# choutilin/makani

Measured on AMD Instinct MI355X. Metric: SFNO fwd+bwd samples/sec, 73ch 721x1440, higher is better.
Workload: dtype bf16; 1 GPU; sfno_linear_73chq_sc3_layers8_edim384 fwd+bwd+Adam, 73ch 721x1440, per-GPU batch 1; global_batch=1, parallelism=h1, spectral_dtype=f32 (GEMMs as 6 bf16 MFMA products of exact 3-way operand splits), step_launch=eager, micro_batches=1, python_gc=disabled in the timed region, adam=after backward

## Files before the change

include/makani_amd.h:

```cpp
#ifndef MAKANI_AMD_H
#define MAKANI_AMD_H

#include <stdint.h>

#ifdef __cplusplus
extern "C" {
#endif

int mk_version(void);
const char* mk_last_error(void);


int mk_quadrature(int grid, int nlat, double* theta, double* weights);

int mk_legendre_kpad(int nlat);

int mk_legendre_table(int grid, int nlat, int lmax, int mmax, int with_quad_weights, float* out);

int mk_fft_twiddle_len(int nlon);
int mk_fft_twiddles(int nlon, float* out);

int mk_rfft(const void* x, int x_dtype, float* xf, const float* twiddles,
            int bc, int nlat, int nlon, int mmax, float scale0, float scale_m, float scale_h,
            void* stream);

int mk_irfft(const float* xf, void* x, int x_dtype, const float* twiddles,
             int bc, int nlat, int nlon, int mmax, float scale0, float scale_m, float scale_h,
             void* stream);

int mk_legendre_fwd(const float* xf, const float* tab, float* c,
                    int bc, int nlat, int lmax, int mmax_loc, int m_off, int mmax_glob, void* stream);

int mk_legendre_inv(const float* c, const float* tab, float* xf,
                    int bc, int nlat, int lmax, int mmax_loc, int m_off, int mmax_glob, void* stream);

long long mk_legendre_x3_bytes(int nlat, int lmax, int mmax, int inverse);
int mk_legendre_x3_split(const float* tab, void* out, int nlat, int lmax, int mmax, int inverse, void* stream);
int mk_legendre_fwd_x3(const float* xf, const void* tab_x3, float* c,
                       int bc, int nlat, int lmax, int mmax_loc, int m_off, int mmax_glob, void* stream);
int mk_legendre_inv_x3(const float* c, const void* tab_x3, float* xf,
                       int bc, int nlat, int lmax, int mmax_loc, int m_off, int mmax_glob, void* stream);

int mk_rfft_ex(const void* x, int x_dtype, float* xf, const float* twiddles, int bc, int nlat, int nlon,
               int mmax, float scale0, float scale_m, float scale_h, int xf_layout, void* stream);
int mk_irfft_ex(const float* xf, void* x, int x_dtype, const float* twiddles, int bc, int nlat, int nlon,
                int mmax, float scale0, float scale_m, float scale_h, int xf_layout, void* stream);
int mk_legendre_fwd_x3_ex(const float* xf, const void* tab_x3, float* c, int bc, int nlat, int lmax,
                          int mmax_loc, int m_off, int mmax_glob, int xf_layout, void* stream);
int mk_legendre_inv_x3_ex(const float* c, const void* tab_x3, float* xf, int bc, int nlat, int lmax,
                          int mmax_loc, int m_off, int mmax_glob, int xf_layout, void* stream);

int mk_rfft_pm(const void* x, int x_dtype, float* xf, const float* twiddles, int bc, int nlat, int nlon, int mmax,
               float scale0, float scale_m, float scale_h, int chans, int chans_per_peer, void* stream);
int mk_irfft_pm(const float* xf, void* x, int x_dtype, const float* twiddles, int bc, int nlat, int nlon, int mmax,
                float scale0, float scale_m, float scale_h, int chans, int chans_per_peer, void* stream);

int mk_irfft_sums(const float* xf, void* x, int x_dtype, const float* twiddles, int bc, int nlat, int nlon, int mmax,
                  float scale0, float scale_m, float scale_h, int xf_layout, int chans, int chans_per_peer, double* rowsums,
                  void* stream);

int mk_dhconv_fwd(const float* x, const float* w, float* y, int lloc, int mloc, int batch,
                  int cin, int cout, int l_off, int m_off, void* stream);
int mk_dhconv_dgrad(const float* gy, const float* w, float* gx, int lloc, int mloc, int batch,
                    int cin, int cout, int l_off, int m_off, void* stream);
int mk_dhconv_wgrad(const float* x, const float* gy, float* gw, int lloc, int mloc, int batch,
                    int cin, int cout, int l_off, int m_off, void* stream);

int mk_dhconv_fwd_x3(const float* x, const float* w, float* y, int lloc, int mloc, int batch,
                     int cin, int cout, int l_off, int m_off, void* stream);
int mk_dhconv_dgrad_x3(const float* gy, const float* w, float* gx, int lloc, int mloc, int batch,
                       int cin, int cout, int l_off, int m_off, void* stream);
int mk_dhconv_wgrad_x3(const float* x, const float* gy, float* gw, int lloc, int mloc, int batch,
                       int cin, int cout, int l_off, int m_off, void* stream);

int mk_diag_fwd(const float* x, const float* w, float* y, int batch, int cin, int cout, long long P, void* stream);
int mk_diag_dgrad(const float* gy, const float* w, float* gx, int batch, int cin, int cout, long long P, void* stream);
int mk_diag_wgrad(const float* x, const float* gy, float* gw, int batch, int cin, int cout, long long P, void* stream);

int mk_spec_pack(const float* c_std, float* c_prv, int bc, int lloc, int mloc, void* stream);
int mk_spec_unpack(const float* c_prv, float* c_std, int bc, int lloc, int mloc,
                   int l_off, int m_off, void* stream);

int mk_bias_gelu_fwd(const void* x, const float* bias, void* y, int dtype, int rows, int C, long long P,
                     void* stream);
int mk_bias_gelu_bwd(const void* x, const float* bias, const void* gy, void* gx, float* gbias, int dtype,
                     int rows, int C, long long P, void* stream);
int mk_instnorm_fwd(const void* x, const float* weight, const float* bias, void* y, float* stats,
                    double* workspace, int dtype, int rows, int C, long long P, float eps, int fuse_gelu,
                    void* stream);
int mk_instnorm_bwd(const void* x, const void* gy, const float* stats, const float* weight, const float* bias,
                    void* gx, double* workspace, int dtype, int rows, int C, long long P, int fuse_gelu,
                    void* stream);

int mk_instnorm_fwd_ex(const void* x, const float* weight, const float* bias, void* y, float* stats,
                       double* workspace, int dtype, int rows, int C, long long P, long long count, float eps,
                       int fuse_gelu, int phase, void* stream);
int mk_instnorm_bwd_ex(const void* x, const void* gy, const float* stats, const float* weight, const float* bias,
                       void* gx, double* workspace, int dtype, int rows, int C, long long P, long long count,
                       int fuse_gelu, int phase, void* stream);
int mk_instnorm_bwd_wb(const void* x, const void* gy, const float* stats, const float* weight, const float* bias, void* gx,
                       double* workspace, float* gwb, int dtype, int C, long long P, int fuse_gelu, void* stream);

int mk_wmse_fwd(const void* pred, int dtype, const float* tar, const float* wrow, double* loss, long long rows,
                int H, int W, float scale, void* stream);
int mk_wmse_bwd(const void* pred, int dtype, const float* tar, const float* wrow, const float* gloss, void* gpred,
                long long rows, int H, int W, float scale, void* stream);

int mk_conv1x1_x3(const float* a, long long lda, const float* b, long long ldb, float* c, long long ldc, int M, int K, long long N,
                  int batch, long long sa, long long sb, long long sc, int mode, void* stream);
int mk_conv1x1_x3_bias_act(const float* a, long long lda, const float* b, long long ldb, float* c, long long ldc, int M, int K,
                           long long N, int batch, long long sb, long long sc, const float* bias, int act, void* stream);

int mk_conv1x1_wgrad(const void* gy, const void* x, float* gw, int batch, int cout, int cin, long long P,
                     void* stream);
int mk_conv1x1_wgrad_act(const void* gy, const void* x, float* gw, int batch, int cout, int cin, long long P, int x_act,
                         void* stream);
long long mk_pce_image_bytes(int M, int K);
int mk_pce_pack(const void* w, int w_dtype , int transpose, int M, int K, int ldw, void* img,
                void* stream);
int mk_pce_pack_layout(int M, int K, long long* out3);
int mk_pce_pack_batch(const void* desc_dev, int n, void* arena, long long total_elements, void* stream);
int mk_pce_gemm(const void* x, const void* wimg, void* y, const float* bias, const void* addend, const void* aux_in,
                void* aux_out, int gelu, int batch, int M, int K, long long P, void* stream);
int mk_pce_gemm_ex(const void* x, const void* wimg, void* y, const float* bias, const void* addend, const float* addend_affine,
                   const void* aux_in, void* aux_out, int gelu, double* rowstats, int batch, int M, int K, long long P,
                   void* stream);
long long mk_pce_mlp_image_bytes(int M, int Hd, int K1);
int mk_pce_mlp_pack(const void* a1, int a1_transposed, int lda1, const void* a2, int a2_transposed, int lda2,
                    int w_dtype , int M, int Hd, int K1, void* img, void* stream);
int mk_pce_mlp(const void* x, const void* wimg, void* y, void* mid_out, const void* mid_in, const float* b1, const float* b2,
               double* rowstats_y, double* rowsum_mid, int mode, int batch, int M, int Hd, int K1, long long P, void* stream);
int mk_pce_mlp_debug_stamps(unsigned long long* out512);
int mk_instnorm_coeffs(const double* sums, const float* weight, const float* bias, float* stats, float* affine, int rows,
                       int C, long long count, float eps, void* stream);
int mk_pce_debug_stamps(unsigned long long* out512);

int mk_adam_step(float* p, const float* g, float* m, float* v, long long n, float lr, float beta1, float beta2, float eps,
                 float weight_decay, int step, void* stream);

long long mk_mt_chunks(long long n);
int mk_mt_sumsq(int T, const uint64_t* x, const long long* n, double* partials, double* tsum, int clip_mode, float max_norm,
                float* norm_out, float* coef_out, float* steps, const int* inc_slots, int ninc, void* stream);
int mk_mt_norm_finish(int T, const double* tsum, int clip_mode, float max_norm, float* norm_out, float* coef_out,
                      float* steps, const int* inc_slots, int ninc, void* stream);
int mk_mt_step_inc(float* steps, const int* slots, int nslots, void* stream);
int mk_mt_scale(int T, const uint64_t* x, const long long* n, const float* coef, void* stream);
int mk_mt_adam(int T, const uint64_t* pgmv, const long long* n, const int* step_or_slot, const float* steps, float lr,
               const float* lr_dev, float beta1, float beta2, float eps, float weight_decay, int adamw, const float* coef,
               void* stream);
int mk_mt_lamb(int stage, int T, const uint64_t* pgmv, const long long* n, const int* step_or_slot, const float* steps,
               float lr, const float* lr_dev, float beta1, float beta2, float beta3, float eps, float weight_decay, int adamw,
               int bias_correction, int trust, const float* coef, double* part_p, double* part_u, double* tsum_p,
               double* tsum_u, void* stream);

long long mk_geo_metric_workspace(int B, int C, int H);
int mk_geo_metric_sums(const void* pred, int dtype, const float* tar, const float* clim, const float* wrow, double* workspace,
                       double* sums, int B, int C, int H, int W, void* stream);

long long mk_geo_lp_workspace(int B, int C, int H);
int mk_geo_lp_sums(const void* pred, int dtype, const float* tar, const float* wrow, double* workspace, double* sums, int p,
                   int B, int C, int H, int W, void* stream);
int mk_geo_lp_bwd(const void* pred, int dtype, const float* tar, const float* wrow, const float* g, void* gpred, int p,
                  int B, int C, int H, int W, void* stream);

int mk_input_assemble(const void* x, int x_dtype, const float* u, const float* stat, const float* mean, const float* std,
                      const int* mask_chans, int n_mask, int mask_src, void* out, int out_dtype, int B, int T, int C, int Cu,
                      int Cs, int H, int W, void* stream);
int mk_input_assemble_bwd(const void* gout, int g_dtype, const float* stat, const float* std, const int* mask_chans, int n_mask,
                          int mask_src, void* gx, int x_dtype, int B, int T, int C, int Cu, int Cs, int H, int W, void* stream);
// ... 10 lines not shown
```

makani_amd/_lib.py:

```python
import ctypes
import os

import torch

from . import build as _build

_LIB = None

_c_int = ctypes.c_int
_c_float = ctypes.c_float
_vp = ctypes.c_void_p

SIGNATURES = {
    "mk_version": (_c_int, []),
    "mk_last_error": (ctypes.c_char_p, []),
    "mk_quadrature": (_c_int, [_c_int, _c_int, _vp, _vp]),
    "mk_legendre_kpad": (_c_int, [_c_int]),
    "mk_legendre_table": (_c_int, [_c_int, _c_int, _c_int, _c_int, _c_int, _vp]),
    "mk_fft_twiddle_len": (_c_int, [_c_int]),
    "mk_fft_twiddles": (_c_int, [_c_int, _vp]),
    "mk_rfft": (_c_int, [_vp, _c_int, _vp, _vp, _c_int, _c_int, _c_int, _c_int, _c_float, _c_float, _c_float, _vp]),
    "mk_irfft": (_c_int, [_vp, _vp, _c_int, _vp, _c_int, _c_int, _c_int, _c_int, _c_float, _c_float, _c_float, _vp]),
    "mk_legendre_fwd": (_c_int, [_vp, _vp, _vp, _c_int, _c_int, _c_int, _c_int, _c_int, _c_int, _vp]),
    "mk_legendre_inv": (_c_int, [_vp, _vp, _vp, _c_int, _c_int, _c_int, _c_int, _c_int, _c_int, _vp]),
    "mk_legendre_x3_bytes": (ctypes.c_longlong, [_c_int, _c_int, _c_int, _c_int]),
    "mk_legendre_x3_split": (_c_int, [_vp, _vp, _c_int, _c_int, _c_int, _c_int, _vp]),
    "mk_legendre_fwd_x3": (_c_int, [_vp, _vp, _vp, _c_int, _c_int, _c_int, _c_int, _c_int, _c_int, _vp]),
    "mk_legendre_inv_x3": (_c_int, [_vp, _vp, _vp, _c_int, _c_int, _c_int, _c_int, _c_int, _c_int, _vp]),
    "mk_rfft_ex": (_c_int, [_vp, _c_int, _vp, _vp, _c_int, _c_int, _c_int, _c_int, _c_float, _c_float, _c_float, _c_int, _vp]),
    "mk_irfft_ex": (_c_int, [_vp, _vp, _c_int, _vp, _c_int, _c_int, _c_int, _c_int, _c_float, _c_float, _c_float, _c_int, _vp]),
    "mk_rfft_pm": (_c_int, [_vp, _c_int, _vp, _vp, _c_int, _c_int, _c_int, _c_int, _c_float, _c_float, _c_float, _c_int, _c_int, _vp]),
    "mk_irfft_pm": (_c_int, [_vp, _vp, _c_int, _vp, _c_int, _c_int, _c_int, _c_int, _c_float, _c_float, _c_float, _c_int, _c_int, _vp]),
    "mk_irfft_sums": (_c_int, [_vp, _vp, _c_int, _vp, _c_int, _c_int, _c_int, _c_int, _c_float, _c_float, _c_float, _c_int, _c_int,
                               _c_int, _vp, _vp]),
    "mk_legendre_fwd_x3_ex": (_c_int, [_vp, _vp, _vp, _c_int, _c_int, _c_int, _c_int, _c_int, _c_int, _c_int, _vp]),
    "mk_legendre_inv_x3_ex": (_c_int, [_vp, _vp, _vp, _c_int, _c_int, _c_int, _c_int, _c_int, _c_int, _c_int, _vp]),
    "mk_dhconv_fwd": (_c_int, [_vp, _vp, _vp] + [_c_int] * 7 + [_vp]),
    "mk_dhconv_dgrad": (_c_int, [_vp, _vp, _vp] + [_c_int] * 7 + [_vp]),
    "mk_dhconv_wgrad": (_c_int, [_vp, _vp, _vp] + [_c_int] * 7 + [_vp]),
    "mk_dhconv_fwd_x3": (_c_int, [_vp, _vp, _vp] + [_c_int] * 7 + [_vp]),
    "mk_dhconv_dgrad_x3": (_c_int, [_vp, _vp, _vp] + [_c_int] * 7 + [_vp]),
    "mk_dhconv_wgrad_x3": (_c_int, [_vp, _vp, _vp] + [_c_int] * 7 + [_vp]),
    "mk_diag_fwd": (_c_int, [_vp, _vp, _vp, _c_int, _c_int, _c_int, ctypes.c_longlong, _vp]),
    "mk_diag_dgrad": (_c_int, [_vp, _vp, _vp, _c_int, _c_int, _c_int, ctypes.c_longlong, _vp]),
    "mk_diag_wgrad": (_c_int, [_vp, _vp, _vp, _c_int, _c_int, _c_int, ctypes.c_longlong, _vp]),
    "mk_spec_pack": (_c_int, [_vp, _vp, _c_int, _c_int, _c_int, _vp]),
    "mk_spec_unpack": (_c_int, [_vp, _vp, _c_int, _c_int, _c_int, _c_int, _c_int, _vp]),
    "mk_bias_gelu_fwd": (_c_int, [_vp, _vp, _vp, _c_int, _c_int, _c_int, ctypes.c_longlong, _vp]),
    "mk_bias_gelu_bwd": (_c_int, [_vp, _vp, _vp, _vp, _vp, _c_int, _c_int, _c_int, ctypes.c_longlong, _vp]),
    "mk_instnorm_fwd": (_c_int, [_vp, _vp, _vp, _vp, _vp, _vp, _c_int, _c_int, _c_int, ctypes.c_longlong, _c_float,
                                 _c_int, _vp]),
    "mk_instnorm_fwd_ex": (_c_int, [_vp, _vp, _vp, _vp, _vp, _vp, _c_int, _c_int, _c_int, ctypes.c_longlong,
                                    ctypes.c_longlong, _c_float, _c_int, _c_int, _vp]),
    "mk_instnorm_bwd_ex": (_c_int, [_vp, _vp, _vp, _vp, _vp, _vp, _vp, _c_int, _c_int, _c_int, ctypes.c_longlong,
                                    ctypes.c_longlong, _c_int, _c_int, _vp]),
    "mk_instnorm_bwd_wb": (_c_int, [_vp, _vp, _vp, _vp, _vp, _vp, _vp, _vp, _c_int, _c_int, ctypes.c_longlong, _c_int, _vp]),
    "mk_wmse_fwd": (_c_int, [_vp, _c_int, _vp, _vp, _vp, ctypes.c_longlong, _c_int, _c_int, _c_float, _vp]),
    "mk_wmse_bwd": (_c_int, [_vp, _c_int, _vp, _vp, _vp, _vp, ctypes.c_longlong, _c_int, _c_int, _c_float, _vp]),
    "mk_conv1x1_wgrad": (_c_int, [_vp, _vp, _vp, _c_int, _c_int, _c_int, ctypes.c_longlong, _vp]),
    "mk_conv1x1_x3": (_c_int, [_vp, ctypes.c_longlong, _vp, ctypes.c_longlong, _vp, ctypes.c_longlong, _c_int, _c_int, ctypes.c_longlong,
                               _c_int, ctypes.c_longlong, ctypes.c_longlong, ctypes.c_longlong, _c_int, _vp]),
    "mk_conv1x1_x3_bias_act": (_c_int, [_vp, ctypes.c_longlong, _vp, ctypes.c_longlong, _vp, ctypes.c_longlong, _c_int, _c_int,
                                        ctypes.c_longlong, _c_int, ctypes.c_longlong, ctypes.c_longlong, _vp, _c_int, _vp]),
    "mk_conv1x1_wgrad_act": (_c_int, [_vp, _vp, _vp, _c_int, _c_int, _c_int, ctypes.c_longlong, _c_int, _vp]),
    "mk_pce_mlp_image_bytes": (ctypes.c_longlong, [_c_int, _c_int, _c_int]),
    "mk_pce_mlp_pack": (_c_int, [_vp, _c_int, _c_int, _vp, _c_int, _c_int, _c_int, _c_int, _c_int, _c_int, _vp, _vp]),
    "mk_pce_mlp": (_c_int, [_vp, _vp, _vp, _vp, _vp, _vp, _vp, _vp, _vp, _c_int, _c_int, _c_int, _c_int, _c_int,
                            ctypes.c_longlong, _vp]),
    "mk_pce_mlp_debug_stamps": (_c_int, [_vp]),
    "mk_pce_image_bytes": (ctypes.c_longlong, [_c_int, _c_int]),
    "mk_pce_pack": (_c_int, [_vp, _c_int, _c_int, _c_int, _c_int, _c_int, _vp, _vp]),
    "mk_pce_pack_layout": (_c_int, [_c_int, _c_int, _vp]),
    "mk_pce_pack_batch": (_c_int, [_vp, _c_int, _vp, ctypes.c_longlong, _vp]),
    "mk_pce_gemm": (_c_int, [_vp, _vp, _vp, _vp, _vp, _vp, _vp, _c_int, _c_int, _c_int, _c_int, ctypes.c_longlong, _vp]),
    "mk_pce_gemm_ex": (_c_int, [_vp, _vp, _vp, _vp, _vp, _vp, _vp, _vp, _c_int, _vp, _c_int, _c_int, _c_int, ctypes.c_longlong, _vp]),
    "mk_instnorm_coeffs": (_c_int, [_vp, _vp, _vp, _vp, _vp, _c_int, _c_int, ctypes.c_longlong, ctypes.c_float, _vp]),
    "mk_pce_debug_stamps": (_c_int, [_vp]),
    "mk_adam_step": (_c_int, [_vp, _vp, _vp, _vp, ctypes.c_longlong] + [_c_float] * 5 + [_c_int, _vp]),
    "mk_instnorm_bwd": (_c_int, [_vp, _vp, _vp, _vp, _vp, _vp, _vp, _c_int, _c_int, _c_int, ctypes.c_longlong,
                                 _c_int, _vp]),
    "mk_mt_chunks": (ctypes.c_longlong, [ctypes.c_longlong]),
    "mk_mt_sumsq": (_c_int, [_c_int, _vp, _vp, _vp, _vp, _c_int, _c_float, _vp, _vp, _vp, _vp, _c_int, _vp]),
    "mk_mt_norm_finish": (_c_int, [_c_int, _vp, _c_int, _c_float, _vp, _vp, _vp, _vp, _c_int, _vp]),
    "mk_mt_step_inc": (_c_int, [_vp, _vp, _c_int, _vp]),
    "mk_mt_scale": (_c_int, [_c_int, _vp, _vp, _vp, _vp]),
    "mk_mt_adam": (_c_int, [_c_int, _vp, _vp, _vp, _vp, _c_float, _vp] + [_c_float] * 4 + [_c_int, _vp, _vp]),
    "mk_mt_lamb": (_c_int, [_c_int, _c_int, _vp, _vp, _vp, _vp, _c_float, _vp] + [_c_float] * 5 + [_c_int] * 3
                   + [_vp] * 6),
    "mk_geo_metric_workspace": (ctypes.c_longlong, [_c_int, _c_int, _c_int]),
    "mk_geo_metric_sums": (_c_int, [_vp, _c_int, _vp, _vp, _vp, _vp, _vp, _c_int, _c_int, _c_int, _c_int, _vp]),
    "mk_geo_lp_workspace": (ctypes.c_longlong, [_c_int, _c_int, _c_int]),
    "mk_geo_lp_sums": (_c_int, [_vp, _c_int, _vp, _vp, _vp, _vp] + [_c_int] * 5 + [_vp]),
    "mk_geo_lp_bwd": (_c_int, [_vp, _c_int, _vp, _vp, _vp, _vp] + [_c_int] * 5 + [_vp]),
    "mk_input_assemble": (_c_int, [_vp, _c_int, _vp, _vp, _vp, _vp, _vp, _c_int, _c_int, _vp, _c_int] + [_c_int] * 7 + [_vp]),
    "mk_input_assemble_bwd": (_c_int, [_vp, _c_int, _vp, _vp, _vp, _c_int, _c_int, _vp, _c_int] + [_c_int] * 7 + [_vp]),
    "mk_history_workspace": (ctypes.c_longlong, [_c_int, _c_int, _c_int]),
    "mk_history_sums": (_c_int, [_vp, _c_int, _vp, _vp, _vp, _vp] + [_c_int] * 6 + [_vp]),
}


def lib_path():
    return _build.LIB


def load():
    global _LIB
    if _LIB is not None:
        return _LIB
    path = _build.LIB
    override = os.environ.get("MK_LIB_OVERRIDE")
    if override:
        path = override
    elif _build.stale():
        if _build.have_hipcc():
            path = _build.build(verbose=False)
        elif not os.path.exists(path):
            raise RuntimeError(f"makani_amd: {path} is missing and hipcc is not available to build it")
        else:
            raise RuntimeError(f"makani_amd: {path} is older than its sources and hipcc is not available to rebuild it")
    try:
        lib = ctypes.CDLL(path)
    except OSError as e:
        raise RuntimeError(f"makani_amd: cannot load the HIP extension {path}: {e}") from e
    for name, (res, args) in SIGNATURES.items():
        fn = getattr(lib, name)
# ... 11 lines not shown
```

makani_amd/csrc/fft.hip:

```cpp
#include "common.h"
#include "../../include/makani_amd.h"

#include <hip/hip_bf16.h>
#include <cstdlib>
#include <type_traits>
#include <utility>

namespace {

struct XfLayout {
    int sm, sk;
    int C, Cp, Bn;
    long long pstride;
};
static thread_local XfLayout g_xl = {0, 0, 0, 0, 0, 0};
static thread_local double* g_rowsums = nullptr;

struct XfChan {
    size_t pbase;
    int bcx0, BCx;
};
__device__ __forceinline__ XfChan xf_chan(const XfLayout& xl, int bc0, int BC) {
    XfChan c{0, bc0, BC};
    if (xl.Cp) {
        const int b = bc0 / xl.C, ch = bc0 - b * xl.C, pp = ch / xl.Cp;
        c.pbase = (size_t)pp * (size_t)xl.pstride;
        c.bcx0 = b * xl.Cp + (ch - pp * xl.Cp);
        c.BCx = xl.Bn * xl.Cp;
    }
    return c;
}


template <int I>
using IC = std::integral_constant<int, I>;

template <class F, int... Is>
__device__ __forceinline__ void static_for_impl(F&& f, std::integer_sequence<int, Is...>) {
    (f(IC<Is>{}), ...);
}
template <int N, class F>
__device__ __forceinline__ void static_for(F&& f) {
    static_for_impl(static_cast<F&&>(f), std::make_integer_sequence<int, N>{});
}

constexpr double kPi = 3.14159265358979323846264338327950288;

constexpr double cx_reduce(double x) {
    while (x > kPi) x -= 2.0 * kPi;
    while (x < -kPi) x += 2.0 * kPi;
    return x;
}
constexpr double cx_sin(double x) {
    x = cx_reduce(x);
    double term = x, sum = x;
    for (int n = 1; n < 20; ++n) {
        term *= -x * x / ((2.0 * n) * (2.0 * n + 1.0));
        sum += term;
    }
    return sum;
}
constexpr double cx_cos(double x) {
    x = cx_reduce(x);
    double term = 1.0, sum = 1.0;
    for (int n = 1; n < 20; ++n) {
        term *= -x * x / ((2.0 * n - 1.0) * (2.0 * n));
        sum += term;
    }
    return sum;
}

__device__ __forceinline__ float2 cmul(float2 a, float2 b) {
    return make_float2(a.x * b.x - a.y * b.y, a.x * b.y + a.y * b.x);
}
__device__ __forceinline__ float2 cadd(float2 a, float2 b) { return make_float2(a.x + b.x, a.y + b.y); }
__device__ __forceinline__ float2 csub(float2 a, float2 b) { return make_float2(a.x - b.x, a.y - b.y); }
__device__ __forceinline__ float2 mul_mi(float2 a) { return make_float2(a.y, -a.x); }

template <int R>
struct Dft;

template <>
struct Dft<2> {
    static __device__ __forceinline__ void run(float2 (&v)[2]) {
        const float2 a = v[0], b = v[1];
        v[0] = cadd(a, b);
        v[1] = csub(a, b);
    }
};

template <>
struct Dft<3> {
    static __device__ __forceinline__ void run(float2 (&v)[3]) {
        constexpr float s = 0.86602540378443864676f;
        const float2 t = cadd(v[1], v[2]);
        const float2 d = csub(v[1], v[2]);
        const float2 m = make_float2(v[0].x - 0.5f * t.x, v[0].y - 0.5f * t.y);
        const float2 q = mul_mi(make_float2(s * d.x, s * d.y));
// ... 403 lines not shown
    float* x = (float*)xout;
    MK_REQUIRE(x_dtype == 0 || x_dtype == 1, "x_dtype must be 0 (fp32) or 1 (bf16)");
    MK_REQUIRE(x_dtype == 0 || (!fft_legacy() && mmax <= 241 && (nlon == 480 || nlon == 1440)),
               "bf16 output rows are built for the production lengths only (nlon 480 / 1440, mmax <= 241)");
    MK_REQUIRE(x && xf && twiddles, "null pointer");
    MK_REQUIRE(bc > 0 && nlat > 0 && nlon >= 2 && nlon % 2 == 0, "bad sizes (nlon must be even)");
    MK_REQUIRE(mmax >= 1 && mmax <= nlon / 2 + 1, "mmax out of range");
    MK_REQUIRE((long long)nlat * mk::ceil_div(bc, 8) < 2147483647LL, "grid too large");
    hipStream_t st = (hipStream_t)stream;
    const bool split = !fft_legacy() && mmax <= 241 && (nlon == 480 || nlon == 1440);
    if (split && nlon == 480) {
        launch_irfft_split<1>(xf, xout, x_dtype, twiddles, bc, nlat, mmax, scale0, scale_m, scale_h, st);
    } else if (split) {
        launch_irfft_split<3>(xf, xout, x_dtype, twiddles, bc, nlat, mmax, scale0, scale_m, scale_h, st);
    } else
    switch (nlon / 2) {
#define X(H, G) \
    case H:     \
        launch_irfft<H, G>(xf, x, twiddles, bc, nlat, mmax, scale0, scale_m, scale_h, st); \
        break;
        MK_FFT_SIZES(X)
#undef X
        default: {
            MK_REQUIRE((long long)nlat * bc < 2147483647LL, "grid too large");
            const dim3 grid((unsigned)(nlat * bc));
            const size_t lds = sizeof(float2) * mmax;
            hipLaunchKernelGGL(irdft_generic_kernel, grid, dim3(kThreads), lds, st, (const float2*)xf, x,
                               (const float2*)twiddles, bc, nlat, nlon, mmax, scale0, scale_m, scale_h, g_xl);
        }
    }
    MK_LAUNCH_CHECK();
    return 0;
}

static int fft_pm_setup(int bc, int nlat, int nlon, int mmax, int chans, int chans_per_peer) {
    MK_REQUIRE(chans > 0 && chans_per_peer > 0 && bc % chans == 0 && chans % chans_per_peer == 0, "bad channel blocking");
    MK_REQUIRE(chans_per_peer % 24 == 0, "channel blocks must be multiples of 24 (tiles of 8 / 24 rows must not straddle them)");
    MK_REQUIRE(!fft_legacy() && mmax <= 241 && (nlon == 480 || nlon == 1440), "peer-major rows exist for the split kernels only");
    const int Bn = bc / chans;
    g_xl = XfLayout{1, mmax, chans, chans_per_peer, Bn, (long long)nlat * mmax * Bn * chans_per_peer};
    return 0;
}

extern "C" int mk_rfft_pm(const void* x, int x_dtype, float* xf, const float* twiddles, int bc, int nlat, int nlon, int mmax,
                          float scale0, float scale_m, float scale_h, int chans, int chans_per_peer, void* stream) {
    MK_REQUIRE(x && xf && twiddles, "null pointer");
    MK_REQUIRE(bc > 0 && nlat > 0 && mmax >= 1, "bad sizes");
    MK_REQUIRE(x_dtype == 0 || x_dtype == 1, "x_dtype must be 0 (fp32) or 1 (bf16)");
    if (int e = fft_pm_setup(bc, nlat, nlon, mmax, chans, chans_per_peer)) return e;
    if (nlon == 480)
        launch_rfft_split<1>(x, x_dtype, xf, twiddles, bc, nlat, mmax, scale0, scale_m, scale_h, (hipStream_t)stream);
    else
        launch_rfft_split<3>(x, x_dtype, xf, twiddles, bc, nlat, mmax, scale0, scale_m, scale_h, (hipStream_t)stream);
    MK_LAUNCH_CHECK();
    return 0;
}

extern "C" int mk_irfft_pm(const float* xf, void* x, int x_dtype, const float* twiddles, int bc, int nlat, int nlon, int mmax,
                           float scale0, float scale_m, float scale_h, int chans, int chans_per_peer, void* stream) {
    MK_REQUIRE(x && xf && twiddles, "null pointer");
    MK_REQUIRE(bc > 0 && nlat > 0 && mmax >= 1, "bad sizes");
    MK_REQUIRE(x_dtype == 0 || x_dtype == 1, "x_dtype must be 0 (fp32) or 1 (bf16)");
    if (int e = fft_pm_setup(bc, nlat, nlon, mmax, chans, chans_per_peer)) return e;
    if (nlon == 480)
        launch_irfft_split<1>(xf, x, x_dtype, twiddles, bc, nlat, mmax, scale0, scale_m, scale_h, (hipStream_t)stream);
    else
        launch_irfft_split<3>(xf, x, x_dtype, twiddles, bc, nlat, mmax, scale0, scale_m, scale_h, (hipStream_t)stream);
    MK_LAUNCH_CHECK();
    return 0;
}

extern "C" int mk_irfft_sums(const float* xf, void* x, int x_dtype, const float* twiddles, int bc, int nlat, int nlon, int mmax,
                             float scale0, float scale_m, float scale_h, int xf_layout, int chans, int chans_per_peer,
                             double* rowsums, void* stream) {
    MK_REQUIRE(rowsums != nullptr, "null pointer");
    MK_REQUIRE(!fft_legacy() && mmax <= 241 && (nlon == 480 || nlon == 1440), "row statistics come from the split kernels only");
    g_rowsums = rowsums;
    const int rc = chans_per_peer > 0
        ? mk_irfft_pm(xf, x, x_dtype, twiddles, bc, nlat, nlon, mmax, scale0, scale_m, scale_h, chans, chans_per_peer, stream)
        : mk_irfft_ex(xf, x, x_dtype, twiddles, bc, nlat, nlon, mmax, scale0, scale_m, scale_h, xf_layout, stream);
    g_rowsums = nullptr;
    return rc;
}
```

makani_amd/csrc/fft_split.h:

```cpp

constexpr int SH = 240;
constexpr int SP = 272;
constexpr int SNSUB = 24;
constexpr int STHREADS = 384;
constexpr int SLDS_F2 = SNSUB * SP + 96;

__device__ __forceinline__ int pair_tile(int i) {
    const int xcd = i & 7, seq = i >> 3;
    return ((((seq >> 1) << 3) + xcd) << 1) + (seq & 1);
}

__device__ __forceinline__ int sub_base(int sr, int S) { return sr * SP + 4 * (sr / S); }
__device__ __forceinline__ int phi(int i) { return i + (i >> 4); }
__device__ __forceinline__ int opaque(int v) {
    asm volatile("" : "+v"(v));
    return v;
}

template <typename T> __device__ __forceinline__ float as_stored(float v);
template <> __device__ __forceinline__ float as_stored<float>(float v) { return v; }
template <> __device__ __forceinline__ float as_stored<__hip_bfloat16>(float v) { return __bfloat162float(__float2bfloat16(v)); }

template <bool SUMS = false, typename TOut = float>
__device__ __forceinline__ void split_passes(float2* lds, int tid, int S, const float2 (&tw15)[15], float* red = nullptr) {
// ... 111 lines not shown
#pragma unroll
            for (int c = 0; c < S; ++c) InVec<TIn>::unpack(raw[it][c], vals[c]);
#pragma unroll
            for (int sq = 0; sq < S; ++sq) {
                float4* dst = reinterpret_cast<float4*>(lds + sub_base(g * S + sq, S) + (E / 2) * p);
#pragma unroll
                for (int h = 0; h < E / 4; ++h) {
                    float o[4];
#pragma unroll
                    for (int a = 0; a < 4; ++a) {
                        const int f = (4 * h + a) * S + sq;
                        o[a] = vals[f / E][f % E];
                    }
                    dst[h] = make_float4(o[0], o[1], o[2], o[3]);
                }
            }
        }
    }
    __syncthreads();
    if (!(exp & 2)) split_passes(lds, tid, S, tw15);
    float2 wfirst[S];
    wfirst[0] = tw[HH + S * (tid / G)];
#pragma unroll
    for (int s = 1; s < S; ++s) wfirst[s] = tw[HH + s * (tid / G)];
    __syncthreads();
    if (exp & 8) return;

    const float2* tw2 = tw + HH;
    constexpr int NPAIR = SH / 2 + 1;
    constexpr int STEP = STHREADS / G, PIT = (NPAIR + STEP - 1) / STEP;
    static_assert(STHREADS % G == 0, "items of a thread must keep their channel");
    const int mp0 = tid / G, g = tid - mp0 * G;
    if (bc0 + g < BC) {
        float2* dst0 = xf + xc.pbase + ((size_t)mp0 * xl.sm + (size_t)k * xl.sk) * xc.BCx + (xc.bcx0 + g);
        float2* dst1 = xf + xc.pbase + ((size_t)(SH - mp0) * xl.sm + (size_t)k * xl.sk) * xc.BCx + (xc.bcx0 + g);
        const ptrdiff_t dstep = (ptrdiff_t)STEP * xl.sm * xc.BCx;
#pragma unroll
        for (int it = 0; it < PIT; ++it) {
            const int mp = mp0 + STEP * it;
            if (mp < NPAIR) {
                const int m1 = SH - mp;
                const int p0 = phi(mp), p1 = phi(mp == 0 ? 0 : m1);
                const float2 wsub = it ? cmul(wfirst[0], tw2[S * STEP * it]) : wfirst[0];
                float2 acc0 = make_float2(0.f, 0.f), acc1 = make_float2(0.f, 0.f);
#pragma unroll
                for (int s = 0; s < S; ++s) {
                    const float2* zs = lds + sub_base(g * S + s, S);
                    const float2 a = zs[p0];
                    const float2 b = zs[p1];
                    const float2 e = make_float2(0.5f * (a.x + b.x), 0.5f * (a.y - b.y));
                    const float2 d = make_float2(0.5f * (a.x - b.x), 0.5f * (a.y + b.y));
                    const float2 pp = cmul(wsub, d);
                    float2 f0 = make_float2(e.x + pp.y, e.y - pp.x);
                    float2 f1 = make_float2(e.x - pp.y, -e.y - pp.x);
                    if (s > 0) {
                        const float2 w = it ? cmul(wfirst[s], tw2[s * STEP * it]) : wfirst[s];
                        constexpr float kc[3] = {1.f, 0.5f, -0.5f}, ks[3] = {0.f, -0.86602540378443864676f, -0.86602540378443864676f};
                        static_assert(S == 1 || S == 3, "combine constants are for S = 3");
                        f0 = cmul(f0, w);
                        f1 = cmul(f1, cmul(make_float2(w.x, -w.y), make_float2(kc[s], ks[s])));
                    }
                    acc0 = cadd(acc0, f0);
                    acc1 = cadd(acc1, f1);
                }
                if (exp & 4) {
                    if (acc0.x + acc1.x != 12345.678f) continue;
                }
                if (mp < M) {
                    const float sc = (mp == 0) ? scale0 : scale_m;
                    dst0[(ptrdiff_t)it * dstep] = make_float2(sc * acc0.x, sc * acc0.y);
                }
                if (m1 != mp && m1 < M) {
                    const float sc = (m1 == HH) ? scale_h : scale_m;
                    dst1[-(ptrdiff_t)it * dstep] = make_float2(sc * acc1.x, sc * acc1.y);
                }
            }
        }
    }
}

template <typename T> struct OutVec;
template <> struct OutVec<float> {
    static constexpr int E = 4;
    static __device__ __forceinline__ void store(float* p, const float (&o)[4]) {
        *reinterpret_cast<float4*>(p) = make_float4(o[0], o[1], o[2], o[3]);
    }
};
template <> struct OutVec<__hip_bfloat16> {
    static constexpr int E = 8;
    static __device__ __forceinline__ void store(__hip_bfloat16* p, const float (&o)[8]) {
        __hip_bfloat16 h[8];
#pragma unroll
        for (int i = 0; i < 8; ++i) h[i] = __float2bfloat16(o[i]);
        *reinterpret_cast<uint4*>(p) = *reinterpret_cast<const uint4*>(h);
    }
};

template <int S, typename TOut, bool WIDE, int PERSIST, bool SUMS = false>
__global__ __launch_bounds__(STHREADS, PERSIST ? 3 : 5) void irfft_split_kernel(const float2* __restrict__ xf, TOut* __restrict__ x,
                                                               const float2* __restrict__ tw, int BC, int K, int M,
                                                               float scale0, float scale_m, float scale_h, XfLayout xl,
                                                               double* __restrict__ rowsums) {
    constexpr int N = 480 * S, G = SNSUB / S, HH = N / 2;
    extern __shared__ __attribute__((aligned(16))) float2 lds[];
    float* red = reinterpret_cast<float*>(lds + SLDS_F2);
    const int tid = threadIdx.x;
    const int ntile = (BC + G - 1) / G;
    const int total = ntile * K;
    const float2* tw2 = tw + HH;
    const int total16 = (total + 15) & ~15;
    auto next_valid = [&](int i) {
        while (i < total16 && pair_tile(i) >= total) i += (int)gridDim.x;
        return i;
    };
    int sched = PERSIST ? next_valid(blockIdx.x) : (int)blockIdx.x;
    if (sched >= total16) return;
    int tile = pair_tile(sched);
    if (!PERSIST && tile >= total) return;

    float2 tw15[15];
    auto load_tw15 = [&]() {
#pragma unroll
        for (int r = 0; r < 15; ++r) tw15[r] = tw[((tid & 15) * r) * S];
    };
    if constexpr (PERSIST != 0) load_tw15();

    float2 wfirst[S];
    wfirst[0] = tw2[S * (tid / G)];
#pragma unroll
    for (int s = 1; s < S; ++s) wfirst[s] = tw2[s * (tid / G)];

    constexpr int NPAIR = SH / 2 + 1;
    constexpr int PIT = (G * NPAIR + STHREADS - 1) / STHREADS;
    float2 xa[PIT], xb[PIT];
    constexpr int STEP = STHREADS / G;
    static_assert(STHREADS % G == 0 && PIT == (NPAIR + STEP - 1) / STEP, "items of a thread keep their channel");
    auto gather = [&](int t, int tl) {
        const int k = t / ntile, bc0 = (t - k * ntile) * G;
        const XfChan xc = xf_chan(xl, bc0, BC);
        const int jp0 = tl / G, g = tl - jp0 * G;
        const bool chan_ok = bc0 + g < BC;
        if constexpr (!WIDE) {
            typedef unsigned int gf_u2 __attribute__((ext_vector_type(2)));
            const float2* tbase = xf + xc.pbase + (size_t)k * xl.sk * xc.BCx + xc.bcx0;
            const __amdgpu_buffer_rsrc_t rs = __builtin_amdgcn_make_buffer_rsrc(const_cast<float2*>(tbase), 0, 0x7FFFFFFF, 0x00020000);
            const unsigned mstride = (unsigned)xl.sm * (unsigned)xc.BCx * 8u;
            unsigned offa = (unsigned)g * 8u + (unsigned)jp0 * mstride;
            unsigned offb = (unsigned)g * 8u + (unsigned)(SH - jp0) * mstride;
            const unsigned dstepb = (unsigned)STEP * mstride;
#pragma unroll
            for (int it = 0; it < PIT; ++it) {
                const int jp = jp0 + STEP * it, j1 = SH - jp;
                const bool oa = chan_ok && jp < NPAIR && jp < M, ob = chan_ok && jp < NPAIR && j1 < M;
                xa[it] = __builtin_bit_cast(float2, (gf_u2)__builtin_amdgcn_raw_buffer_load_b64(rs, oa ? offa : 0x80000000u, 0, 0));
                xb[it] = __builtin_bit_cast(float2, (gf_u2)__builtin_amdgcn_raw_buffer_load_b64(rs, ob ? offb : 0x80000000u, 0, 0));
                offa += dstepb;
                offb -= dstepb;
            }
        } else {
            const float2* base = xf + xc.pbase + (size_t)k * xl.sk * xc.BCx + (xc.bcx0 + g);
#pragma unroll
            for (int it = 0; it < PIT; ++it) {
                const int jp = jp0 + STEP * it, j1 = SH - jp;
                const bool oa = chan_ok && jp < NPAIR && jp < M, ob = chan_ok && jp < NPAIR && j1 < M;
                xa[it] = *(oa ? base + (size_t)jp * xl.sm * xc.BCx : xf);
                xb[it] = *(ob ? base + (size_t)j1 * xl.sm * xc.BCx : xf);
            }
        }
    };
    gather(tile, tid);
  for (;;) {
    const int tl = opaque(tid);
    const int k = tile / ntile, bc0 = (tile - k * ntile) * G;
    const int jp0 = tl / G, g = tl - jp0 * G;
    const bool chan_ok = bc0 + g < BC;
#pragma unroll
    for (int it = 0; it < PIT; ++it) {
        const int jp = jp0 + STEP * it;
        if (jp >= NPAIR) continue;
        const int j1 = SH - jp;
        const float sa = (chan_ok && jp < M) ? ((jp == 0) ? scale0 : scale_m) : 0.f;
        const float sb = (chan_ok && j1 < M) ? ((j1 == HH) ? scale_h : scale_m) : 0.f;
        const float2 a0 = make_float2(sa * xa[it].x, sa * xa[it].y);
        const float2 b0 = make_float2(sb * xb[it].x, sb * xb[it].y);
        float2 wsub = it ? cmul(wfirst[0], tw2[S * STEP * it]) : wfirst[0];
        wsub.y = -wsub.y;
#pragma unroll
        for (int s = 0; s < S; ++s) {
            float2 ya = a0, yb = b0;
            if (s > 0) {
                constexpr float kc[3] = {1.f, 0.5f, -0.5f}, ks[3] = {0.f, 0.86602540378443864676f, 0.86602540378443864676f};
                const float2 w = it ? cmul(wfirst[s], tw2[s * STEP * it]) : wfirst[s];
                ya = cmul(ya, make_float2(w.x, -w.y));
                yb = cmul(yb, cmul(w, make_float2(kc[s], ks[s])));
            }
            if (jp == 0) {
                ya.y = 0.f;
                yb.y = 0.f;
                if (S > 1) yb.x *= 2.f;
            }
            const float2 e = make_float2(ya.x + yb.x, ya.y - yb.y);
            const float2 d = make_float2(ya.x - yb.x, ya.y + yb.y);
            const float2 t = cmul(wsub, d);
            float2* zs = lds + sub_base(g * S + s, S);
            zs[jp] = make_float2(e.x - t.y, -(e.y + t.x));
            if (jp != 0 && j1 != jp) zs[j1] = make_float2(e.x + t.y, e.y - t.x);
        }
    }
    if constexpr (PERSIST == 0) load_tw15();
    __syncthreads();
    const int next = PERSIST ? next_valid(sched + (int)gridDim.x) : total16;
    if (next < total16) gather(pair_tile(next), opaque(tid));
    if constexpr (SUMS) split_passes<true, TOut>(lds, tl, S, tw15, red);
    else split_passes(lds, tl, S, tw15);
    __syncthreads();
    if (SUMS && tl < 2 * G) {
        const int gch = tl >> 1, t = tl & 1;
        if (bc0 + gch < BC) {
            float v = 0.f;
#pragma unroll
            for (int sq = 0; sq < S; ++sq) v += red[2 * (gch * S + sq) + t];
            atomicAdd(&rowsums[2 * (size_t)(bc0 + gch) + t], (double)v);
        }
    }

    constexpr int EO = OutVec<TOut>::E;
    constexpr int GPR = N / (EO * S), NGRP = G * GPR, OIT = (NGRP + STHREADS - 1) / STHREADS;
#pragma unroll
    for (int it = 0; it < OIT; ++it) {
        const int v = tl + it * STHREADS;
        const int g = v / GPR, p = v - g * GPR;
        if (v < NGRP && bc0 + g < BC) {
            float r[S][EO];
#pragma unroll
            for (int sq = 0; sq < S; ++sq) {
                const float2* zs = lds + sub_base(g * S + sq, S) + phi((EO / 2) * p);
#pragma unroll
                for (int h = 0; h < EO / 2; ++h) {
                    const float2 z = zs[h];
                    r[sq][2 * h] = z.x;
                    r[sq][2 * h + 1] = -z.y;
                }
            }
            TOut* dst = x + ((size_t)(bc0 + g) * K + k) * N + (size_t)p * EO * S;
#pragma unroll
            for (int c = 0; c < S; ++c) {
                float o[EO];
#pragma unroll
                for (int e = 0; e < EO; ++e) {
                    const int f = c * EO + e;
                    o[e] = r[f % S][f / S];
                }
                OutVec<TOut>::store(dst + c * EO, o);
            }
        }
    }
    if (next >= total16) break;
    sched = next;
    tile = pair_tile(next);
    __syncthreads();
  }
}

static inline unsigned split_grid(long long tiles) { return (unsigned)((tiles + 15) / 16 * 16); }

static inline int fft_exp() {
    static const int v = [] { const char* e = getenv("MK_FFT_EXP"); return e ? atoi(e) : 0; }();
    return v;
}

template <int S>
int launch_rfft_split(const void* x, int x_dtype, float* xf, const float* tw, int bc, int nlat, int mmax, float s0,
                      float sm, float sh, hipStream_t st) {
    constexpr int G = SNSUB / S;
    const dim3 grid((unsigned)((mk::ceil_div(bc, G) * nlat + 15) / 16 * 16));
    const size_t lds = sizeof(float2) * SLDS_F2;
    if (x_dtype == 0)
        hipLaunchKernelGGL((rfft_split_kernel<S, float>), grid, dim3(STHREADS), lds, st, (const float*)x, (float2*)xf,
                           (const float2*)tw, bc, nlat, mmax, s0, sm, sh, fft_exp(), g_xl);
    else
        hipLaunchKernelGGL((rfft_split_kernel<S, __hip_bfloat16>), grid, dim3(STHREADS), lds, st,
                           (const __hip_bfloat16*)x, (float2*)xf, (const float2*)tw, bc, nlat, mmax, s0, sm, sh, fft_exp(), g_xl);
    return 0;
}

template <int S>
int launch_irfft_split(const float* xf, void* x, int x_dtype, const float* tw, int bc, int nlat, int mmax, float s0,
                       float sm, float sh, hipStream_t st) {
    constexpr int G = SNSUB / S;
    const dim3 grid(split_grid(mk::ceil_div(bc, G) * (long long)nlat));
    const size_t lds = sizeof(float2) * SLDS_F2 + 2 * SNSUB * sizeof(float);
    const long long bcx = g_xl.Cp ? (long long)g_xl.Bn * g_xl.Cp : (long long)bc;
    const bool wide = ((long long)SH * g_xl.sm + 1) * bcx * 8 >= (1LL << 31);
#define MK_IRFFT_LAUNCH(T, W, PS, SM)                                                                                  \
    hipLaunchKernelGGL((irfft_split_kernel<S, T, W, PS, SM>), grid, dim3(STHREADS), lds, st, (const float2*)xf, (T*)x,    \
                       (const float2*)tw, bc, nlat, mmax, s0, sm, sh, g_xl, g_rowsums)
#define MK_IRFFT_PICK(T)                                                                                               \
    if (g_rowsums) {                                                                                                   \
        if (wide) MK_IRFFT_LAUNCH(T, true, 1, true); else MK_IRFFT_LAUNCH(T, false, 0, true);                          \
    } else {                                                                                                           \
        if (wide) MK_IRFFT_LAUNCH(T, true, 1, false); else MK_IRFFT_LAUNCH(T, false, 0, false);                        \
    }
    if (x_dtype == 0) {
        MK_IRFFT_PICK(float)
    } else {
        MK_IRFFT_PICK(__hip_bfloat16)
    }
#undef MK_IRFFT_PICK
#undef MK_IRFFT_LAUNCH
    return 0;
}

static inline bool fft_legacy() {
    static const bool v = [] {
        const char* e = getenv("MK_FFT_LEGACY");
        return e && e[0] == '1';
    }();
    return v;
}
```

makani_amd/csrc/gemm_x3.hip:

```cpp
#include "common.h"
#include "../../include/makani_amd.h"

#include <cstdint>
#include <cstdlib>

namespace {

typedef float f32x16 __attribute__((ext_vector_type(16)));
typedef __bf16 bf16x8 __attribute__((ext_vector_type(8)));
typedef uint32_t u32x4 __attribute__((ext_vector_type(4)));

#ifndef MK_X3_DB
#define MK_X3_DB 1
#endif
constexpr int X3_DB = MK_X3_DB;
constexpr int XT = 256;
constexpr int XM = 128, XN = 128, XK = 32;
constexpr int XPITCH = 208;
constexpr int XROWB = 192;
constexpr int XIMG = XM * XPITCH + 128;
constexpr int X3_LDS = 2 * XIMG;

__device__ __forceinline__ int plain_off(int r) { return r * XPITCH; }
__device__ __forceinline__ int pair_off(int r) { return ((r >> 1) + ((r & 1) << 6)) * XPITCH + ((r & 1) << 7); }
// ... 247 lines not shown
#pragma unroll
                for (int t = 0; t < 6; ++t)
#pragma unroll
                    for (int b = 0; b < 2; ++b) {
#if defined(MK_X3_SKIP25)
                        if (s == 1 && b == 1) continue;
#endif
#if defined(MK_X3_NOMFMA)
                        acc[a][b][t] += __builtin_bit_cast(float4, af[PA[t]]).x * __builtin_bit_cast(float4, bf[b][PB[t]]).y;
#elif defined(MK_X3_AGPR)
                        asm volatile("v_mfma_f32_32x32x16_bf16 %0, %1, %2, %0" : "+a"(acc[a][b]) : "v"(af[PA[t]]), "v"(bf[b][PB[t]]));
#else
                        acc[a][b] = __builtin_amdgcn_mfma_f32_32x32x16_bf16(af[PA[t]], bf[b][PB[t]], acc[a][b], 0, 0, 0);
#endif
                    }
            }
    }
}

template <int DB, class AS, class BS, int EPI = 0>
__device__ __forceinline__ void x3_tile(const AS& as, const BS& bs, int kt0, int kt1, int rvalid, int cvalid, float* cbase,
                                        long long ldc, char* lds, int exp = 0, const float* rowbias = nullptr, int act = 0) {
    const int tid = threadIdx.x, lane = tid & 63;
    const int wave = __builtin_amdgcn_readfirstlane(tid >> 6);
    const int wr = wave >> 1, wc = wave & 1;
    const int fi = lane & 31, kg = lane >> 5;
    char* As = lds;
    char* Bs = lds + XIMG;

    f32x16 acc[2][2];
#pragma unroll
    for (int a = 0; a < 2; ++a)
#pragma unroll
        for (int b = 0; b < 2; ++b)
#pragma unroll
            for (int r = 0; r < 16; ++r) acc[a][b][r] = 0.f;
#if !defined(MK_X3_VGPR_ACC)
    asm volatile("" : "+a"(acc[0][0]), "+a"(acc[0][1]), "+a"(acc[1][0]), "+a"(acc[1][1]));
#endif

    bool live[2];
    int a_off[2], b_off[2];
#pragma unroll
    for (int a = 0; a < 2; ++a) {
        a_off[a] = AS::row_off(wr * 64 + a * 32 + fi) + kg * 16;
        b_off[a] = BS::row_off(wc * 64 + 2 * fi + a) + kg * 16;
        live[a] = (wr * 64 + a * 32 < rvalid) && (wc * 64 < cvalid);
    }

    typename AS::Regs ra;
    typename BS::Regs rb[DB];
    if (kt0 < kt1) {
        as.gload(kt0, ra, tid);
        bs.gload(kt0, rb[0], tid);
        as.sstore(ra, As, tid);
        bs.sstore(rb[0], Bs, tid);
        __syncthreads();
        if (kt0 + 1 < kt1) as.gload(kt0 + 1, ra, tid);
#pragma unroll
        for (int j = 0; j < DB; ++j)
            if (kt0 + 1 + j < kt1) bs.gload(kt0 + 1 + j, rb[j], tid);
    }
    for (int ktb = kt0; ktb < kt1; ktb += DB) {
#pragma unroll
        for (int j = 0; j < DB; ++j) {
            const int kt = ktb + j;
            if (kt >= kt1) break;
            if (!(exp & 4)) x3_mfma_step(As, Bs, a_off, b_off, live, acc);
            if (kt + 1 < kt1) {
                __syncthreads();
                if (!(exp & 2)) {
                    as.sstore(ra, As, tid);
                    bs.sstore(rb[j], Bs, tid);
                }
                __syncthreads();
                if (!(exp & 1)) {
                    if (kt + 2 < kt1 && !(exp & 8)) as.gload(kt + 2, ra, tid);
                    if (kt + 1 + DB < kt1 && !(exp & 16)) bs.gload(kt + 1 + DB, rb[j], tid);
                }
            }
        }
    }
    const int col = wc * 64 + 2 * fi;
    if (col < cvalid) {
#pragma unroll
        for (int a = 0; a < 2; ++a)
#pragma unroll
            for (int r = 0; r < 16; ++r) {
                const int row = wr * 64 + a * 32 + (r & 3) + 8 * (r >> 2) + 4 * kg;
                if (row < rvalid) {
                    if constexpr (EPI == 1) {
                        float2* d = reinterpret_cast<float2*>(cbase + (long long)row * ldc + col);
                        const float2 o = *d;
                        *d = make_float2(o.x + acc[a][0][r], o.y + acc[a][1][r]);
                        continue;
                    } else if constexpr (EPI == 2) {
                        atomicAdd(cbase + (long long)row * ldc + col, acc[a][0][r]);
                        if (col + 1 < cvalid) atomicAdd(cbase + (long long)row * ldc + col + 1, acc[a][1][r]);
                        continue;
                    } else if constexpr (EPI == 3) {
                        const float bv = rowbias ? rowbias[row] : 0.f;
                        float v0 = acc[a][0][r] + bv, v1 = acc[a][1][r] + bv;
                        if (act) {
                            v0 = 0.5f * v0 * (1.f + erff(v0 * 0.70710678118654752440f));
                            v1 = 0.5f * v1 * (1.f + erff(v1 * 0.70710678118654752440f));
                        }
                        *reinterpret_cast<float2*>(cbase + (long long)row * ldc + col) = make_float2(v0, v1);
                        continue;
                    }
#ifndef MK_X3_PLAIN_STORE
                    typedef float x3_f2 __attribute__((ext_vector_type(2)));
                    x3_f2 v2;
                    v2[0] = acc[a][0][r];
                    v2[1] = acc[a][1][r];
                    __builtin_nontemporal_store(v2, reinterpret_cast<x3_f2*>(cbase + (long long)row * ldc + col));
#else
                    *reinterpret_cast<float2*>(cbase + (long long)row * ldc + col) = make_float2(acc[a][0][r], acc[a][1][r]);
#endif
                }
            }
    }
}

struct TileId {
    int batch, tm, tn;
    bool valid;
};
__device__ __forceinline__ TileId decode_block(int nbatch, int tiles_m, int tiles_n) {
    const int bid = blockIdx.x;
    const int xcd = bid & 7, q = bid >> 3;
    const int T = tiles_m * tiles_n;
    TileId t;
    t.batch = (q / T) * 8 + xcd;
    const int r = q % T;
    t.tm = r / tiles_n;
    t.tn = r - t.tm * tiles_n;
    t.valid = t.batch < nbatch;
    return t;
}
static inline long long grid_blocks(int nbatch, int tiles_m, int tiles_n) {
    return (long long)mk::ceil_div(nbatch, 8) * 8 * tiles_m * tiles_n;
}

static int x3_exp() {
    static const int v = [] { const char* e = getenv("MK_X3_EXP"); return e ? atoi(e) : 0; }();
    return v;
}

struct LegX3Params {
    const float* src;
    const char* tab;
    float* dst;
    int K, L, Mloc, m_off, N2;
    int RT;
    int KC;
    int tiles_n;
    int kmajor;
    int exp;
};

template <class AS>
__global__ __launch_bounds__(XT, 3) void legendre_fwd_x3_kernel(LegX3Params p) {
    extern __shared__ __attribute__((aligned(16))) char lds_x3[];
    const TileId t = decode_block(p.Mloc, p.RT, p.tiles_n);
    if (!t.valid) return;
    const int m = t.batch, mg = p.m_off + m;
// ... 195 lines not shown
    if (nblk >= 2147483647LL) return -1;
    if (33LL * p.Mloc * p.N2 * 4 >= (1LL << 31)) return -2;
    const dim3 grid((unsigned)nblk), blk(XT);
    if (fwd) hipLaunchKernelGGL(legendre_fwd_x3_kernel<F32TileStager>, grid, blk, X3_LDS, st, p);
    else hipLaunchKernelGGL(legendre_inv_x3_kernel<F32TileStager>, grid, blk, X3_LDS, st, p);
    return 0;
}

extern "C" int mk_legendre_fwd_x3_ex(const float* xf, const void* tab_x3, float* c, int bc, int nlat, int lmax,
                                     int mmax_loc, int m_off, int mmax_glob, int xf_layout, void* stream) {
    MK_REQUIRE(xf && tab_x3 && c, "null pointer");
    MK_REQUIRE(bc > 0 && nlat > 0 && lmax > 0 && mmax_loc > 0, "bad sizes");
    MK_REQUIRE(m_off >= 0 && m_off + mmax_loc <= mmax_glob, "mode shard out of range");
    MK_REQUIRE(xf_layout == 0 || xf_layout == 1, "xf_layout must be 0 ([M][K][BC]) or 1 ([K][M][BC])");
    MK_REQUIRE(legendre_x3_launch(true, xf, tab_x3, c, bc, nlat, lmax, mmax_loc, m_off, xf_layout, (hipStream_t)stream) == 0,
               "operand too large: grid over 2^31 blocks, or 33 * mmax_loc * 2 * bc * 4 bytes (one k-step of the data operand) over 2^31");
    MK_LAUNCH_CHECK();
    return 0;
}

extern "C" int mk_legendre_fwd_x3(const float* xf, const void* tab_x3, float* c, int bc, int nlat, int lmax, int mmax_loc,
                                  int m_off, int mmax_glob, void* stream) {
    return mk_legendre_fwd_x3_ex(xf, tab_x3, c, bc, nlat, lmax, mmax_loc, m_off, mmax_glob, 0, stream);
}

extern "C" int mk_legendre_inv_x3_ex(const float* c, const void* tab_x3, float* xf, int bc, int nlat, int lmax,
                                     int mmax_loc, int m_off, int mmax_glob, int xf_layout, void* stream) {
    MK_REQUIRE(xf && tab_x3 && c, "null pointer");
    MK_REQUIRE(bc > 0 && nlat > 0 && lmax > 0 && mmax_loc > 0, "bad sizes");
    MK_REQUIRE(m_off >= 0 && m_off + mmax_loc <= mmax_glob, "mode shard out of range");
    MK_REQUIRE(xf_layout == 0 || xf_layout == 1, "xf_layout must be 0 ([M][K][BC]) or 1 ([K][M][BC])");
    MK_REQUIRE(legendre_x3_launch(false, c, tab_x3, xf, bc, nlat, lmax, mmax_loc, m_off, xf_layout, (hipStream_t)stream) == 0,
               "operand too large: grid over 2^31 blocks, or 33 * mmax_loc * 2 * bc * 4 bytes (one k-step of the data operand) over 2^31");
    MK_LAUNCH_CHECK();
    return 0;
}

extern "C" int mk_legendre_inv_x3(const float* c, const void* tab_x3, float* xf, int bc, int nlat, int lmax, int mmax_loc,
                                  int m_off, int mmax_glob, void* stream) {
    return mk_legendre_inv_x3_ex(c, tab_x3, xf, bc, nlat, lmax, mmax_loc, m_off, mmax_glob, 0, stream);
}

static int dh_x3_check(const void* a, const void* b, const void* c, int lloc, int mloc, int batch, int cin, int cout,
                       int l_off, int m_off) {
    MK_REQUIRE(a && b && c, "null pointer");
    MK_REQUIRE(lloc > 0 && mloc > 0 && batch > 0 && cin > 0 && cout > 0, "bad sizes");
    MK_REQUIRE(l_off >= 0 && m_off >= 0, "negative shard offset");
    MK_REQUIRE(cin % 2 == 0 && cout % 2 == 0, "the bf16x3 dhconv kernels need even channel counts (use the fp32 kernels)");
    return 0;
}

extern "C" int mk_dhconv_fwd_x3(const float* x, const float* w, float* y, int lloc, int mloc, int batch, int cin,
                                int cout, int l_off, int m_off, void* stream) {
    if (int e = dh_x3_check(x, w, y, lloc, mloc, batch, cin, cout, l_off, m_off)) return e;
    DhX3Params p{x, w, y, lloc, mloc, batch, cin, cout, l_off, m_off, mk::ceil_div(mloc * batch, XM),
                 mk::ceil_div(2 * cout, XN), x3_exp()};
    const long long nblk = grid_blocks(lloc, p.tiles_m, p.tiles_n);
    MK_REQUIRE(nblk < 2147483647LL, "grid too large");
    hipLaunchKernelGGL(dhconv_fwd_x3_kernel, dim3((unsigned)nblk), dim3(XT), X3_LDS, (hipStream_t)stream, p);
    MK_LAUNCH_CHECK();
    return 0;
}

extern "C" int mk_dhconv_dgrad_x3(const float* gy, const float* w, float* gx, int lloc, int mloc, int batch, int cin,
                                  int cout, int l_off, int m_off, void* stream) {
    if (int e = dh_x3_check(gy, w, gx, lloc, mloc, batch, cin, cout, l_off, m_off)) return e;
    DhX3Params p{gy, w, gx, lloc, mloc, batch, cin, cout, l_off, m_off, mk::ceil_div(mloc * batch, XM),
                 mk::ceil_div(2 * cin, XN), x3_exp()};
    const long long nblk = grid_blocks(lloc, p.tiles_m, p.tiles_n);
    MK_REQUIRE(nblk < 2147483647LL, "grid too large");
    hipLaunchKernelGGL(dhconv_dgrad_x3_kernel, dim3((unsigned)nblk), dim3(XT), X3_LDS, (hipStream_t)stream, p);
    MK_LAUNCH_CHECK();
    return 0;
}

extern "C" int mk_dhconv_wgrad_x3(const float* x, const float* gy, float* gw, int lloc, int mloc, int batch, int cin,
                                  int cout, int l_off, int m_off, void* stream) {
    if (int e = dh_x3_check(x, gy, gw, lloc, mloc, batch, cin, cout, l_off, m_off)) return e;
    DhX3Params p{x, gy, gw, lloc, mloc, batch, cin, cout, l_off, m_off, mk::ceil_div(cin, XM),
                 mk::ceil_div(2 * cout, XN), x3_exp()};
    const long long nblk = grid_blocks(lloc, p.tiles_m, p.tiles_n);
    MK_REQUIRE(nblk < 2147483647LL, "grid too large");
    hipLaunchKernelGGL(dhconv_wgrad_x3_kernel, dim3((unsigned)nblk), dim3(XT), X3_LDS, (hipStream_t)stream, p);
    MK_LAUNCH_CHECK();
    return 0;
}


namespace {
struct ConvX3Params {
    const float* a;
    const float* b;
    float* c;
    long long lda, ldb, ldc, sa, sb, sc;
    int M, K, N, nwork, tiles_m, tiles_n, nslab, kslab;
    const float* bias;
    int act;
};
template <int MODE>
__global__ __launch_bounds__(XT, 3) void conv_x3_kernel(ConvX3Params p) {
    extern __shared__ __attribute__((aligned(16))) char lds_x3[];
    TileId t = decode_block(p.nwork, p.tiles_m, MODE == 2 ? p.tiles_n : 1);
    if (!t.valid) return;
    if constexpr (MODE != 2) {
        const int w = t.batch;
        t.batch = w / p.tiles_n;
        t.tn = w - t.batch * p.tiles_n;
    }
    const int m0 = t.tm * XM, n0 = t.tn * XN;
    if constexpr (MODE == 2) {
        const int b = t.batch / p.nslab, slab = t.batch - b * p.nslab;
        const int kt0 = slab * p.kslab, ktn = (p.K + XK - 1) / XK;
        const int kt1 = kt0 + p.kslab < ktn ? kt0 + p.kslab : ktn;
        RowStager as, bs;
        as.base = p.a + b * p.sa + (long long)m0 * p.lda;
        as.ld = p.lda;
        as.rows = p.M - m0;
        as.kvalid = p.K;
        bs.base = p.b + b * p.sb + (long long)n0 * p.ldb;
        bs.ld = p.ldb;
        bs.rows = p.N - n0;
        bs.kvalid = p.K;
        x3_tile<X3_DB, RowStager, RowStager, 2>(as, bs, kt0, kt1, p.M - m0, p.N - n0, p.c + (long long)m0 * p.ldc + n0, p.ldc, lds_x3);
    } else {
        RowStager as;
        as.base = p.a + (long long)m0 * p.lda;
        as.ld = p.lda;
        as.rows = p.M - m0;
        as.kvalid = (p.K + 3) / 4 * 4;
        TransStager bs;
        bs.base = p.b + t.batch * p.sb + n0;
        bs.ldk = p.ldb;
        bs.k_lo = 0;
        bs.k_hi = p.K;
        bs.cvalid = p.N - n0;
        x3_tile<X3_DB, RowStager, TransStager, MODE>(as, bs, 0, (p.K + XK - 1) / XK, p.M - m0, p.N - n0,
                                                     p.c + t.batch * p.sc + (long long)m0 * p.ldc + n0, p.ldc, lds_x3, 0,
                                                     (MODE == 3 && p.bias) ? p.bias + m0 : nullptr, p.act);
    }
}
}

static int conv_x3_launch(const float* a, long long lda, const float* b, long long ldb, float* c, long long ldc, int M, int K,
                          long long N, int batch, long long sa, long long sb, long long sc, int mode, const float* bias, int act,
                          void* stream) {
    MK_REQUIRE(a && b && c, "null pointer");
    MK_REQUIRE(M > 0 && K > 0 && N > 0 && batch > 0, "bad sizes");
    MK_REQUIRE(mode >= 0 && mode <= 3, "mode must be 0 (store), 1 (accumulate), 2 (weight gradient) or 3 (store with bias / GELU)");
    MK_REQUIRE((((uintptr_t)a | (uintptr_t)b | (uintptr_t)c) & 15) == 0, "operands must be 16-byte aligned");
    ConvX3Params p;
    p.a = a; p.b = b; p.c = c;
    p.lda = lda; p.ldb = ldb; p.ldc = ldc;
    p.sa = sa; p.sb = sb; p.sc = sc;
    p.M = M; p.K = K;
    p.bias = bias; p.act = act;
    MK_REQUIRE(N < 2147483647LL, "N too large");
    p.N = (int)N;
    p.tiles_m = mk::ceil_div(M, XM);
    p.tiles_n = mk::ceil_div((int)N, XN);
    p.nslab = 1;
    p.kslab = 0;
    if (mode == 2) {
        MK_REQUIRE(lda % 4 == 0 && ldb % 4 == 0 && K % 4 == 0 && sa % 4 == 0 && sb % 4 == 0, "weight gradient: row strides and the contraction length must be multiples of 4");
        const int ktn = mk::ceil_div(K, XK);
        long long want = 1536 / ((long long)p.tiles_m * p.tiles_n * batch);
        if (want < 1) want = 1;
// ... 36 lines not shown
```

makani_amd/csrc/pointwise.hip:

```cpp
#include "common.h"
#include "../../include/makani_amd.h"

#include <hip/hip_bf16.h>

namespace {

constexpr int kT = 256;
constexpr int kE = 8;
constexpr int kSteps = 4;
constexpr int kChunk = kT * kE * kSteps;

template <typename T> struct IO;
template <> struct IO<float> {
    static __device__ __forceinline__ void load(const float* p, float (&v)[kE]) {
        const float4 a = reinterpret_cast<const float4*>(p)[0], b = reinterpret_cast<const float4*>(p)[1];
        v[0] = a.x; v[1] = a.y; v[2] = a.z; v[3] = a.w; v[4] = b.x; v[5] = b.y; v[6] = b.z; v[7] = b.w;
    }
    static __device__ __forceinline__ void store(float* p, const float (&v)[kE]) {
        reinterpret_cast<float4*>(p)[0] = make_float4(v[0], v[1], v[2], v[3]);
        reinterpret_cast<float4*>(p)[1] = make_float4(v[4], v[5], v[6], v[7]);
    }
    static __device__ __forceinline__ float ld1(const float* p) { return *p; }
    static __device__ __forceinline__ void st1(float* p, float v) { *p = v; }
};
// ... 47 lines not shown
        const PhiPair c = normal_cdf_pdf_fast(z);
        return fmaf(z, c.phi, c.Phi);
    }
};

template <typename T, class F>
__device__ __forceinline__ void for_chunk(long long P, F&& f) {
    const long long c0 = (long long)blockIdx.x * kChunk;
#pragma unroll
    for (int s = 0; s < kSteps; ++s) {
        const long long off = c0 + ((long long)s * kT + threadIdx.x) * kE;
        if (off + kE <= P)
            f(off, kE);
        else if (off < P)
            f(off, (int)(P - off));
    }
}

__device__ __forceinline__ float block_sum(float v, float* red) {
#pragma unroll
    for (int o = 32; o > 0; o >>= 1) v += __shfl_down(v, o, 64);
    const int lane = threadIdx.x & 63, wave = threadIdx.x >> 6;
    __syncthreads();
    if (lane == 0) red[wave] = v;
    __syncthreads();
    return red[0] + red[1] + red[2] + red[3];
}

template <typename T>
__global__ __launch_bounds__(kT) void bias_gelu_fwd_kernel(const T* __restrict__ x, const float* __restrict__ bias,
                                                           T* __restrict__ y, int C, long long P) {
    const int row = blockIdx.y;
    const float b = bias ? bias[row % C] : 0.f;
    const T* xr = x + (long long)row * P;
    T* yr = y + (long long)row * P;
    for_chunk<T>(P, [&](long long off, int n) {
        float v[kE];
        if (n == kE) {
            IO<T>::load(xr + off, v);
#pragma unroll
            for (int i = 0; i < kE; ++i) v[i] = Act<T>::gelu(v[i] + b);
            IO<T>::store(yr + off, v);
        } else {
            for (int i = 0; i < n; ++i) IO<T>::st1(yr + off + i, Act<T>::gelu(IO<T>::ld1(xr + off + i) + b));
        }
    });
}

template <typename T>
__global__ __launch_bounds__(kT) void bias_gelu_bwd_kernel(const T* __restrict__ x, const float* __restrict__ bias,
                                                           const T* __restrict__ gy, T* __restrict__ gx,
                                                           float* __restrict__ gbias, int C, long long P) {
    __shared__ float red[4];
    const int row = blockIdx.y;
    const float b = bias ? bias[row % C] : 0.f;
    const long long ro = (long long)row * P;
    float acc = 0.f;
    for_chunk<T>(P, [&](long long off, int n) {
        float v[kE], g[kE];
        if (n == kE) {
            IO<T>::load(x + ro + off, v);
            IO<T>::load(gy + ro + off, g);
#pragma unroll
            for (int i = 0; i < kE; ++i) {
                g[i] *= Act<T>::gelu_grad(v[i] + b);
                acc += g[i];
            }
            IO<T>::store(gx + ro + off, g);
        } else {
            for (int i = 0; i < n; ++i) {
                const float r = IO<T>::ld1(gy + ro + off + i) * Act<T>::gelu_grad(IO<T>::ld1(x + ro + off + i) + b);
                acc += r;
                IO<T>::st1(gx + ro + off + i, r);
            }
        }
    });
    if (gbias) {
        const float s = block_sum(acc, red);
        if (threadIdx.x == 0) atomicAdd(&gbias[row % C], s);
    }
}

template <typename T>
__global__ __launch_bounds__(kT) void rowsum2_kernel(const T* __restrict__ x, double* __restrict__ sums, long long P) {
    __shared__ float red[4];
    const int row = blockIdx.y;
    const T* xr = x + (long long)row * P;
    float s1 = 0.f, s2 = 0.f;
    for_chunk<T>(P, [&](long long off, int n) {
        float v[kE];
        if (n == kE) {
            IO<T>::load(xr + off, v);
#pragma unroll
            for (int i = 0; i < kE; ++i) {
                s1 += v[i];
                s2 = fmaf(v[i], v[i], s2);
            }
        } else {
            for (int i = 0; i < n; ++i) {
                const float t = IO<T>::ld1(xr + off + i);
                s1 += t;
                s2 = fmaf(t, t, s2);
            }
        }
    });
    const float t1 = block_sum(s1, red);
    const float t2 = block_sum(s2, red);
    if (threadIdx.x == 0) {
        atomicAdd(&sums[2 * row], (double)t1);
        atomicAdd(&sums[2 * row + 1], (double)t2);
    }
}

template <typename T, bool GELU>
__global__ __launch_bounds__(kT) void instnorm_apply_kernel(const T* __restrict__ x, const double* __restrict__ sums,
                                                            const float* __restrict__ w, const float* __restrict__ b,
                                                            T* __restrict__ y, float* __restrict__ stats, int C,
                                                            long long P, double count, float eps) {
    const int row = blockIdx.y, c = row % C;
    const double mean_d = sums[2 * row] / count;
    double var_d = sums[2 * row + 1] / count - mean_d * mean_d;
    if (var_d < 0.0) var_d = 0.0;
    const float mean = (float)mean_d, rstd = (float)(1.0 / sqrt(var_d + (double)eps));
    if (blockIdx.x == 0 && threadIdx.x == 0) {
        stats[2 * row] = mean;
        stats[2 * row + 1] = rstd;
    }
    const float sc = rstd * (w ? w[c] : 1.f), sh = (b ? b[c] : 0.f) - mean * sc;
    const T* xr = x + (long long)row * P;
    T* yr = y + (long long)row * P;
    for_chunk<T>(P, [&](long long off, int n) {
        float v[kE];
        if (n == kE) {
            IO<T>::load(xr + off, v);
#pragma unroll
            for (int i = 0; i < kE; ++i) {
                const float z = fmaf(v[i], sc, sh);
                v[i] = GELU ? Act<T>::gelu(z) : z;
            }
            IO<T>::store(yr + off, v);
        } else {
            for (int i = 0; i < n; ++i) {
                const float z = fmaf(IO<T>::ld1(xr + off + i), sc, sh);
                IO<T>::st1(yr + off + i, GELU ? Act<T>::gelu(z) : z);
            }
        }
    });
}

template <typename T, bool GELU>
__global__ __launch_bounds__(kT) void instnorm_bwd_sums_kernel(const T* __restrict__ x, const T* __restrict__ gy,
                                                               const float* __restrict__ stats,
                                                               const float* __restrict__ w, const float* __restrict__ b,
                                                               double* __restrict__ sums, int C, long long P) {
    __shared__ float red[4];
    const int row = blockIdx.y, c = row % C;
    const float mean = stats[2 * row], rstd = stats[2 * row + 1];
    const float wc = w ? w[c] : 1.f, bc = b ? b[c] : 0.f;
    const long long ro = (long long)row * P;
    float s1 = 0.f, s2 = 0.f;
    for_chunk<T>(P, [&](long long off, int n) {
        float v[kE], g[kE];
        if (n == kE) {
            IO<T>::load(x + ro + off, v);
            IO<T>::load(gy + ro + off, g);
        } else {
// ... 22 lines not shown
template <typename T, bool GELU>
__global__ __launch_bounds__(kT) void instnorm_bwd_apply_kernel(const T* __restrict__ x, const T* __restrict__ gy,
                                                                const float* __restrict__ stats,
                                                                const float* __restrict__ w, const float* __restrict__ b,
                                                                const double* __restrict__ sums, T* __restrict__ gx, int C,
                                                                long long P, double count, float* __restrict__ gwb) {
    const int row = blockIdx.y, c = row % C;
    const float mean = stats[2 * row], rstd = stats[2 * row + 1];
    const float wc = w ? w[c] : 1.f, bc = b ? b[c] : 0.f;
    const float m1 = (float)(sums[2 * row] / count), m2 = (float)(sums[2 * row + 1] / count);
    if (gwb != nullptr && blockIdx.x == 0 && threadIdx.x == 0) {
        gwb[c] = (float)sums[2 * row + 1];
        gwb[C + c] = (float)sums[2 * row];
    }
    const float k = wc * rstd;
    const long long ro = (long long)row * P;
    for_chunk<T>(P, [&](long long off, int n) {
        float v[kE], g[kE];
        if (n == kE) {
            IO<T>::load(x + ro + off, v);
            IO<T>::load(gy + ro + off, g);
#pragma unroll
            for (int i = 0; i < kE; ++i) {
                const float xh = (v[i] - mean) * rstd;
                float gi = g[i];
                if (GELU) gi *= Act<T>::gelu_grad(fmaf(xh, wc, bc));
                g[i] = k * (gi - m1 - xh * m2);
            }
            IO<T>::store(gx + ro + off, g);
        } else {
            for (int i = 0; i < n; ++i) {
                const float xh = (IO<T>::ld1(x + ro + off + i) - mean) * rstd;
                float gi = IO<T>::ld1(gy + ro + off + i);
                if (GELU) gi *= Act<T>::gelu_grad(fmaf(xh, wc, bc));
                IO<T>::st1(gx + ro + off + i, k * (gi - m1 - xh * m2));
            }
        }
    });
}

inline dim3 pw_grid(long long rows, long long P) { return dim3((unsigned)((P + kChunk - 1) / kChunk), (unsigned)rows); }

__global__ void zero_doubles_kernel(double* p, int n) {
    const int i = blockIdx.x * blockDim.x + threadIdx.x;
    if (i < n) p[i] = 0.0;
}
static inline void zero_doubles(double* p, int n, hipStream_t st) {
    hipLaunchKernelGGL(zero_doubles_kernel, dim3((unsigned)((n + 255) / 256)), dim3(256), 0, st, p, n);
}

}

#define PW_CHECK()                                                                              \
    MK_REQUIRE(rows > 0 && rows <= 65535 && C > 0 && P > 0, "bad sizes (rows = B*C must be <= 65535)"); \
    MK_REQUIRE(dtype == 0 || dtype == 1, "dtype must be 0 (fp32) or 1 (bf16)");                 \
    MK_REQUIRE((P % 8) == 0, "P = H*W must be a multiple of 8 (16-byte row alignment)")

extern "C" int mk_bias_gelu_fwd(const void* x, const float* bias, void* y, int dtype, int rows, int C, long long P,
                                void* stream) {
    MK_REQUIRE(x && y, "null pointer");
    PW_CHECK();
    hipStream_t st = (hipStream_t)stream;
    if (dtype == 0)
        hipLaunchKernelGGL(bias_gelu_fwd_kernel<float>, pw_grid(rows, P), dim3(kT), 0, st, (const float*)x, bias,
                           (float*)y, C, P);
    else
        hipLaunchKernelGGL(bias_gelu_fwd_kernel<__hip_bfloat16>, pw_grid(rows, P), dim3(kT), 0, st,
                           (const __hip_bfloat16*)x, bias, (__hip_bfloat16*)y, C, P);
    MK_LAUNCH_CHECK();
    return 0;
}

extern "C" int mk_bias_gelu_bwd(const void* x, const float* bias, const void* gy, void* gx, float* gbias, int dtype,
                                int rows, int C, long long P, void* stream) {
    MK_REQUIRE(x && gy && gx, "null pointer");
    PW_CHECK();
    hipStream_t st = (hipStream_t)stream;
    if (dtype == 0)
        hipLaunchKernelGGL(bias_gelu_bwd_kernel<float>, pw_grid(rows, P), dim3(kT), 0, st, (const float*)x, bias,
                           (const float*)gy, (float*)gx, gbias, C, P);
    else
        hipLaunchKernelGGL(bias_gelu_bwd_kernel<__hip_bfloat16>, pw_grid(rows, P), dim3(kT), 0, st,
                           (const __hip_bfloat16*)x, bias, (const __hip_bfloat16*)gy, (__hip_bfloat16*)gx, gbias, C, P);
    MK_LAUNCH_CHECK();
    return 0;
}

extern "C" int mk_instnorm_fwd_ex(const void* x, const float* weight, const float* bias, void* y, float* stats,
                                  double* workspace, int dtype, int rows, int C, long long P, long long count, float eps,
                                  int fuse_gelu, int phase, void* stream) {
    MK_REQUIRE(x && workspace, "null pointer");
    MK_REQUIRE(phase == 1 || (y && stats), "null pointer");
    MK_REQUIRE(phase >= 0 && phase <= 2 && count > 0, "bad phase / count");
    PW_CHECK();
    hipStream_t st = (hipStream_t)stream;
    if (phase != 2) zero_doubles(workspace, 2 * rows, st);
    const dim3 g = pw_grid(rows, P);
    const double cnt = (double)count;
#define LAUNCH(T)                                                                                              \
    if (phase != 2) hipLaunchKernelGGL(rowsum2_kernel<T>, g, dim3(kT), 0, st, (const T*)x, workspace, P);      \
    if (phase != 1) {                                                                                          \
        if (fuse_gelu)                                                                                         \
            hipLaunchKernelGGL((instnorm_apply_kernel<T, true>), g, dim3(kT), 0, st, (const T*)x, workspace, weight, \
                               bias, (T*)y, stats, C, P, cnt, eps);                                            \
        else                                                                                                   \
            hipLaunchKernelGGL((instnorm_apply_kernel<T, false>), g, dim3(kT), 0, st, (const T*)x, workspace, weight, \
                               bias, (T*)y, stats, C, P, cnt, eps);                                            \
    }
    if (dtype == 0) {
        LAUNCH(float)
    } else {
        LAUNCH(__hip_bfloat16)
    }
#undef LAUNCH
    MK_LAUNCH_CHECK();
    return 0;
}

extern "C" int mk_instnorm_fwd(const void* x, const float* weight, const float* bias, void* y, float* stats,
                               double* workspace, int dtype, int rows, int C, long long P, float eps, int fuse_gelu,
                               void* stream) {
    return mk_instnorm_fwd_ex(x, weight, bias, y, stats, workspace, dtype, rows, C, P, P, eps, fuse_gelu, 0, stream);
}

namespace {
__global__ void instnorm_coeffs_kernel(const double* __restrict__ sums, const float* __restrict__ w, const float* __restrict__ b,
                                       float* __restrict__ stats, float* __restrict__ affine, int rows, int C, double count,
                                       float eps) {
    const int row = blockIdx.x * blockDim.x + threadIdx.x;
    if (row >= rows) return;
    const int c = row % C;
    const double mean_d = sums[2 * row] / count;
    double var_d = sums[2 * row + 1] / count - mean_d * mean_d;
    if (var_d < 0.0) var_d = 0.0;
    const float mean = (float)mean_d, rstd = (float)(1.0 / sqrt(var_d + (double)eps));
    stats[2 * row] = mean;
    stats[2 * row + 1] = rstd;
    const float sc = rstd * (w ? w[c] : 1.f);
    affine[2 * row] = sc;
    affine[2 * row + 1] = (b ? b[c] : 0.f) - mean * sc;
}
}

extern "C" int mk_instnorm_coeffs(const double* sums, const float* weight, const float* bias, float* stats, float* affine,
                                  int rows, int C, long long count, float eps, void* stream) {
    MK_REQUIRE(sums && stats && affine, "null pointer");
    MK_REQUIRE(rows > 0 && C > 0 && count > 0, "bad sizes");
    hipLaunchKernelGGL(instnorm_coeffs_kernel, dim3((unsigned)((rows + 255) / 256)), dim3(256), 0, (hipStream_t)stream, sums,
                       weight, bias, stats, affine, rows, C, (double)count, eps);
    MK_LAUNCH_CHECK();
    return 0;
}

static int instnorm_bwd_launch(const void* x, const void* gy, const float* stats, const float* weight,
                               const float* bias, void* gx, double* workspace, int dtype, int rows, int C, long long P,
                               long long count, int fuse_gelu, int phase, float* gwb, void* stream) {
    MK_REQUIRE(x && gy && stats && workspace, "null pointer");
    MK_REQUIRE(gwb == nullptr || (rows == C && phase == 0), "parameter gradients from the kernel: one sample, unsharded rows only");
    MK_REQUIRE(phase == 1 || gx, "null pointer");
    MK_REQUIRE(phase >= 0 && phase <= 2 && count > 0, "bad phase / count");
    PW_CHECK();
    hipStream_t st = (hipStream_t)stream;
    if (phase != 2) zero_doubles(workspace, 2 * rows, st);
    const dim3 g = pw_grid(rows, P);
    const double cnt = (double)count;
#define LAUNCH(T, G)                                                                                               \
// ... 109 lines not shown
```

makani_amd/layers.py:

```python
import math
import os

import torch
import torch.nn as nn
import torch.nn.functional as F
from torch.utils.checkpoint import checkpoint


class _X3Conv(torch.autograd.Function):

    @staticmethod
    def forward(ctx, x3, w, addend):
        from . import ops
        wf = w.detach().float()
        ctx.save_for_backward(x3, wf)
        ctx.cfg = (w.dtype, addend is not None)
        return ops.conv1x1_x3(wf, x3, out=None if addend is None else addend.detach())

    @staticmethod
    def backward(ctx, gy):
        from . import ops
        x3, wf = ctx.saved_tensors
        wdt, has_addend = ctx.cfg
        gy = gy.contiguous()
# ... 83 lines not shown
    def backward(ctx, gy):
        from . import ops
        x3, w = ctx.saved_tensors
        has_bias, has_addend = ctx.has
        gy = gy.contiguous()
        gx = gw = gb = None
        (wimg_t, gbuf), ctx.step = (ctx.step or (None, None)), None
        if ctx.needs_input_grad[0]:
            gx = ops.pce_gemm(gy, wimg_t if wimg_t is not None else ops.pce_pack(w, transpose=True), w.shape[1])
        if ctx.needs_input_grad[1]:
            gw = ops.conv1x1_wgrad_raw(gy, x3, out=gbuf).to(w.dtype)
        if has_bias and ctx.needs_input_grad[2]:
            gb = _row_sums(gy).to(ctx.bias_dtype)
        return gx, gw, gb, (gy if has_addend else None)


class _PceConvNormAdd(torch.autograd.Function):

    @staticmethod
    def forward(ctx, x3, w, bias, z4, sums, nw, nb, eps, group, count):
        from . import ops
        B, C, H, W = z4.shape
        if group is not None:
            torch.distributed.all_reduce(sums, group=group)
        cnt = H * W if group is None else int(count)
        wf = None if nw is None else nw.detach().float().contiguous()
        bf = None if nb is None else nb.detach().float().contiguous()
        stats, affine = ops.instance_norm_coeffs(sums, wf, bf, B * C, C, cnt, eps)
        y = ops.pce_gemm(x3, ops.pce_pack(w), w.shape[0], bias=bias, addend=z4.view(B, C, H * W), addend_affine=affine)
        empty = z4.new_empty(0, dtype=torch.float32)
        ctx.save_for_backward(x3, w, z4, stats, wf if wf is not None else empty, bf if bf is not None else empty)
        ctx.cfg = (None if bias is None else bias.dtype, None if nw is None else nw.dtype, None if nb is None else nb.dtype,
                   group, cnt)
        ctx.step = _step_items(w)
        return y

    @staticmethod
    def backward(ctx, gy):
        from . import ops
        x3, w, z4, stats, wf, bf = ctx.saved_tensors
        bias_dtype, nw_dtype, nb_dtype, group, cnt = ctx.cfg
        B, C, H, W = z4.shape
        gy = gy.contiguous()
        gx = gw = gb = None
        (wimg_t, gbuf), ctx.step = (ctx.step or (None, None)), None
        if ctx.needs_input_grad[0]:
            gx = ops.pce_gemm(gy, wimg_t if wimg_t is not None else ops.pce_pack(w, transpose=True), w.shape[1])
        if ctx.needs_input_grad[1]:
            gw = ops.conv1x1_wgrad_raw(gy, x3, out=gbuf).to(w.dtype)
        if bias_dtype is not None and ctx.needs_input_grad[2]:
            gb = _row_sums(gy).to(bias_dtype)
        gz, gnw, gnb = ops.instance_norm_backward(z4, gy.view(B, C, H, W), stats, wf if nw_dtype is not None else None,
                                                  bf if nb_dtype is not None else None, False, group, cnt,
                                                  grad_dtype=nw_dtype if (nw_dtype is not None and nw_dtype == nb_dtype) else None)
        return (gx, gw, gb, gz, None, gnw.to(nw_dtype) if nw_dtype is not None else None,
                gnb.to(nb_dtype) if nb_dtype is not None else None, None, None, None)


def conv_plus_instance_norm(conv, x, z, sums, norm):
    from . import comm, ops
    from .layer_norm import DistributedInstanceNorm2d
    if sums is None or not isinstance(conv, Conv1x1) or z.dtype != torch.bfloat16 or not z.is_contiguous() or z.dim() != 4:
        return None
    if os.environ.get("MK_NORM_SKIP_FUSION", "1") == "0":
        return None
    group = count = None
    if isinstance(norm, DistributedInstanceNorm2d):
        if comm.get_size("spatial") > 1:
            group, count = comm.get_group("spatial"), norm._global_count(z)
        nw, nb = (norm.weight, norm.bias) if norm.affine else (None, None)
    elif isinstance(norm, InstanceNorm2d) and not norm.track_running_stats:
        nw, nb = norm.weight, norm.bias
    else:
        return None
    x3 = _engine_field(x)
    if x3 is None or not ops.pce_supported_train(conv.out_channels, conv.in_channels) or conv.out_channels != z.shape[1]:
        return None
    B, H, W = x.shape[0], x.shape[-2], x.shape[-1]
    if tuple(z.shape) != (B, conv.out_channels, H, W):
        return None
    with torch.autocast("cuda", enabled=False):
        y = _PceConvNormAdd.apply(x3, conv.weight2d(), conv.bias, z, sums, nw, nb, norm.eps, group, count)
    return y.view(B, conv.out_channels, H, W)


class _PceMLP(torch.autograd.Function):

    @staticmethod
    def forward(ctx, x3, w1, b1, w2, b2, apply_b2, want_row_sums, keep_pre=True):
        from . import ops
        if keep_pre:
            h, pre = ops.pce_gemm(x3, ops.pce_pack(w1), w1.shape[0], bias=b1, want_pre=True, gelu=True)
        else:
            h, pre = ops.pce_gemm(x3, ops.pce_pack(w1), w1.shape[0], bias=b1, gelu=True), x3.new_empty(0)
        want_row_sums = bool(want_row_sums) and w2.shape[0] <= 768
        y = ops.pce_gemm(h, ops.pce_pack(w2), w2.shape[0], bias=b2 if (apply_b2 and b2 is not None) else None,
                         want_row_sums=want_row_sums)
        y, sums = y if want_row_sums else (y, x3.new_empty(0, dtype=torch.float64))
        ctx.save_for_backward(x3, w1, w2, pre, h)
        ctx.cfg = (None if b1 is None else b1.dtype, None if b2 is None else (b2.dtype, tuple(b2.shape)), bool(apply_b2))
        ctx.step = _step_items(w1) + _step_items(w2)
        ctx.mark_non_differentiable(sums)
        return y, sums

    @staticmethod
    def backward(ctx, gy, _gsums):
        from . import ops
        x3, w1, w2, pre, h = ctx.saved_tensors
        b1_dtype, b2_info, apply_b2 = ctx.cfg
        gy = gy.contiguous()
        need_gb1 = b1_dtype is not None and ctx.needs_input_grad[2]
        fused_gb1 = need_gb1 and w2.shape[1] <= 768
        (w1img_t, g1buf, w2img_t, g2buf), ctx.step = (ctx.step or (None, None, None, None)), None
        gpre = ops.pce_gemm(gy, w2img_t if w2img_t is not None else ops.pce_pack(w2, transpose=True), w2.shape[1], aux_in=pre,
                            want_row_sums=fused_gb1)
        if fused_gb1:
            gpre, gsum = gpre
        gx = gw1 = gb1 = gw2 = gb2 = None
        if ctx.needs_input_grad[0]:
            gx = ops.pce_gemm(gpre, w1img_t if w1img_t is not None else ops.pce_pack(w1, transpose=True), w1.shape[1])
        if ctx.needs_input_grad[1]:
            gw1 = ops.conv1x1_wgrad_raw(gpre, x3, out=g1buf).to(w1.dtype)
        if need_gb1:
            if fused_gb1:
                g1 = gsum.view(gy.shape[0], -1, 2)[..., 0]
                gb1 = (g1[0] if g1.shape[0] == 1 else g1.sum(0)).to(b1_dtype)
            else:
                gb1 = _row_sums(gpre).to(b1_dtype)
        if ctx.needs_input_grad[3]:
            gw2 = ops.conv1x1_wgrad_raw(gy, h, out=g2buf).to(w2.dtype)
        if b2_info is not None and ctx.needs_input_grad[4]:
            gb2 = _row_sums(gy).to(b2_info[0]) if apply_b2 else torch.zeros(b2_info[1], dtype=b2_info[0], device=gy.device)
        return gx, gw1, gb1, gw2, gb2, None, None, None


class _PceMLPFused(torch.autograd.Function):

    @staticmethod
    def forward(ctx, x3, w1, b1, w2, b2, apply_b2, want_row_sums):
        from . import ops
        out = ops.pce_mlp(x3, ops.pce_mlp_pack(w1, False, w2, False), 0, b1=b1,
                          b2=b2 if (apply_b2 and b2 is not None) else None, want_row_sums=bool(want_row_sums))
        y, pre = out[0], out[1]
        sums = out[2] if want_row_sums else x3.new_empty(0, dtype=torch.float64)
        ctx.save_for_backward(x3, w1, w2, pre)
        ctx.cfg = (None if b1 is None else b1.dtype, None if b2 is None else (b2.dtype, tuple(b2.shape)), bool(apply_b2))
        ctx.step = (ops.arena_grad_buffer(w1) if w1.requires_grad else None, ops.arena_grad_buffer(w2) if w2.requires_grad else None)
        ctx.mark_non_differentiable(sums)
        return y, sums

    @staticmethod
    def backward(ctx, gy, _gsums):
        from . import ops
        x3, w1, w2, pre = ctx.saved_tensors
        b1_dtype, b2_info, apply_b2 = ctx.cfg
        (g1buf, g2buf), ctx.step = (ctx.step or (None, None)), None
        gy = gy.contiguous()
        need_gb1 = b1_dtype is not None and ctx.needs_input_grad[2]
        out = ops.pce_mlp(gy, ops.pce_mlp_pack(w2, True, w1, True), 1, pre=pre, want_mid_sums=need_gb1)
        gx, gpre = out[0], out[1]
        gw1 = gb1 = gw2 = gb2 = None
        if ctx.needs_input_grad[1]:
            gw1 = ops.conv1x1_wgrad_raw(gpre, x3, out=g1buf).to(w1.dtype)
        if need_gb1:
            g1 = out[2].view(gy.shape[0], -1)
            gb1 = (g1[0] if g1.shape[0] == 1 else g1.sum(0)).to(b1_dtype)
# ... 314 lines not shown
```

makani_amd/ops.py:

```python
import ctypes
import math
import os

import numpy as np
import torch

from . import _lib

GRIDS = {"equiangular": 0, "legendre-gauss": 1}


def _stream():
    return torch.cuda.current_stream().cuda_stream


def _need_cuda(*tensors):
    for t in tensors:
        if not t.is_cuda:
            raise RuntimeError("makani_amd: the spectral ops run only on a HIP device (got a CPU tensor); "
                               "there is no CPU fallback")


def quadrature(grid, nlat):
    if grid not in GRIDS:
        raise ValueError(f"Unknown quadrature mode {grid}")
    lib = _lib.load()
    theta = np.empty(nlat, dtype=np.float64)
    w = np.empty(nlat, dtype=np.float64)
    _lib.check(lib.mk_quadrature(GRIDS[grid], nlat, theta.ctypes.data, w.ctypes.data), "mk_quadrature")
    return theta, w


def legendre_kpad(nlat):
    return _lib.load().mk_legendre_kpad(nlat)


def legendre_table(grid, nlat, lmax, mmax, with_quad_weights):
    if grid not in GRIDS:
        raise ValueError(f"Unknown quadrature mode {grid}")
    lib = _lib.load()
    kp = lib.mk_legendre_kpad(nlat)
    out = torch.empty(mmax, lmax, kp, dtype=torch.float32)
    _lib.check(lib.mk_legendre_table(GRIDS[grid], nlat, lmax, mmax, int(bool(with_quad_weights)), out.data_ptr()),
               "mk_legendre_table")
    return out


def fft_twiddles(nlon):
    lib = _lib.load()
    out = torch.empty(lib.mk_fft_twiddle_len(nlon), dtype=torch.float32)
    _lib.check(lib.mk_fft_twiddles(nlon, out.data_ptr()), "mk_fft_twiddles")
    return out


def rfft_raw(x, twiddles, mmax, s0, sm, sh, kmajor=False):
    _need_cuda(x, twiddles)
    assert x.dim() == 3 and x.is_contiguous()
    bc, k, n = x.shape
    if x.dtype == torch.float32:
        dt = 0
    elif x.dtype == torch.bfloat16:
        dt = 1
    else:
        raise TypeError(f"mk_rfft: unsupported dtype {x.dtype}")
    xf = torch.empty((k, mmax, bc) if kmajor else (mmax, k, bc), dtype=torch.complex64, device=x.device)
    _lib.check(_lib.load().mk_rfft_ex(x.data_ptr(), dt, xf.data_ptr(), twiddles.data_ptr(), bc, k, n, mmax,
                                      s0, sm, sh, int(bool(kmajor)), _stream()), "mk_rfft")
    return xf


def irfft_bf16_rows(nlon, mmax):
    return nlon in (480, 1440) and mmax <= 241


def irfft_sums_supported(nlon, mmax):
    return nlon in (480, 1440) and mmax <= 241 and os.environ.get("MK_FFT_LEGACY", "0") != "1" \
        and os.environ.get("MK_IRFFT_SUMS", "1") != "0"


def irfft_sums_raw(xf, twiddles, nlon, out_dtype, kmajor=False, chans=0, cpp=0):
    _need_cuda(xf, twiddles)
    assert xf.is_contiguous() and xf.dtype == torch.complex64 and out_dtype in (torch.float32, torch.bfloat16)
    if cpp:
        p, k, m, bcp = xf.shape
        bc = (bcp // cpp) * chans
    elif kmajor:
        k, m, bc = xf.shape
    else:
        m, k, bc = xf.shape
    x = torch.empty(bc, k, nlon, dtype=out_dtype, device=xf.device)
    sums = torch.zeros(bc, 2, dtype=torch.float64, device=xf.device)
    _lib.check(_lib.load().mk_irfft_sums(xf.data_ptr(), x.data_ptr(), 1 if out_dtype == torch.bfloat16 else 0, twiddles.data_ptr(),
                                         bc, k, nlon, m, 1.0, 1.0, 1.0, int(bool(kmajor)), int(chans), int(cpp), sums.data_ptr(),
                                         _stream()), "mk_irfft_sums")
    return x, sums


def irfft_raw(xf, twiddles, nlon, s0, sm, sh, out_dtype=torch.float32, kmajor=False):
    _need_cuda(xf, twiddles)
    assert xf.dim() == 3 and xf.is_contiguous() and xf.dtype == torch.complex64
    if kmajor:
        k, m, bc = xf.shape
    else:
        m, k, bc = xf.shape
    fused = out_dtype == torch.bfloat16 and irfft_bf16_rows(nlon, m)
    x = torch.empty(bc, k, nlon, dtype=torch.bfloat16 if fused else torch.float32, device=xf.device)
    _lib.check(_lib.load().mk_irfft_ex(xf.data_ptr(), x.data_ptr(), 1 if fused else 0, twiddles.data_ptr(), bc, k, nlon, m,
                                       s0, sm, sh, int(bool(kmajor)), _stream()), "mk_irfft")
    return x if x.dtype == out_dtype else x.to(out_dtype)


def fft_pm_supported(nlon, mmax, chans, chans_per_peer):
    return (irfft_bf16_rows(nlon, mmax) and chans_per_peer > 0 and chans % chans_per_peer == 0 and chans_per_peer % 24 == 0
            and os.environ.get("MK_FFT_LEGACY") != "1")


def rfft_pm_raw(x, twiddles, mmax, s0, sm, sh, chans, chans_per_peer):
    _need_cuda(x, twiddles)
    assert x.dim() == 3 and x.is_contiguous() and x.dtype in (torch.float32, torch.bfloat16)
    bc, k, n = x.shape
    xf = torch.empty(chans // chans_per_peer, k, mmax, (bc // chans) * chans_per_peer, dtype=torch.complex64, device=x.device)
    _lib.check(_lib.load().mk_rfft_pm(x.data_ptr(), 0 if x.dtype == torch.float32 else 1, xf.data_ptr(), twiddles.data_ptr(),
                                      bc, k, n, mmax, s0, sm, sh, chans, chans_per_peer, _stream()), "mk_rfft_pm")
    return xf


def irfft_pm_raw(xf, twiddles, nlon, s0, sm, sh, chans, chans_per_peer, out_dtype=torch.float32):
    _need_cuda(xf, twiddles)
    assert xf.dim() == 4 and xf.is_contiguous() and xf.dtype == torch.complex64
    p, k, m, bcp = xf.shape
    bc = (bcp // chans_per_peer) * chans
    fused = out_dtype == torch.bfloat16
    x = torch.empty(bc, k, nlon, dtype=torch.bfloat16 if fused else torch.float32, device=xf.device)
    _lib.check(_lib.load().mk_irfft_pm(xf.data_ptr(), x.data_ptr(), 1 if fused else 0, twiddles.data_ptr(), bc, k, nlon, m,
                                       s0, sm, sh, chans, chans_per_peer, _stream()), "mk_irfft_pm")
    return x if x.dtype == out_dtype else x.to(out_dtype)


SPECTRAL_GEMM = os.environ.get("MK_SPECTRAL_GEMM", "bf16x3")


def _gemm_mode(mode):
    mode = mode or SPECTRAL_GEMM
    if mode not in ("bf16x3", "f32"):
        raise ValueError(f"unknown spectral GEMM mode {mode!r} (bf16x3 | f32)")
    return mode


def legendre_x3_image(table, nlat, inverse):
    _need_cuda(table)
    cache = table.__dict__.setdefault("_mk_x3", {})
    key = (int(nlat), int(bool(inverse)))
    entry = cache.get(key)
    if entry is None:
        lib = _lib.load()
        mg, lmax, kp = table.shape
        assert kp == legendre_kpad(nlat) and table.is_contiguous() and table.dtype == torch.float32
        nbytes = lib.mk_legendre_x3_bytes(nlat, lmax, mg, key[1])
        img = torch.empty(nbytes, dtype=torch.uint8, device=table.device)
        _lib.check(lib.mk_legendre_x3_split(table.data_ptr(), img.data_ptr(), nlat, lmax, mg, key[1], _stream()),
                   "mk_legendre_x3_split")
        ev = torch.cuda.Event()
        ev.record()
        cache[key] = entry = [img, ev]
        return img
    if entry[1] is not None:
        if torch.cuda.is_current_stream_capturing():
            return entry[0]
        elif entry[1].query():
            entry[1] = None
        else:
            torch.cuda.current_stream().wait_event(entry[1])
    return entry[0]


def legendre_fwd_raw(xf, table, lmax, m_off=0, mode=None, kmajor=False):
    _need_cuda(xf, table)
    assert xf.is_contiguous() and xf.dtype == torch.complex64 and table.dtype == torch.float32
# ... 463 lines not shown
            x, sums = irfft_sums_raw(xf, twiddles, nlon, out_dtype, True, chans, cpp)
            ctx.mark_non_differentiable(sums)
            return x, sums
        return irfft_pm_raw(xf, twiddles, nlon, 1.0, 1.0, 1.0, chans, cpp, out_dtype)

    @staticmethod
    def backward(ctx, gx, *_):
        (tw,) = ctx.saved_tensors
        mmax, chans, cpp = ctx.cfg
        if gx.dtype not in (torch.float32, torch.bfloat16):
            gx = gx.float()
        return rfft_pm_raw(gx.contiguous(), tw, mmax, 1.0, 2.0, 1.0, chans, cpp), None, None, None, None, None, None


class _LegendreFwd(torch.autograd.Function):

    @staticmethod
    def forward(ctx, xf, table, lmax, m_off, kmajor=False):
        ctx.table = table
        ctx.nlat, ctx.m_off, ctx.kmajor = xf.shape[0] if kmajor else xf.shape[1], m_off, kmajor
        return legendre_fwd_raw(xf, table, lmax, m_off, kmajor=kmajor)

    @staticmethod
    def backward(ctx, gc):
        return legendre_inv_raw(gc.contiguous(), ctx.table, ctx.nlat, ctx.m_off, kmajor=ctx.kmajor), None, None, None, None


class _LegendreInv(torch.autograd.Function):

    @staticmethod
    def forward(ctx, c, table, nlat, m_off, kmajor=False):
        ctx.table = table
        ctx.lmax, ctx.m_off, ctx.kmajor = c.shape[0], m_off, kmajor
        return legendre_inv_raw(c, table, nlat, m_off, kmajor=kmajor)

    @staticmethod
    def backward(ctx, gxf):
        return legendre_fwd_raw(gxf.contiguous(), ctx.table, ctx.lmax, ctx.m_off, kmajor=ctx.kmajor), None, None, None, None


class _SpecPack(torch.autograd.Function):
    @staticmethod
    def forward(ctx, c_std, l_off, m_off):
        ctx.offs = (l_off, m_off)
        return spec_pack_raw(c_std)

    @staticmethod
    def backward(ctx, g):
        return spec_unpack_raw(g.contiguous(), *ctx.offs), None, None


class _SpecUnpack(torch.autograd.Function):
    @staticmethod
    def forward(ctx, c_prv, l_off, m_off):
        return spec_unpack_raw(c_prv, l_off, m_off)

    @staticmethod
    def backward(ctx, g):
        return spec_pack_raw(g.contiguous()), None, None


class _Dhconv(torch.autograd.Function):

    @staticmethod
    def forward(ctx, x, w, batch, l_off, m_off):
        wp = _w_phys(w)
        ctx.save_for_backward(x, wp)
        ctx.args = (batch, l_off, m_off)
        return dhconv_fwd_raw(x, wp, batch, l_off, m_off)

    @staticmethod
    def backward(ctx, gy):
        x, wp = ctx.saved_tensors
        batch, l_off, m_off = ctx.args
        gy = gy.contiguous()
        gx = gw = None
        if ctx.needs_input_grad[0]:
            gx = dhconv_dgrad_raw(gy, wp, batch, l_off, m_off)
        if ctx.needs_input_grad[1]:
            gw = dhconv_wgrad_raw(x, gy, batch, l_off, m_off).permute(1, 2, 0)
        return gx, gw, None, None, None


def rfft(x, twiddles, mmax, kmajor=False):
    return _RFFT.apply(x, twiddles, mmax, kmajor)


def irfft(xf, twiddles, nlon, out_dtype=torch.float32, kmajor=False, want_sums=False):
    return _IRFFT.apply(xf, twiddles, nlon, out_dtype, kmajor, want_sums)


def rfft_pm(x, twiddles, mmax, chans, cpp):
    return _RFFTpm.apply(x, twiddles, mmax, chans, cpp)


def irfft_pm(xf, twiddles, nlon, out_dtype, chans, cpp, want_sums=False):
    return _IRFFTpm.apply(xf, twiddles, nlon, out_dtype, chans, cpp, want_sums)


def legendre_fwd(xf, table, lmax, m_off=0, kmajor=False):
    return _LegendreFwd.apply(xf, table, lmax, m_off, kmajor)


def legendre_inv(c, table, nlat, m_off=0, kmajor=False):
    return _LegendreInv.apply(c, table, nlat, m_off, kmajor)


def spec_pack(c_std, l_off=0, m_off=0):
    return _SpecPack.apply(c_std, l_off, m_off)


def spec_unpack(c_prv, l_off=0, m_off=0):
    return _SpecUnpack.apply(c_prv, l_off, m_off)


def dhconv(x, w, batch, l_off=0, m_off=0):
    return _Dhconv.apply(x, w, batch, l_off, m_off)


def _pw_dtype(t):
    if t.dtype == torch.float32:
        return 0
    if t.dtype == torch.bfloat16:
        return 1
    raise TypeError(f"makani_amd pointwise ops: unsupported dtype {t.dtype}")


def pointwise_supported(x):
    return (x.is_cuda and x.dim() == 4 and x.is_contiguous() and x.dtype in (torch.float32, torch.bfloat16)
            and (x.shape[2] * x.shape[3]) % 8 == 0 and x.shape[0] * x.shape[1] <= 65535)


class _BiasGelu(torch.autograd.Function):

    @staticmethod
    def forward(ctx, x, bias):
        _need_cuda(x)
        B, C, H, W = x.shape
        y = torch.empty_like(x)
        bf = None if bias is None else bias.detach().float().contiguous()
        _lib.check(_lib.load().mk_bias_gelu_fwd(x.data_ptr(), 0 if bf is None else bf.data_ptr(), y.data_ptr(),
                                                _pw_dtype(x), B * C, C, H * W, _stream()), "mk_bias_gelu_fwd")
        ctx.save_for_backward(x, bf if bf is not None else x.new_empty(0))
        ctx.has_bias = bias is not None
        ctx.bias_dtype = None if bias is None else bias.dtype
        return y

    @staticmethod
    def backward(ctx, gy):
        x, bf = ctx.saved_tensors
        B, C, H, W = x.shape
        gy = gy.contiguous()
        gx = torch.empty_like(x)
        gb = torch.zeros(C, dtype=torch.float32, device=x.device) if ctx.has_bias else None
        _lib.check(_lib.load().mk_bias_gelu_bwd(x.data_ptr(), bf.data_ptr() if ctx.has_bias else 0, gy.data_ptr(),
                                                gx.data_ptr(), 0 if gb is None else gb.data_ptr(), _pw_dtype(x),
                                                B * C, C, H * W, _stream()), "mk_bias_gelu_bwd")
        return gx, (gb.to(ctx.bias_dtype) if gb is not None else None)


class _InstanceNorm(torch.autograd.Function):

    @staticmethod
    def forward(ctx, x, weight, bias, eps, fuse_gelu, group, count, sums=None):
        _need_cuda(x)
        B, C, H, W = x.shape
# ... 47 lines not shown
                                          wf.data_ptr() if wf is not None else 0, bf.data_ptr() if bf is not None else 0,
                                          gx.data_ptr(), ws.data_ptr(), _pw_dtype(x), B * C, C, H * W, cnt, int(fuse_gelu),
                                          phase, _stream()), "mk_instnorm_bwd_ex")
    if group is None and B == 1 and grad_dtype == torch.float32 and wf is not None and bf is not None:
        out = torch.empty(2, C, dtype=torch.float32, device=x.device)
        _lib.check(lib.mk_instnorm_bwd_wb(x.data_ptr(), gy.data_ptr(), stats.data_ptr(), wf.data_ptr(), bf.data_ptr(),
                                          gx.data_ptr(), ws.data_ptr(), out.data_ptr(), _pw_dtype(x), C, H * W, int(fuse_gelu),
                                          _stream()), "mk_instnorm_bwd_wb")
        return gx, out[0], out[1]
    if group is None:
        run(0)
        local = ws
    else:
        run(1)
        local = ws.clone()
        torch.distributed.all_reduce(ws, group=group)
        run(2)
    sums = local.view(B, C, 2)
    sums = sums[0] if B == 1 else sums.sum(0)
    if grad_dtype is not None:
        out = torch.empty(2, C, dtype=grad_dtype, device=x.device)
        out.copy_(sums.t())
        return gx, out[1], out[0]
    return gx, sums[:, 1], sums[:, 0]


def instance_norm_coeffs(sums, weight, bias, rows, channels, count, eps):
    _need_cuda(sums)
    assert sums.dtype == torch.float64 and sums.is_contiguous() and sums.numel() == 2 * rows
    stats = torch.empty(rows, 2, dtype=torch.float32, device=sums.device)
    affine = torch.empty(rows, 2, dtype=torch.float32, device=sums.device)
    _lib.check(_lib.load().mk_instnorm_coeffs(sums.data_ptr(), 0 if weight is None else weight.data_ptr(),
                                              0 if bias is None else bias.data_ptr(), stats.data_ptr(), affine.data_ptr(),
                                              rows, channels, int(count), float(eps), _stream()), "mk_instnorm_coeffs")
    return stats, affine


class _WeightedMSE(torch.autograd.Function):

    @staticmethod
    def forward(ctx, pred, tar, wrow, scale):
        _need_cuda(pred, tar, wrow)
        B, C, H, W = pred.shape
        loss = torch.empty(1, dtype=torch.float64, device=pred.device)
        _lib.check(_lib.load().mk_wmse_fwd(pred.data_ptr(), _pw_dtype(pred), tar.data_ptr(), wrow.data_ptr(), loss.data_ptr(),
                                           B * C * H, H, W, float(scale), _stream()), "mk_wmse_fwd")
        ctx.save_for_backward(pred, tar, wrow)
        ctx.scale = float(scale)
        return loss.float().squeeze(0)

    @staticmethod
    def backward(ctx, g):
        pred, tar, wrow = ctx.saved_tensors
        B, C, H, W = pred.shape
        gp = torch.empty_like(pred)
        g32 = g.detach().float().reshape(1).contiguous()
        _lib.check(_lib.load().mk_wmse_bwd(pred.data_ptr(), _pw_dtype(pred), tar.data_ptr(), wrow.data_ptr(), g32.data_ptr(),
                                           gp.data_ptr(), B * C * H, H, W, ctx.scale, _stream()), "mk_wmse_bwd")
        return gp, None, None, None


def weighted_mse(pred, tar, wrow, scale=1.0):
    if not (pred.is_cuda and pred.is_contiguous() and tar.is_contiguous() and tar.dtype == torch.float32
            and pred.dtype in (torch.float32, torch.bfloat16) and pred.shape[-1] % 8 == 0):
        w = wrow.view(1, 1, -1, 1)
        return scale * (((pred.float() - tar) ** 2) * w).sum()
    return _WeightedMSE.apply(pred, tar, wrow.float().contiguous(), scale)


def row_sums(t3):
    _need_cuda(t3)
    assert t3.dim() == 3 and t3.is_contiguous()
    b, c, p = t3.shape
    if os.environ.get("MK_ROWSUM") == "torch":
        return torch.sum(t3, dim=-1, dtype=torch.float32).view(-1)
    ws = torch.empty(b * c, 2, dtype=torch.float64, device=t3.device)
    _lib.check(_lib.load().mk_instnorm_fwd_ex(t3.data_ptr(), 0, 0, 0, 0, ws.data_ptr(), _pw_dtype(t3), b * c, c, p, p, 0.0, 0,
                                              1, _stream()), "mk_instnorm_fwd_ex")
    return ws[:, 0].float()


def bias_gelu(x, bias):
    return _BiasGelu.apply(x, bias)


def instance_norm(x, weight, bias, eps=1e-5, fuse_gelu=False, group=None, count=None, row_sums=None):
    return _InstanceNorm.apply(x, weight, bias, eps, fuse_gelu, group, count, row_sums)


GEO_METRIC_SUMS = ("l1", "sq", "cov", "var_p", "var_t")


@torch.no_grad()
def geo_metric_sums(prd, tar, clim, wrow):
    if prd.dim() != 4 or tar.shape != prd.shape:
        raise ValueError(f"geo_metric_sums: prediction {tuple(prd.shape)} and target {tuple(tar.shape)} must be equal [B, C, H, W]")
    B, C, H, W = prd.shape
    if wrow.numel() != H:
        raise ValueError(f"geo_metric_sums: wrow has {wrow.numel()} weights for {H} latitude rows")
    if clim is not None and tuple(clim.shape[-3:]) != (C, H, W):
        raise ValueError(f"geo_metric_sums: climatology {tuple(clim.shape)} does not match [C, H, W] = {(C, H, W)}")
    if not prd.is_cuda:
        p, t = prd.double(), tar.double()
        w = wrow.double().reshape(1, 1, H, 1)
        c = clim.double().reshape(1, C, H, W) if clim is not None else torch.zeros((), dtype=torch.float64)
        d, pa, ta = p - t, p - c, t - c
        return torch.stack([(w * d.abs()).sum((-2, -1)), (w * d * d).sum((-2, -1)), (w * pa * ta).sum((-2, -1)),
                            (w * pa * pa).sum((-2, -1)), (w * ta * ta).sum((-2, -1))], dim=-1)
    _need_cuda(prd, tar, wrow, *([clim] if clim is not None else []))
    if prd.dtype not in (torch.float32, torch.bfloat16):
        prd = prd.float()
    prd = prd.contiguous()
    tar = tar.float().contiguous()
    wrow = wrow.float().contiguous()
    clim = clim.float().contiguous() if clim is not None else None
    lib = _lib.load()
    ws = torch.empty(lib.mk_geo_metric_workspace(B, C, H), dtype=torch.float64, device=prd.device)
    out = torch.empty(B, C, 5, dtype=torch.float64, device=prd.device)
    _lib.check(lib.mk_geo_metric_sums(prd.data_ptr(), _pw_dtype(prd), tar.data_ptr(), clim.data_ptr() if clim is not None else None,
                                      wrow.data_ptr(), ws.data_ptr(), out.data_ptr(), B, C, H, W, _stream()), "mk_geo_metric_sums")
    return out


def _geo_lp_sums_torch(prd, tar, wrow, p):
    w = wrow.double().reshape(1, 1, -1, 1)
    d, t = prd.double() - tar.double(), tar.double()
    if p == 2:
        return torch.stack([(w * d * d).sum((-2, -1)), (w * t * t).sum((-2, -1))], dim=-1)
    return torch.stack([(w * d.abs()).sum((-2, -1)), (w * t.abs()).sum((-2, -1))], dim=-1)


class _GeoLpSums(torch.autograd.Function):

    @staticmethod
    def forward(ctx, prd, tar, wrow, p):
        B, C, H, W = prd.shape
        lib = _lib.load()
        ws = torch.empty(lib.mk_geo_lp_workspace(B, C, H), dtype=torch.float64, device=prd.device)
        out = torch.empty(B, C, 2, dtype=torch.float64, device=prd.device)
        _lib.check(lib.mk_geo_lp_sums(prd.data_ptr(), _pw_dtype(prd), tar.data_ptr(), wrow.data_ptr(), ws.data_ptr(),
                                      out.data_ptr(), p, B, C, H, W, _stream()), "mk_geo_lp_sums")
        ctx.save_for_backward(prd, tar, wrow)
        ctx.p = p
        return out

    @staticmethod
    @torch.autograd.function.once_differentiable
    def backward(ctx, g):
        prd, tar, wrow = ctx.saved_tensors
        B, C, H, W = prd.shape
        gp = torch.empty_like(prd)
        g0 = g[..., 0].float().contiguous()
        _lib.check(_lib.load().mk_geo_lp_bwd(prd.data_ptr(), _pw_dtype(prd), tar.data_ptr(), wrow.data_ptr(), g0.data_ptr(),
                                             gp.data_ptr(), ctx.p, B, C, H, W, _stream()), "mk_geo_lp_bwd")
        return gp, None, None, None


def geo_lp_sums(prd, tar, wrow, p):
    if p not in (1, 2):
        raise ValueError(f"geo_lp_sums: p must be 1 or 2, got {p}")
    if prd.dim() != 4 or tar.shape != prd.shape:
        raise ValueError(f"geo_lp_sums: prediction {tuple(prd.shape)} and target {tuple(tar.shape)} must be equal [B, C, H, W]")
    if wrow.numel() != prd.shape[-2]:
        raise ValueError(f"geo_lp_sums: wrow has {wrow.numel()} weights for {prd.shape[-2]} latitude rows")
    if not prd.is_cuda or tar.requires_grad:
        return _geo_lp_sums_torch(prd, tar, wrow, int(p))
# ... 99 lines not shown
```

makani_amd/sfnonet.py:

```python
import math
import os
from functools import partial

import torch
import torch.nn as nn
import torch.nn.functional as F
from torch.utils.checkpoint import checkpoint

from . import comm
from .distributed import DistributedInverseRealFFT2, DistributedInverseRealSHT, DistributedRealFFT2, DistributedRealSHT
from .layer_norm import DistributedInstanceNorm2d, DistributedLayerNorm
from .layers import (Conv1x1, DropPath, EncoderDecoder, InstanceNorm2d, InverseRealFFT2, MLP, RealFFT2, _engine_field,
                     _is_exact_gelu, conv_plus_instance_norm)
from .sht import InverseRealSHT, RealSHT
from .spectral_convolution import FactorizedSpectralConv, SpectralAttention, SpectralConv

_ACTIVATIONS = {"relu": nn.ReLU, "gelu": nn.GELU, "silu": nn.SiLU}


def _local_shape(transform):
    if comm.get_size("spatial") > 1:
        return transform.lat_shapes[comm.get_rank("h")], transform.lon_shapes[comm.get_rank("w")]
    return transform.nlat, transform.nlon


def _make_skip(kind, embed_dim, gain):
    if kind in ("none", None):
        return None, gain
    if kind == "identity":
        return nn.Identity(), gain / 2.0
    if kind == "linear":
        conv = Conv1x1(embed_dim, embed_dim, bias=False)
        nn.init.normal_(conv.weight, std=math.sqrt(gain / 2.0 / embed_dim))
        return conv, gain / 2.0
    raise ValueError(f"Unknown skip connection type {kind}")


class SpectralFilterLayer(nn.Module):
    def __init__(self, forward_transform, inverse_transform, embed_dim, filter_type="linear", operator_type="diagonal",
                 hidden_size_factor=1, factorization=None, rank=1.0, separable=False, complex_activation="real",
                 spectral_layers=1, bias=False, drop_rate=0.0, gain=1.0):
        super().__init__()
        common = dict(operator_type=operator_type, separable=separable, bias=bias, gain=gain)
        if filter_type == "non-linear":
            self.filter = SpectralAttention(forward_transform, inverse_transform, embed_dim, embed_dim, operator_type=operator_type,
                                            hidden_size_factor=hidden_size_factor, complex_activation=complex_activation,
                                            spectral_layers=spectral_layers, drop_rate=drop_rate, bias=bias, gain=gain)
        elif filter_type != "linear":
            raise NotImplementedError
        elif factorization is None:
            self.filter = SpectralConv(forward_transform, inverse_transform, embed_dim, embed_dim, **common)
        else:
            self.filter = FactorizedSpectralConv(forward_transform, inverse_transform, embed_dim, embed_dim, rank=rank,
                                                 factorization=factorization, **common)

    def forward(self, x, want_row_sums=False):
        if want_row_sums and isinstance(self.filter, SpectralConv) and type(self.filter).forward is SpectralConv.forward:
            return self.filter(x, want_row_sums=True)
        out = self.filter(x)
        return (out[0], out[1], None) if want_row_sums else out


class FourierNeuralOperatorBlock(nn.Module):

    def __init__(self, forward_transform, inverse_transform, embed_dim, filter_type="linear", operator_type="diagonal",
                 mlp_ratio=2.0, mlp_drop_rate=0.0, path_drop_rate=0.0, act_layer=nn.GELU,
                 norm_layer=(nn.Identity, nn.Identity), rank=1.0, factorization=None, separable=False,
                 inner_skip="linear", outer_skip=None, use_mlp=False, comm_feature_inp_name=None,
                 comm_feature_hidden_name=None, complex_activation="real", spectral_layers=1, bias=False,
                 final_activation=False, checkpointing=0):
        super().__init__()
        self.input_shape_loc = _local_shape(forward_transform)
        self.output_shape_loc = _local_shape(inverse_transform)
        has_act = act_layer != nn.Identity

        self.norm0 = norm_layer[0]()
        skip, filter_gain = _make_skip(inner_skip, embed_dim, 2.0 if has_act else 1.0)
        if skip is not None:
            self.inner_skip = skip
        self.filter = SpectralFilterLayer(forward_transform, inverse_transform, embed_dim, filter_type, operator_type,
                                          hidden_size_factor=mlp_ratio, factorization=factorization, rank=rank,
                                          separable=separable, complex_activation=complex_activation,
                                          spectral_layers=spectral_layers, bias=bias, drop_rate=path_drop_rate,
                                          gain=filter_gain)
        self.act_layer0 = act_layer()
        self.norm1 = norm_layer[1]()
        skip, mlp_gain = _make_skip(outer_skip, embed_dim, 2.0 if (final_activation and has_act) else 1.0)
        if skip is not None:
            self.outer_skip = skip
        if use_mlp == True:
            self.mlp = MLP(in_features=embed_dim, hidden_features=int(embed_dim * mlp_ratio), act_layer=act_layer,
                           drop_rate=mlp_drop_rate, drop_type="features", comm_inp_name=comm_feature_inp_name,
                           comm_hidden_name=comm_feature_hidden_name, checkpointing=checkpointing, gain=mlp_gain)
        self.drop_path = DropPath(path_drop_rate) if path_drop_rate > 0.0 else nn.Identity()
        if final_activation:
            self.act_layer1 = act_layer()

    @staticmethod
    def _removes_channel_constants(norm):
        return (isinstance(norm, (nn.InstanceNorm2d, DistributedInstanceNorm2d))
                and not getattr(norm, "track_running_stats", False))

    def forward(self, x):
        inner = getattr(self, "inner_skip", None)
        hip_norm0 = isinstance(self.norm0, (InstanceNorm2d, DistributedInstanceNorm2d)) \
            and not getattr(self.norm0, "track_running_stats", False)
        sums0 = None
        if hip_norm0 and isinstance(self.filter, SpectralFilterLayer):
            x, residual, sums0 = self.filter(x, want_row_sums=True)
        else:
            x, residual = self.filter(x)
        if inner is None and hip_norm0 and _is_exact_gelu(self.act_layer0):
            x = self.norm0(x, fuse_gelu=True, row_sums=sums0)
        elif hip_norm0:
            x = self.norm0(x, row_sums=sums0)
            if inner is not None:
                x = x + inner(residual)
            x = self.act_layer0(x)
        else:
            x = self.norm0(x)
            if inner is not None:
                x = x + inner(residual)
            x = self.act_layer0(x)
        sums = None
        if hasattr(self, "mlp"):
            if isinstance(self.norm1, (InstanceNorm2d, DistributedInstanceNorm2d)):
                x, sums = self.mlp(x, skip_last_bias=self._removes_channel_constants(self.norm1), want_row_sums=True)
            else:
                x = self.mlp(x, skip_last_bias=self._removes_channel_constants(self.norm1))
        outer = getattr(self, "outer_skip", None)
        if sums is not None and isinstance(self.drop_path, nn.Identity) and not hasattr(self, "act_layer1"):
            y = conv_plus_instance_norm(outer, residual, x, sums, self.norm1)
            if y is not None:
                return y
        x = self.drop_path(self.norm1(x, row_sums=sums) if sums is not None else self.norm1(x))
        if isinstance(outer, Conv1x1):
            x = outer(residual, addend=x)
        elif outer is not None:
            x = x + outer(residual)
        if hasattr(self, "act_layer1"):
            x = self.act_layer1(x)
        return x


class SphericalFourierNeuralOperatorNet(nn.Module):

    def __init__(self, spectral_transform="sht", model_grid_type="equiangular", sht_grid_type="legendre-gauss",
                 filter_type="linear", operator_type="dhconv", inp_shape=(721, 1440), out_shape=(721, 1440),
                 scale_factor=8, inp_chans=2, out_chans=2, embed_dim=32, num_layers=4, repeat_layers=1, use_mlp=True,
                 mlp_ratio=2.0, encoder_ratio=1, decoder_ratio=1, activation_function="gelu", encoder_layers=1,
                 pos_embed="none", pos_drop_rate=0.0, path_drop_rate=0.0, mlp_drop_rate=0.0,
                 normalization_layer="instance_norm", max_modes=None, hard_thresholding_fraction=1.0, big_skip=True,
                 rank=1.0, factorization=None, separable=False, complex_activation="real", spectral_layers=3,
                 bias=False, checkpointing=0, **kwargs):
        super().__init__()
        if comm.get_size("matmul") > 1:
            raise NotImplementedError("channel ('matmul', fin/fout) parallelism is outside the built hot path")
        if activation_function not in _ACTIVATIONS:
            raise ValueError(f"Unknown activation function {activation_function}")
        act = _ACTIVATIONS[activation_function]

        self.inp_shape, self.out_shape = tuple(inp_shape), tuple(out_shape)
        self.inp_chans, self.out_chans, self.embed_dim = inp_chans, out_chans, embed_dim
        self.repeat_layers, self.big_skip, self.checkpointing = repeat_layers, big_skip, checkpointing
        self.h, self.w = int(self.inp_shape[0] // scale_factor), int(self.inp_shape[1] // scale_factor)

        self._init_spectral_transforms(spectral_transform, model_grid_type, sht_grid_type, hard_thresholding_fraction, max_modes)

        self.encoder = EncoderDecoder(num_layers=encoder_layers, input_dim=inp_chans, output_dim=embed_dim,
                                      hidden_dim=int(encoder_ratio * embed_dim), act_layer=act, input_format="nchw")
        self.pos_drop = nn.Dropout(p=pos_drop_rate) if pos_drop_rate > 0.0 else nn.Identity()

        norm = self._norm_factory(normalization_layer, embed_dim)
        drop_rates = torch.linspace(0, path_drop_rate, num_layers).tolist()
        self.blocks = nn.ModuleList()
        for i, drop in enumerate(drop_rates):
            self.blocks.append(FourierNeuralOperatorBlock(
                self.trans_down if i == 0 else self.trans,
                self.itrans_up if i == num_layers - 1 else self.itrans,
                embed_dim, filter_type=filter_type, operator_type=operator_type, mlp_ratio=mlp_ratio,
                mlp_drop_rate=mlp_drop_rate, path_drop_rate=drop, act_layer=act, norm_layer=(norm, norm),
                inner_skip="none", outer_skip="linear", use_mlp=use_mlp, comm_feature_inp_name="fin",
                comm_feature_hidden_name="fout", rank=rank, factorization=factorization, separable=separable,
                complex_activation=complex_activation, spectral_layers=spectral_layers, bias=bias,
                checkpointing=checkpointing))

        self.decoder = EncoderDecoder(num_layers=encoder_layers, input_dim=embed_dim, output_dim=out_chans,
                                      hidden_dim=int(decoder_ratio * embed_dim), act_layer=act,
                                      gain=0.5 if big_skip else 1.0, input_format="nchw")
        if big_skip:
            self.residual_transform = Conv1x1(inp_chans, out_chans, bias=False)
            self.residual_transform.weight.is_shared_mp = ["spatial"]
            self.residual_transform.weight.sharded_dims_mp = [None, None, None, None]
            nn.init.normal_(self.residual_transform.weight, mean=0.0, std=math.sqrt(0.5 / inp_chans))
        self._init_pos_embed(pos_embed)

    @staticmethod
    def _norm_factory(kind, embed_dim):
        if kind == "instance_norm":
            if comm.get_size("spatial") > 1:
                return partial(DistributedInstanceNorm2d, num_features=embed_dim, eps=1e-6, affine=True)
            return partial(InstanceNorm2d, num_features=embed_dim, eps=1e-6, affine=True, track_running_stats=False)
        if kind == "none":
            return nn.Identity
        if kind == "layer_norm":
            return partial(DistributedLayerNorm, normalized_shape=(embed_dim), elementwise_affine=True, eps=1e-6)
        raise NotImplementedError(f"Error, normalization {kind} not implemented.")

    def _init_spectral_transforms(self, spectral_transform="sht", model_grid_type="equiangular",
                                  sht_grid_type="legendre-gauss", hard_thresholding_fraction=1.0, max_modes=None):
        if max_modes is not None:
            modes = dict(lmax=max_modes[0], mmax=max_modes[1])
        else:
            modes = dict(lmax=int(self.h * hard_thresholding_fraction),
                         mmax=int((self.w // 2 + 1) * hard_thresholding_fraction))
        distributed = comm.get_size("spatial") > 1
        if spectral_transform == "sht":
            fwd, inv = (DistributedRealSHT, DistributedInverseRealSHT) if distributed else (RealSHT, InverseRealSHT)
            outer, inner = dict(grid=model_grid_type, **modes), dict(grid=sht_grid_type, **modes)
        elif spectral_transform == "fft":
            fwd, inv = (DistributedRealFFT2, DistributedInverseRealFFT2) if distributed else (RealFFT2, InverseRealFFT2)
            outer = inner = modes
        else:
            raise ValueError("Unknown spectral transform")
        self.trans_down = fwd(*self.inp_shape, **outer).float()
        self.itrans_up = inv(*self.out_shape, **outer).float()
        self.trans = fwd(self.h, self.w, **inner).float()
        self.itrans = inv(self.h, self.w, **inner).float()
        self.inp_shape_loc = _local_shape(self.trans_down)
        self.out_shape_loc = _local_shape(self.itrans_up)
        self.h_loc, self.w_loc = _local_shape(self.itrans)

    def _init_pos_embed(self, kind):
        if kind in ("none", "None", None):
            return
        if kind == "direct":
            self.pos_embed = nn.Parameter(torch.zeros(1, self.embed_dim, *self.inp_shape_loc))
            nn.init.trunc_normal_(self.pos_embed, std=0.02)
        elif kind == "frequency":
            if comm.get_size("spatial") > 1:
                lloc, mloc = self.itrans_up.l_shapes[comm.get_rank("h")], self.itrans_up.m_shapes[comm.get_rank("w")]
            else:
                lloc, mloc = self.itrans_up.lmax, self.itrans_up.mmax
            re = nn.Parameter(torch.tril(torch.randn(1, self.embed_dim, lloc, mloc), diagonal=0))
            im = nn.Parameter(torch.tril(torch.randn(1, self.embed_dim, lloc, mloc - 1), diagonal=-1))
            for t in (re, im):
                nn.init.trunc_normal_(t, std=0.02)
            self.pos_embed = nn.ParameterList([re, im])
        else:
            raise ValueError("Unknown position embedding type")
        self.pos_embed.type = kind
        self.pos_embed.is_shared_mp = []
        self.pos_embed.sharded_dims_mp = [None, None, "h", "w"]

    def no_weight_decay(self):
        return {"pos_embed", "cls_token"}

    def _position_field(self, like):
        if self.pos_embed.type == "direct":
            return self.pos_embed
        re, im = self.pos_embed
        coeffs = torch.complex(re, F.pad(im, (1, 0)))
        with torch.autocast(device_type=like.device.type, enabled=False):
            return self.itrans_up(coeffs)

    def _big_skip_input(self, x):
        if self.out_shape == self.inp_shape:
            return x
        with torch.autocast(device_type=x.device.type, enabled=False):
            return self.itrans_up(self.trans_down(x.float()).contiguous()).to(x.dtype)

    def _forward_features(self, x):
        for _ in range(self.repeat_layers):
            for blk in self.blocks:
                x = checkpoint(blk, x, use_reentrant=False) if self.checkpointing >= 3 else blk(x)
        return x

    def _engine_arena(self, x):
        from . import ops
        from .layers import Conv1x1
        if not (x.is_cuda and x.dim() == 4 and os.environ.get("MK_ENGINE_ARENA", "1") != "0"):
            return None
        if not (x.dtype == torch.bfloat16 or (torch.is_autocast_enabled() and torch.get_autocast_dtype("cuda") == torch.bfloat16)):
            return None
        cached = self.__dict__.get("_arena")
        if cached is None:
            convs = [m for m in self.modules() if isinstance(m, Conv1x1)]
        else:
            convs = cached[0]
        ptrs = [m.weight.data_ptr() for m in convs]
        if cached is None or cached[1] != ptrs:
            cached = (convs, ptrs, ops.EngineArena([m.weight2d() for m in convs if m.weight.is_cuda]))
            self.__dict__["_arena"] = cached
        return cached[2] if cached[2].n else None

    def forward(self, x):
        arena = self._engine_arena(x)
        if arena is None:
            return self._forward(x)
        with arena.scope():
            return self._forward(x)

    def _forward(self, x):
        if self.big_skip and self.out_shape == self.inp_shape and x.dtype == torch.float32 and x.dim() == 4:
            x3 = _engine_field(x)
            if x3 is not None and x3.dtype != x.dtype:
                x = x3.view(x.shape)
        skip_in = self._big_skip_input(x) if self.big_skip else None
        x = checkpoint(self.encoder, x, use_reentrant=False) if self.checkpointing >= 1 else self.encoder(x)
        if hasattr(self, "pos_embed"):
            x = x + self._position_field(x)
        x = self._forward_features(self.pos_drop(x))
        x = checkpoint(self.decoder, x, use_reentrant=False) if self.checkpointing >= 1 else self.decoder(x)
        if skip_in is not None:
            x = self.residual_transform(skip_in, addend=x)
        return x


class FourierNeuralOperatorNet(SphericalFourierNeuralOperatorNet):
    def __init__(self, *args, **kwargs):
        super().__init__(*args, spectral_transform="fft", **kwargs)
```

makani_amd/spectral_convolution.py:

```python
import math

import torch
import torch.nn as nn

from . import comm, ops
from .contractions import get_contract_fun
from .distributed import DistributedInverseRealFFT2, DistributedInverseRealSHT, DistributedRealSHT
from .sht import InverseRealSHT, RealSHT


def _is_hip_pair(fwd, inv):
    return isinstance(fwd, (RealSHT, DistributedRealSHT)) and isinstance(inv, (InverseRealSHT, DistributedInverseRealSHT))


class SpectralConv(nn.Module):
    def __init__(self, forward_transform, inverse_transform, in_channels, out_channels, operator_type="diagonal",
                 separable=False, bias=False, gain=1.0):
        super().__init__()
        self.forward_transform = forward_transform
        self.inverse_transform = inverse_transform
        self.in_channels = in_channels
        self.out_channels = out_channels
        self.modes_lat = self.inverse_transform.lmax
        self.modes_lon = self.inverse_transform.mmax
        self.scale_residual = (self.forward_transform.nlat != self.inverse_transform.nlat) or \
                              (self.forward_transform.nlon != self.inverse_transform.nlon)
        if hasattr(self.forward_transform, "grid"):
            self.scale_residual = self.scale_residual or (self.forward_transform.grid != self.inverse_transform.grid)
        self.operator_type = operator_type
        self.separable = separable
        assert self.inverse_transform.lmax == self.modes_lat
        assert self.inverse_transform.mmax == self.modes_lon

        weight_shape = [in_channels]
        if not self.separable:
            weight_shape += [out_channels]

        self._distributed = isinstance(self.inverse_transform, (DistributedInverseRealSHT, DistributedInverseRealFFT2))
        if self._distributed:
            hr, wr = comm.get_rank("h"), comm.get_rank("w")
            self.modes_lat_local = self.inverse_transform.l_shapes[hr]
            self.modes_lon_local = self.inverse_transform.m_shapes[wr]
            self.nlat_local = self.inverse_transform.lat_shapes[hr]
            self.nlon_local = self.inverse_transform.lon_shapes[wr]
            self.l_off = sum(self.inverse_transform.l_shapes[:hr])
            self.m_off = sum(self.inverse_transform.m_shapes[:wr])
        else:
            self.modes_lat_local = self.modes_lat
            self.modes_lon_local = self.modes_lon
            self.nlat_local = self.inverse_transform.nlat
            self.nlon_local = self.inverse_transform.nlon
            self.l_off, self.m_off = 0, 0

        if self.operator_type == "diagonal":
            weight_shape += [self.modes_lat_local, self.modes_lon_local]
        elif self.operator_type == "dhconv":
            weight_shape += [self.modes_lat_local]
        else:
            raise ValueError(f"Unsupported operator type f{self.operator_type}")

        scale = math.sqrt(gain / in_channels) * torch.ones(self.modes_lat_local, dtype=torch.complex64)
        scale[0] *= math.sqrt(2.0)
        init = scale * torch.randn(*weight_shape, dtype=torch.complex64)
        if self.operator_type == "dhconv" and not self.separable:
            phys = init.permute(2, 0, 1).contiguous()
            self.weight = nn.Parameter(phys.permute(1, 2, 0))
        else:
            self.weight = nn.Parameter(init)

        if self.operator_type == "dhconv":
            self.weight.is_shared_mp = ["matmul", "w"]
            self.weight.sharded_dims_mp = [None for _ in weight_shape]
            self.weight.sharded_dims_mp[-1] = "h"
        else:
            self.weight.is_shared_mp = ["matmul"]
            self.weight.sharded_dims_mp = [None for _ in weight_shape]
            self.weight.sharded_dims_mp[-1] = "w"
            self.weight.sharded_dims_mp[-2] = "h"

        self._contract = get_contract_fun(self.weight, implementation="factorized", separable=separable,
                                          complex=True, operator_type=operator_type)
        self._fused = _is_hip_pair(forward_transform, inverse_transform) and operator_type == "dhconv" and not separable

        if bias == "constant":
            self.bias = nn.Parameter(torch.zeros(1, self.out_channels, 1, 1))
        elif bias == "position":
            self.bias = nn.Parameter(torch.zeros(1, self.out_channels, self.nlat_local, self.nlon_local))
            self.bias.is_shared_mp = ["matmul"]
            self.bias.sharded_dims_mp = [None, None, "h", "w"]

    def _weight_tensor(self):
        return self.weight

    def _forward_fused(self, x, dtype, want_row_sums=False):
        B, C = x.shape[0], x.shape[1]
        ft, it = self.forward_transform, self.inverse_transform
        xin = x if x.dtype in (torch.float32, torch.bfloat16) else x.float()
        xin = xin.contiguous()
        if isinstance(ft, DistributedRealSHT):
            c = ft.forward_packed(xin)
        else:
            c = ft.forward_packed(xin.view(B * C, xin.shape[2], xin.shape[3]))
        odt = dtype if dtype in (torch.float32, torch.bfloat16) else torch.float32
        residual = x
        if self.scale_residual:
            r = it.inverse_packed(c, B, odt) if self._distributed else it.inverse_packed(c, odt)
            residual = r.view(B, C, r.shape[-2], r.shape[-1]).to(dtype)
        y = ops.dhconv(c, self._weight_tensor(), B, self.l_off, self.m_off)
        sums = None
        if want_row_sums:
            out, sums = it.inverse_packed(y, B, odt, True) if self._distributed else it.inverse_packed(y, odt, True)
        else:
            out = it.inverse_packed(y, B, odt) if self._distributed else it.inverse_packed(y, odt)
        out = out.view(B, self.out_channels, out.shape[-2], out.shape[-1])
        return out, residual, sums

    def forward(self, x, want_row_sums=False):
        dtype = x.dtype
        residual = x
        sums = None
        if self._fused and x.is_cuda and x.dim() == 4:
            with torch.autocast(device_type="cuda", enabled=False):
                x, residual, sums = self._forward_fused(x, dtype, want_row_sums and not hasattr(self, "bias"))
            if sums is not None and x.dtype != dtype:
                sums = None
        else:
            x = x.float()
            with torch.autocast(device_type=x.device.type, enabled=False):
                x = self.forward_transform(x).contiguous()
                if self.scale_residual:
                    residual = self.inverse_transform(x)
                    residual = residual.to(dtype)
            xp = self._contract(x, self._weight_tensor(), separable=self.separable, operator_type=self.operator_type)
            x = xp.contiguous()
            with torch.autocast(device_type=x.device.type, enabled=False):
                x = self.inverse_transform(x)
        if hasattr(self, "bias"):
            x = x + self.bias
        x = x.to(dtype=dtype)
        return (x, residual, sums) if want_row_sums else (x, residual)


class _DenseFactorizedWeight(nn.Module):

    def __init__(self, shape, complex=True):
        super().__init__()
        dtype = torch.complex64 if complex else torch.float32
        self.shape = tuple(shape)
        self.name = "ComplexDense" if complex else "Dense"
        self.tensor = nn.Parameter(torch.empty(*shape, dtype=dtype))

    def normal_(self, mean=0.0, std=1.0):
        with torch.no_grad():
            if self.tensor.is_complex():
                self.tensor.copy_(mean + std * torch.randn(self.shape, dtype=torch.complex64))
            else:
                self.tensor.normal_(mean, std)
        return self

    def to_tensor(self):
        return self.tensor


class FactorizedSpectralConv(SpectralConv):

    def __init__(self, forward_transform, inverse_transform, in_channels, out_channels, operator_type="diagonal",
                 rank=0.2, factorization=None, separable=False, decomposition_kwargs=dict(), bias=False, gain=1.0):
        super().__init__(forward_transform, inverse_transform, in_channels, out_channels, operator_type=operator_type,
                         separable=separable, bias=bias, gain=gain)
        if factorization is None:
            factorization = "ComplexDense"
        complex_weight = factorization[:7].lower() == "complex"
        if factorization.lower() not in ("complexdense", "dense"):
            raise NotImplementedError(f"factorization {factorization} needs tensorly-torch (absent); "
                                      "only the dense factorization is built")
        self.rank = rank
        self.factorization = factorization
        shape = tuple(self.weight.shape)
        ann = (self.weight.is_shared_mp, self.weight.sharded_dims_mp)
        del self.weight
        self.weight = _DenseFactorizedWeight(shape, complex=complex_weight)
        scale = math.sqrt(gain / float(shape[0]))
        self.weight.normal_(mean=0.0, std=scale)
        self.weight.tensor.is_shared_mp, self.weight.tensor.sharded_dims_mp = ann
        self._complex_weight = complex_weight
        self._contract = get_contract_fun(self.weight, implementation="reconstructed", separable=separable,
                                          complex=complex_weight, operator_type=operator_type)
        self._fused = self._fused and complex_weight

    def _weight_tensor(self):
        return self.weight.to_tensor()

    def forward(self, x):
        if self._complex_weight:
            return super().forward(x)
        dtype = x.dtype
        residual = x
        x = x.float()
        with torch.autocast(device_type=x.device.type, enabled=False):
            x = self.forward_transform(x).contiguous()
            if self.scale_residual:
                residual = self.inverse_transform(x).to(dtype)
        x = torch.view_as_real(x)
        xp = self._contract(x, self.weight, separable=self.separable, operator_type=self.operator_type)
        x = torch.view_as_complex(xp.contiguous())
        with torch.autocast(device_type="cuda" if x.is_cuda else "cpu", enabled=False):
# ... 91 lines not shown
```

Before: 23.64 samples/s.

## Move encoder channel mixing and outer skip into spectral domain

Applies the first block's encoder linear projection as a spectral-domain channel mix (new spec_mix GEMM kernels) on the forward SHT output, rather than on the full grid. The outer skip is kept as spectral coefficients and synthesised later, with an irfft epilogue that fuses the affine scale, shift and add. The aim is to drop full-resolution encoder and residual passes and extra elementwise kernels. This adds new kernels and conditional paths whose correctness depends on linearity and matching conditions.

```diff
diff --git a/include/makani_amd.h b/include/makani_amd.h
--- a/include/makani_amd.h
+++ b/include/makani_amd.h
@@ -58,6 +58,9 @@
 int mk_irfft_sums(const float* xf, void* x, int x_dtype, const float* twiddles, int bc, int nlat, int nlon, int mmax,
                   float scale0, float scale_m, float scale_h, int xf_layout, int chans, int chans_per_peer, double* rowsums,
                   void* stream);
+int mk_irfft_affine_add(const float* xf, void* x, int x_dtype, const float* twiddles, int bc, int nlat, int nlon,
+                        int mmax, float scale0, float scale_m, float scale_h, int xf_layout, const void* z,
+                        const float* affine, void* stream);
 
 int mk_dhconv_fwd(const float* x, const float* w, float* y, int lloc, int mloc, int batch,
                   int cin, int cout, int l_off, int m_off, void* stream);
@@ -73,6 +76,13 @@
 int mk_dhconv_wgrad_x3(const float* x, const float* gy, float* gw, int lloc, int mloc, int batch,
                        int cin, int cout, int l_off, int m_off, void* stream);
 
+int mk_spec_mix_fwd(const float* x, const float* w, float* y, int lloc, int mloc, int batch,
+                    int cin, int cout, int l_off, int m_off, void* stream);
+int mk_spec_mix_dgrad(const float* gy, const float* w, float* gx, int lloc, int mloc, int batch,
+                      int cin, int cout, int l_off, int m_off, void* stream);
+int mk_spec_mix_wgrad(const float* x, const float* gy, float* gw, int lloc, int mloc, int batch,
+                      int cin, int cout, int l_off, int m_off, void* stream);
+
 int mk_diag_fwd(const float* x, const float* w, float* y, int batch, int cin, int cout, long long P, void* stream);
 int mk_diag_dgrad(const float* gy, const float* w, float* gx, int batch, int cin, int cout, long long P, void* stream);
 int mk_diag_wgrad(const float* x, const float* gy, float* gw, int batch, int cin, int cout, long long P, void* stream);
@@ -85,6 +95,8 @@
                      void* stream);
 int mk_bias_gelu_bwd(const void* x, const float* bias, const void* gy, void* gx, float* gbias, int dtype,
                      int rows, int C, long long P, void* stream);
+int mk_affine_add(const void* r, const void* z, const float* affine, void* y, int dtype, int rows, long long P,
+                  void* stream);
 int mk_instnorm_fwd(const void* x, const float* weight, const float* bias, void* y, float* stats,
                     double* workspace, int dtype, int rows, int C, long long P, float eps, int fuse_gelu,
                     void* stream);
diff --git a/makani_amd/_lib.py b/makani_amd/_lib.py
--- a/makani_amd/_lib.py
+++ b/makani_amd/_lib.py
@@ -33,6 +33,8 @@
     "mk_irfft_pm": (_c_int, [_vp, _vp, _c_int, _vp, _c_int, _c_int, _c_int, _c_int, _c_float, _c_float, _c_float, _c_int, _c_int, _vp]),
     "mk_irfft_sums": (_c_int, [_vp, _vp, _c_int, _vp, _c_int, _c_int, _c_int, _c_int, _c_float, _c_float, _c_float, _c_int, _c_int,
                                _c_int, _vp, _vp]),
+    "mk_irfft_affine_add": (_c_int, [_vp, _vp, _c_int, _vp, _c_int, _c_int, _c_int, _c_int, _c_float, _c_float, _c_float, _c_int,
+                                     _vp, _vp, _vp]),
     "mk_legendre_fwd_x3_ex": (_c_int, [_vp, _vp, _vp, _c_int, _c_int, _c_int, _c_int, _c_int, _c_int, _c_int, _vp]),
     "mk_legendre_inv_x3_ex": (_c_int, [_vp, _vp, _vp, _c_int, _c_int, _c_int, _c_int, _c_int, _c_int, _c_int, _vp]),
     "mk_dhconv_fwd": (_c_int, [_vp, _vp, _vp] + [_c_int] * 7 + [_vp]),
@@ -41,6 +43,10 @@
     "mk_dhconv_fwd_x3": (_c_int, [_vp, _vp, _vp] + [_c_int] * 7 + [_vp]),
     "mk_dhconv_dgrad_x3": (_c_int, [_vp, _vp, _vp] + [_c_int] * 7 + [_vp]),
     "mk_dhconv_wgrad_x3": (_c_int, [_vp, _vp, _vp] + [_c_int] * 7 + [_vp]),
+    "mk_spec_mix_fwd": (_c_int, [_vp, _vp, _vp] + [_c_int] * 7 + [_vp]),
+    "mk_spec_mix_dgrad": (_c_int, [_vp, _vp, _vp] + [_c_int] * 7 + [_vp]),
+    "mk_spec_mix_wgrad": (_c_int, [_vp, _vp, _vp] + [_c_int] * 7 + [_vp]),
+    "mk_affine_add": (_c_int, [_vp, _vp, _vp, _vp, _c_int, _c_int, ctypes.c_longlong, _vp]),
     "mk_diag_fwd": (_c_int, [_vp, _vp, _vp, _c_int, _c_int, _c_int, ctypes.c_longlong, _vp]),
     "mk_diag_dgrad": (_c_int, [_vp, _vp, _vp, _c_int, _c_int, _c_int, ctypes.c_longlong, _vp]),
     "mk_diag_wgrad": (_c_int, [_vp, _vp, _vp, _c_int, _c_int, _c_int, ctypes.c_longlong, _vp]),
diff --git a/makani_amd/csrc/fft.hip b/makani_amd/csrc/fft.hip
--- a/makani_amd/csrc/fft.hip
+++ b/makani_amd/csrc/fft.hip
@@ -2,6 +2,7 @@
 #include "../../include/makani_amd.h"
 
 #include <hip/hip_bf16.h>
+#include <cstdint>
 #include <cstdlib>
 #include <type_traits>
 #include <utility>
@@ -14,6 +15,8 @@
     long long pstride;
 };
 static thread_local XfLayout g_xl = {0, 0, 0, 0, 0, 0};
+static thread_local const void* g_addz = nullptr;
+static thread_local const float* g_affine = nullptr;
 static thread_local double* g_rowsums = nullptr;
 
 struct XfChan {
@@ -583,3 +586,19 @@
     g_rowsums = nullptr;
     return rc;
 }
+
+extern "C" int mk_irfft_affine_add(const float* xf, void* x, int x_dtype, const float* twiddles, int bc, int nlat, int nlon,
+                                   int mmax, float scale0, float scale_m, float scale_h, int xf_layout, const void* z,
+                                   const float* affine, void* stream) {
+    MK_REQUIRE(z != nullptr && affine != nullptr, "null pointer");
+    MK_REQUIRE(!fft_legacy() && mmax <= 241 && (nlon == 480 || nlon == 1440), "the affine-add epilogue exists in the split kernels only");
+    MK_REQUIRE((((uintptr_t)z | (uintptr_t)x) & 15) == 0, "fields must be 16-byte aligned");
+    MK_REQUIRE(xf_layout == 0 || xf_layout == 1, "xf_layout must be 0 ([M][K][BC]) or 1 ([K][M][BC])");
+    MK_REQUIRE((240LL * (xf_layout ? 1 : nlat) + 1) * bc * 8 < (1LL << 31), "Fourier rows too large for the 32-bit gather offsets");
+    g_addz = z;
+    g_affine = affine;
+    const int rc = mk_irfft_ex(xf, x, x_dtype, twiddles, bc, nlat, nlon, mmax, scale0, scale_m, scale_h, xf_layout, stream);
+    g_addz = nullptr;
+    g_affine = nullptr;
+    return rc;
+}
diff --git a/makani_amd/csrc/fft_split.h b/makani_amd/csrc/fft_split.h
--- a/makani_amd/csrc/fft_split.h
+++ b/makani_amd/csrc/fft_split.h
@@ -217,12 +217,25 @@
 template <typename T> struct OutVec;
 template <> struct OutVec<float> {
     static constexpr int E = 4;
+    static __device__ __forceinline__ void load(const float* p, float (&o)[4]) {
+        const float4 v = *reinterpret_cast<const float4*>(p);
+        o[0] = v.x; o[1] = v.y; o[2] = v.z; o[3] = v.w;
+    }
     static __device__ __forceinline__ void store(float* p, const float (&o)[4]) {
         *reinterpret_cast<float4*>(p) = make_float4(o[0], o[1], o[2], o[3]);
     }
 };
 template <> struct OutVec<__hip_bfloat16> {
     static constexpr int E = 8;
+    static __device__ __forceinline__ void load(const __hip_bfloat16* p, float (&o)[8]) {
+        const uint4 u = *reinterpret_cast<const uint4*>(p);
+        const unsigned int w[4] = {u.x, u.y, u.z, u.w};
+#pragma unroll
+        for (int i = 0; i < 4; ++i) {
+            o[2 * i] = __uint_as_float(w[i] << 16);
+            o[2 * i + 1] = __uint_as_float(w[i] & 0xffff0000u);
+        }
+    }
     static __device__ __forceinline__ void store(__hip_bfloat16* p, const float (&o)[8]) {
         __hip_bfloat16 h[8];
 #pragma unroll
@@ -231,11 +244,12 @@
     }
 };
 
-template <int S, typename TOut, bool WIDE, int PERSIST, bool SUMS = false>
+template <int S, typename TOut, bool WIDE, int PERSIST, bool SUMS = false, bool ADD = false>
 __global__ __launch_bounds__(STHREADS, PERSIST ? 3 : 5) void irfft_split_kernel(const float2* __restrict__ xf, TOut* __restrict__ x,
                                                                const float2* __restrict__ tw, int BC, int K, int M,
                                                                float scale0, float scale_m, float scale_h, XfLayout xl,
-                                                               double* __restrict__ rowsums) {
+                                                               double* __restrict__ rowsums, const TOut* __restrict__ addz,
+                                                               const float* __restrict__ affine) {
     constexpr int N = 480 * S, G = SNSUB / S, HH = N / 2;
     extern __shared__ __attribute__((aligned(16))) float2 lds[];
     float* red = reinterpret_cast<float*>(lds + SLDS_F2);
@@ -377,7 +391,16 @@
                     r[sq][2 * h + 1] = -z.y;
                 }
             }
-            TOut* dst = x + ((size_t)(bc0 + g) * K + k) * N + (size_t)p * EO * S;
+            const size_t doff = ((size_t)(bc0 + g) * K + k) * N + (size_t)p * EO * S;
+            TOut* dst = x + doff;
+            float za[S][EO];
+            float ca = 0.f, cb = 0.f;
+            if constexpr (ADD) {
+                ca = affine[2 * (bc0 + g)];
+                cb = affine[2 * (bc0 + g) + 1];
+#pragma unroll
+                for (int c = 0; c < S; ++c) OutVec<TOut>::load(addz + doff + c * EO, za[c]);
+            }
 #pragma unroll
             for (int c = 0; c < S; ++c) {
                 float o[EO];
@@ -385,6 +408,7 @@
                 for (int e = 0; e < EO; ++e) {
                     const int f = c * EO + e;
                     o[e] = r[f % S][f / S];
+                    if constexpr (ADD) o[e] += fmaf(za[c][e], ca, cb);
                 }
                 OutVec<TOut>::store(dst + c * EO, o);
             }
@@ -429,9 +453,14 @@
     const bool wide = ((long long)SH * g_xl.sm + 1) * bcx * 8 >= (1LL << 31);
 #define MK_IRFFT_LAUNCH(T, W, PS, SM)                                                                                  \
     hipLaunchKernelGGL((irfft_split_kernel<S, T, W, PS, SM>), grid, dim3(STHREADS), lds, st, (const float2*)xf, (T*)x,    \
-                       (const float2*)tw, bc, nlat, mmax, s0, sm, sh, g_xl, g_rowsums)
+                       (const float2*)tw, bc, nlat, mmax, s0, sm, sh, g_xl, g_rowsums, (const T*)nullptr, (const float*)nullptr)
 #define MK_IRFFT_PICK(T)                                                                                               \
-    if (g_rowsums) {                                                                                                   \
+    if (g_addz) {                                                                                                      \
+        if (wide) return -1;                                                                                           \
+        hipLaunchKernelGGL((irfft_split_kernel<S, T, false, 0, false, true>), grid, dim3(STHREADS), lds, st,           \
+                           (const float2*)xf, (T*)x, (const float2*)tw, bc, nlat, mmax, s0, sm, sh, g_xl, nullptr,     \
+                           (const T*)g_addz, g_affine);                                                                \
+    } else if (g_rowsums) {                                                                                                   \
         if (wide) MK_IRFFT_LAUNCH(T, true, 1, true); else MK_IRFFT_LAUNCH(T, false, 0, true);                          \
     } else {                                                                                                           \
         if (wide) MK_IRFFT_LAUNCH(T, true, 1, false); else MK_IRFFT_LAUNCH(T, false, 0, false);                        \
diff --git a/makani_amd/csrc/gemm_x3.hip b/makani_amd/csrc/gemm_x3.hip
--- a/makani_amd/csrc/gemm_x3.hip
+++ b/makani_amd/csrc/gemm_x3.hip
@@ -353,6 +353,26 @@
         }
     }
     const int col = wc * 64 + 2 * fi;
+    if constexpr (EPI == 4) {
+        if (col < cvalid) {
+#pragma unroll
+            for (int a = 0; a < 2; ++a)
+#pragma unroll
+                for (int r = 0; r < 16; r += 2) {
+                    const int row = wr * 64 + a * 32 + (r & 3) + 8 * (r >> 2) + 4 * kg;
+                    if (row < rvalid) {
+                        typedef float x3_f4 __attribute__((ext_vector_type(4)));
+                        x3_f4 v4;
+                        v4[0] = acc[a][0][r];
+                        v4[1] = acc[a][0][r + 1];
+                        v4[2] = acc[a][1][r];
+                        v4[3] = acc[a][1][r + 1];
+                        __builtin_nontemporal_store(v4, reinterpret_cast<x3_f4*>(cbase + (long long)(row >> 1) * ldc + 2 * col));
+                    }
+                }
+        }
+        return;
+    }
     if (col < cvalid) {
 #pragma unroll
         for (int a = 0; a < 2; ++a)
@@ -714,6 +734,227 @@
     const long long nblk = grid_blocks(lloc, p.tiles_m, p.tiles_n);
     MK_REQUIRE(nblk < 2147483647LL, "grid too large");
     hipLaunchKernelGGL(dhconv_wgrad_x3_kernel, dim3((unsigned)nblk), dim3(XT), X3_LDS, (hipStream_t)stream, p);
+    MK_LAUNCH_CHECK();
+    return 0;
+}
+
+namespace {
+
+struct MixParams {
+    const float* a;
+    const float* w;
+    float* dst;
+    int Lloc, Mloc, B, Ca, Cd;
+    int l_off, m_off, tiles_m, tiles_n;
+    int G, ngroups;
+};
+
+__device__ __forceinline__ int mix_rows(int Mloc, int B, int l_off, int m_off, int l) {
+    int nm = l_off + l - m_off + 1;
+    nm = nm < 0 ? 0 : (nm > Mloc ? Mloc : nm);
+    return nm * B;
+}
+
+struct SpecRowStager {
+    const float* base;
+    long long ld;
+    int rows, cvalid;
+    typedef float4 Regs[4];
+    static __device__ __forceinline__ int row_off(int r) { return pair_off(r); }
+    __device__ __forceinline__ void gload(int kt, Regs& r, int tid) const {
+        const __amdgpu_buffer_rsrc_t rs = x3_rsrc(base);
+        const int row = (tid >> 6) * 16 + quad_row(tid & 63), i = kt * XK + (tid & 3) * 8;
+        const unsigned off = (unsigned)(((long long)row * ld + 2 * i) * 4);
+#pragma unroll
+        for (int h = 0; h < 4; ++h) r[h] = x3_load16(rs, (row < rows && i + 2 * h < cvalid) ? off + 16 * h : X3_OOB);
+    }
+    __device__ __forceinline__ void sstore(const Regs& r, char* img, int tid) const {
+        const int row = (tid >> 6) * 16 + quad_row(tid & 63), c = tid & 3;
+        const float re[8] = {r[0].x, r[0].z, r[1].x, r[1].z, r[2].x, r[2].z, r[3].x, r[3].z};
+        const float im[8] = {r[0].y, r[0].w, r[1].y, r[1].w, r[2].y, r[2].w, r[3].y, r[3].w};
+        if (row < rows) {
+            split_store8(re, img + row * XPITCH + c * 16);
+            split_store8(im, img + (row + 64) * XPITCH + 128 + c * 16);
+        }
+    }
+};
+
+struct Row2Stager {
+    const float* base;
+    long long ld;
+    int rows, kvalid;
+    typedef float2 Regs[8];
+    static __device__ __forceinline__ int row_off(int r) { return pair_off(r); }
+    __device__ __forceinline__ void gload(int kt, Regs& r, int tid) const {
+        const __amdgpu_buffer_rsrc_t rs = x3_rsrc(base);
+#pragma unroll
+        for (int q = 0; q < 2; ++q) {
+            const int t = tid + q * XT, row = (t >> 6) * 16 + quad_row(t & 63), k = kt * XK + (t & 3) * 8;
+            const unsigned off = (unsigned)(((long long)row * ld + k) * 4);
+#pragma unroll
+            for (int h = 0; h < 4; ++h)
+                r[4 * q + h] = x3_load8(rs, (row < rows && k + 2 * h < kvalid) ? off + 8 * h : X3_OOB);
+        }
+    }
+    __device__ __forceinline__ void sstore(const Regs& r, char* img, int tid) const {
+#pragma unroll
+        for (int q = 0; q < 2; ++q) {
+            const int t = tid + q * XT, row = (t >> 6) * 16 + quad_row(t & 63);
+            const float v[8] = {r[4 * q].x, r[4 * q].y, r[4 * q + 1].x, r[4 * q + 1].y,
+                                r[4 * q + 2].x, r[4 * q + 2].y, r[4 * q + 3].x, r[4 * q + 3].y};
+            if (row < rows) split_store8(v, img + pair_off(row) + (t & 3) * 16);
+        }
+    }
+};
+
+template <bool PAIR>
+struct MixKStager {
+    const float* base;
+    long long C;
+    long long lpitch;
+    int l0, KPL, cvalid;
+    int Mloc, B, l_off, m_off;
+    typedef float2 Regs[8];
+    static __device__ __forceinline__ int row_off(int r) { return PAIR ? pair_off(r) : plain_off(r); }
+    __device__ __forceinline__ void gload(int kt, Regs& r, int tid) const {
+        const int w = __builtin_amdgcn_readfirstlane(tid >> 6), t = tid & 63;
+        const int li = kt / KPL, l = l0 + li;
+        const int r0 = (kt - li * KPL) * (XK / 2) + w * 4;
+        const int R = mix_rows(Mloc, B, l_off, m_off, l);
+        const __amdgpu_buffer_rsrc_t rs = x3_rsrc(base + (long long)l * lpitch);
+#pragma unroll
+        for (int e = 0; e < 2; ++e) {
+            const int c = t + 64 * e;
+            const bool cok = c < cvalid;
+#pragma unroll
+            for (int j = 0; j < 4; ++j)
+                r[4 * e + j] = x3_load8(rs, (cok && r0 + j < R) ? (unsigned)((((long long)(r0 + j)) * C + c) * 8) : X3_OOB);
+        }
+    }
+    __device__ __forceinline__ void sstore(const Regs& r, char* img, int tid) const {
+        const int w = tid >> 6, t = tid & 63;
+#pragma unroll
+        for (int e = 0; e < 2; ++e) {
+            const float v[8] = {r[4 * e].x, r[4 * e].y, r[4 * e + 1].x, r[4 * e + 1].y,
+                                r[4 * e + 2].x, r[4 * e + 2].y, r[4 * e + 3].x, r[4 * e + 3].y};
+            split_store8(v, img + row_off(t + 64 * e) + w * 16);
+        }
+    }
+};
+
+template <bool TRANS>
+__global__ __launch_bounds__(XT, 3) void spec_mix_x3_kernel(MixParams p) {
+    extern __shared__ __attribute__((aligned(16))) char lds_x3[];
+    const TileId t = decode_block(p.Lloc, p.tiles_m, p.tiles_n);
+    if (!t.valid) return;
+    const int l = p.Lloc - 1 - t.batch;
+    const int R = mix_rows(p.Mloc, p.B, p.l_off, p.m_off, l);
+    const int r0 = t.tm * (XM / 2);
+    if (r0 >= R) return;
+    const int n0 = t.tn * XN;
+    const long long rowbase = (long long)l * p.Mloc * p.B + r0;
+    SpecRowStager as;
+    as.base = p.a + rowbase * 2 * p.Ca;
+    as.ld = 2LL * p.Ca;
+    as.rows = R - r0;
+    as.cvalid = p.Ca;
+    float* cb = p.dst + rowbase * 2 * p.Cd + 2 * n0;
+    const int kts = (p.Ca + XK - 1) / XK;
+    if constexpr (TRANS) {
+        TransStager bs;
+        bs.base = p.w + n0;
+        bs.ldk = p.Cd;
+        bs.k_lo = 0;
+        bs.k_hi = p.Ca;
+        bs.cvalid = p.Cd - n0;
+        x3_tile<X3_DB, SpecRowStager, TransStager, 4>(as, bs, 0, kts, 2 * (R - r0), p.Cd - n0, cb, 2LL * p.Cd, lds_x3);
+    } else {
+        Row2Stager bs;
+        bs.base = p.w + (long long)n0 * p.Ca;
+        bs.ld = p.Ca;
+        bs.rows = p.Cd - n0;
+        bs.kvalid = p.Ca;
+        x3_tile<X3_DB, SpecRowStager, Row2Stager, 4>(as, bs, 0, kts, 2 * (R - r0), p.Cd - n0, cb, 2LL * p.Cd, lds_x3);
+    }
+}
+
+__global__ __launch_bounds__(XT, 3) void spec_mix_wgrad_x3_kernel(MixParams p) {
+    extern __shared__ __attribute__((aligned(16))) char lds_x3[];
+    const TileId t = decode_block(p.ngroups, p.tiles_m, p.tiles_n);
+    if (!t.valid) return;
+    const int g = p.ngroups - 1 - t.batch;
+    const int l0 = g * p.G, l1 = l0 + p.G < p.Lloc ? l0 + p.G : p.Lloc;
+    const int KPL = (mix_rows(p.Mloc, p.B, p.l_off, p.m_off, l1 - 1) + XK / 2 - 1) / (XK / 2);
+    if (KPL == 0) return;
+    const int o0 = t.tm * XM, i0 = t.tn * XN;
+    MixKStager<false> as;
+    as.base = p.a + 2 * o0;
+    as.C = p.Ca;
+    as.lpitch = 2LL * p.Mloc * p.B * p.Ca;
+    as.cvalid = p.Ca - o0;
+    MixKStager<true> bs;
+    bs.base = p.w + 2 * i0;
+    bs.C = p.Cd;
+    bs.lpitch = 2LL * p.Mloc * p.B * p.Cd;
+    bs.cvalid = p.Cd - i0;
+    as.l0 = bs.l0 = l0;
+    as.KPL = bs.KPL = KPL;
+    as.Mloc = bs.Mloc = p.Mloc;
+    as.B = bs.B = p.B;
+    as.l_off = bs.l_off = p.l_off;
+    as.m_off = bs.m_off = p.m_off;
+    x3_tile<X3_DB, MixKStager<false>, MixKStager<true>, 2>(as, bs, 0, (l1 - l0) * KPL, p.Ca - o0, p.Cd - i0,
+                                                            p.dst + (long long)o0 * p.Cd + i0, p.Cd, lds_x3);
+}
+
+}
+
+static int spec_mix_check(const void* a, const void* b, const void* c, int lloc, int mloc, int batch, int cin, int cout, int l_off,
+                          int m_off) {
+    MK_REQUIRE(a && b && c, "null pointer");
+    MK_REQUIRE(lloc > 0 && mloc > 0 && batch > 0 && cin > 0 && cout > 0, "bad sizes");
+    MK_REQUIRE(l_off >= 0 && m_off >= 0, "negative shard offset");
+    MK_REQUIRE(cin % 2 == 0 && cout % 2 == 0, "the spectral channel mix needs even channel counts");
+    MK_REQUIRE((((uintptr_t)a | (uintptr_t)b | (uintptr_t)c) & 15) == 0, "operands must be 16-byte aligned");
+    const long long cmax = cin > cout ? cin : cout;
+    MK_REQUIRE((long long)mloc * batch * cmax * 8 < (1LL << 31) && 33LL * cmax * 4 < (1LL << 31),
+               "one degree of the spectrum must stay below 2^31 bytes");
+    return 0;
+}
+
+static int spec_mix_launch(bool trans, const float* a, const float* w, float* dst, int lloc, int mloc, int batch, int ca, int cd,
+                           int l_off, int m_off, void* stream) {
+    MixParams p{a, w, dst, lloc, mloc, batch, ca, cd, l_off, m_off, mk::ceil_div(mloc * batch, XM / 2), mk::ceil_div(cd, XN), 1, 0};
+    const long long nblk = grid_blocks(lloc, p.tiles_m, p.tiles_n);
+    MK_REQUIRE(nblk < 2147483647LL, "grid too large");
+    if (trans) hipLaunchKernelGGL(spec_mix_x3_kernel<true>, dim3((unsigned)nblk), dim3(XT), X3_LDS, (hipStream_t)stream, p);
+    else hipLaunchKernelGGL(spec_mix_x3_kernel<false>, dim3((unsigned)nblk), dim3(XT), X3_LDS, (hipStream_t)stream, p);
+    MK_LAUNCH_CHECK();
+    return 0;
+}
+
+extern "C" int mk_spec_mix_fwd(const float* x, const float* w, float* y, int lloc, int mloc, int batch, int cin, int cout,
+                               int l_off, int m_off, void* stream) {
+    if (int e = spec_mix_check(x, w, y, lloc, mloc, batch, cin, cout, l_off, m_off)) return e;
+    return spec_mix_launch(false, x, w, y, lloc, mloc, batch, cin, cout, l_off, m_off, stream);
+}
+
+extern "C" int mk_spec_mix_dgrad(const float* gy, const float* w, float* gx, int lloc, int mloc, int batch, int cin, int cout,
+                                 int l_off, int m_off, void* stream) {
+    if (int e = spec_mix_check(gy, w, gx, lloc, mloc, batch, cin, cout, l_off, m_off)) return e;
+    return spec_mix_launch(true, gy, w, gx, lloc, mloc, batch, cout, cin, l_off, m_off, stream);
+}
+
+extern "C" int mk_spec_mix_wgrad(const float* x, const float* gy, float* gw, int lloc, int mloc, int batch, int cin, int cout,
+                                 int l_off, int m_off, void* stream) {
+    if (int e = spec_mix_check(x, gy, gw, lloc, mloc, batch, cin, cout, l_off, m_off)) return e;
+    MixParams p{gy, x, gw, lloc, mloc, batch, cout, cin, l_off, m_off, mk::ceil_div(cout, XM), mk::ceil_div(cin, XN), 1, 0};
+    long long G = (long long)lloc * p.tiles_m * p.tiles_n / 768;
+    p.G = (int)(G < 1 ? 1 : (G > 8 ? 8 : G));
+    p.ngroups = mk::ceil_div(lloc, p.G);
+    const long long nblk = grid_blocks(p.ngroups, p.tiles_m, p.tiles_n);
+    MK_REQUIRE(nblk < 2147483647LL, "grid too large");
+    hipLaunchKernelGGL(spec_mix_wgrad_x3_kernel, dim3((unsigned)nblk), dim3(XT), X3_LDS, (hipStream_t)stream, p);
     MK_LAUNCH_CHECK();
     return 0;
 }
diff --git a/makani_amd/csrc/pointwise.hip b/makani_amd/csrc/pointwise.hip
--- a/makani_amd/csrc/pointwise.hip
+++ b/makani_amd/csrc/pointwise.hip
@@ -153,6 +153,27 @@
 }
 
 template <typename T>
+__global__ __launch_bounds__(kT) void affine_add_kernel(const T* __restrict__ r, const T* __restrict__ z,
+                                                        const float* __restrict__ affine, T* __restrict__ y, long long P) {
+    const int row = blockIdx.y;
+    const float a = affine[2 * row], b = affine[2 * row + 1];
+    const long long ro = (long long)row * P;
+    for_chunk<T>(P, [&](long long off, int n) {
+        float v[kE], u[kE];
+        if (n == kE) {
+            IO<T>::load(r + ro + off, v);
+            IO<T>::load(z + ro + off, u);
+#pragma unroll
+            for (int i = 0; i < kE; ++i) v[i] += fmaf(u[i], a, b);
+            IO<T>::store(y + ro + off, v);
+        } else {
+            for (int i = 0; i < n; ++i)
+                IO<T>::st1(y + ro + off + i, IO<T>::ld1(r + ro + off + i) + fmaf(IO<T>::ld1(z + ro + off + i), a, b));
+        }
+    });
+}
+
+template <typename T>
 __global__ __launch_bounds__(kT) void rowsum2_kernel(const T* __restrict__ x, double* __restrict__ sums, long long P) {
     __shared__ float red[4];
     const int row = blockIdx.y;
@@ -341,6 +362,22 @@
     else
         hipLaunchKernelGGL(bias_gelu_bwd_kernel<__hip_bfloat16>, pw_grid(rows, P), dim3(kT), 0, st,
                            (const __hip_bfloat16*)x, bias, (const __hip_bfloat16*)gy, (__hip_bfloat16*)gx, gbias, C, P);
+    MK_LAUNCH_CHECK();
+    return 0;
+}
+
+extern "C" int mk_affine_add(const void* r, const void* z, const float* affine, void* y, int dtype, int rows, long long P,
+                             void* stream) {
+    MK_REQUIRE(r && z && affine && y, "null pointer");
+    const int C = 1;
+    PW_CHECK();
+    hipStream_t st = (hipStream_t)stream;
+    if (dtype == 0)
+        hipLaunchKernelGGL(affine_add_kernel<float>, pw_grid(rows, P), dim3(kT), 0, st, (const float*)r, (const float*)z, affine,
+                           (float*)y, P);
+    else
+        hipLaunchKernelGGL(affine_add_kernel<__hip_bfloat16>, pw_grid(rows, P), dim3(kT), 0, st, (const __hip_bfloat16*)r,
+                           (const __hip_bfloat16*)z, affine, (__hip_bfloat16*)y, P);
     MK_LAUNCH_CHECK();
     return 0;
 }
diff --git a/makani_amd/layers.py b/makani_amd/layers.py
--- a/makani_amd/layers.py
+++ b/makani_amd/layers.py
@@ -189,6 +189,157 @@
     with torch.autocast("cuda", enabled=False):
         y = _PceConvNormAdd.apply(x3, conv.weight2d(), conv.bias, z, sums, nw, nb, norm.eps, group, count)
     return y.view(B, conv.out_channels, H, W)
+
+
+class _NormSkipAdd(torch.autograd.Function):
+
+    @staticmethod
+    def forward(ctx, r4, z4, sums, nw, nb, eps, group, count):
+        from . import ops
+        B, C, H, W = z4.shape
+        if group is not None:
+            torch.distributed.all_reduce(sums, group=group)
+        cnt = H * W if group is None else int(count)
+        wf = None if nw is None else nw.detach().float().contiguous()
+        bf = None if nb is None else nb.detach().float().contiguous()
+        stats, affine = ops.instance_norm_coeffs(sums, wf, bf, B * C, C, cnt, eps)
+        y = ops.affine_add(r4, z4, affine)
+        empty = z4.new_empty(0, dtype=torch.float32)
+        ctx.save_for_backward(z4, stats, wf if wf is not None else empty, bf if bf is not None else empty)
+        ctx.cfg = (None if nw is None else nw.dtype, None if nb is None else nb.dtype, group, cnt)
+        return y
+
+    @staticmethod
+    def backward(ctx, gy):
+        from . import ops
+        z4, stats, wf, bf = ctx.saved_tensors
+        nw_dtype, nb_dtype, group, cnt = ctx.cfg
+        gy = gy.contiguous()
+        gz, gnw, gnb = ops.instance_norm_backward(z4, gy, stats, wf if nw_dtype is not None else None,
+                                                  bf if nb_dtype is not None else None, False, group, cnt,
+                                                  grad_dtype=nw_dtype if (nw_dtype is not None and nw_dtype == nb_dtype) else None)
+        return (gy, gz, None, gnw.to(nw_dtype) if nw_dtype is not None else None,
+                gnb.to(nb_dtype) if nb_dtype is not None else None, None, None, None)
+
+
+class _NormSkipAddFFT(torch.autograd.Function):
+
+    @staticmethod
+    def forward(ctx, xf, twiddles, nlon, kmajor, z4, sums, nw, nb, eps):
+        from . import ops
+        B, C, H, W = z4.shape
+        wf = None if nw is None else nw.detach().float().contiguous()
+        bf = None if nb is None else nb.detach().float().contiguous()
+        stats, affine = ops.instance_norm_coeffs(sums, wf, bf, B * C, C, H * W, eps)
+        y = ops.irfft_affine_add_raw(xf, twiddles, nlon, z4, affine, kmajor)
+        empty = z4.new_empty(0, dtype=torch.float32)
+        ctx.save_for_backward(z4, stats, wf if wf is not None else empty, bf if bf is not None else empty, twiddles)
+        ctx.cfg = (None if nw is None else nw.dtype, None if nb is None else nb.dtype, xf.shape[1] if kmajor else xf.shape[0],
+                   bool(kmajor))
+        return y
+
+    @staticmethod
+    def backward(ctx, gy):
+        from . import ops
+        z4, stats, wf, bf, tw = ctx.saved_tensors
+        nw_dtype, nb_dtype, mmax, kmajor = ctx.cfg
+        B, C, H, W = z4.shape
+        gy = gy.contiguous()
+        gxf = ops.rfft_raw(gy.view(B * C, H, W), tw, mmax, 1.0, 2.0, 1.0, kmajor) if ctx.needs_input_grad[0] else None
+        gz, gnw, gnb = ops.instance_norm_backward(z4, gy, stats, wf if nw_dtype is not None else None,
+                                                  bf if nb_dtype is not None else None, False, None, H * W,
+                                                  grad_dtype=nw_dtype if (nw_dtype is not None and nw_dtype == nb_dtype) else None)
+        return (gxf, None, None, None, gz, None, gnw.to(nw_dtype) if nw_dtype is not None else None,
+                gnb.to(nb_dtype) if nb_dtype is not None else None, None)
+
+
+def spectral_skip_supported(conv, z_like):
+    from . import ops
+    if not isinstance(conv, Conv1x1) or conv.bias is not None or not ops.spec_mix_supported(conv.in_channels, conv.out_channels):
+        return False
+    if os.environ.get("MK_NORM_SKIP_FUSION", "1") == "0" or os.environ.get("MK_CONV_ENGINE", "pce") != "pce":
+        return False
+    if not (z_like.is_cuda and z_like.dim() == 4):
+        return False
+    return z_like.dtype == torch.bfloat16 or (z_like.dtype == torch.float32 and torch.is_autocast_enabled()
+                                              and torch.get_autocast_dtype("cuda") == torch.bfloat16)
+
+
+def spectral_skip_plus_instance_norm(conv, filt, spec, z, sums, norm):
+    from . import comm, ops
+    from .layer_norm import DistributedInstanceNorm2d
+    if sums is None or z.dtype != torch.bfloat16 or not z.is_contiguous() or z.dim() != 4 or not ops.pointwise_supported(z):
+        return None
+    group = count = None
+    if isinstance(norm, DistributedInstanceNorm2d):
+        if comm.get_size("spatial") > 1:
+            group, count = comm.get_group("spatial"), norm._global_count(z)
+        nw, nb = (norm.weight, norm.bias) if norm.affine else (None, None)
+    elif isinstance(norm, InstanceNorm2d) and not norm.track_running_stats:
+        nw, nb = norm.weight, norm.bias
+    else:
+        return None
+    B, C, H, W = z.shape
+    if C != conv.out_channels or (H, W) != (filt.nlat_local, filt.nlon_local):
+        return None
+    from .sht import InverseRealSHT
+    it = filt.inverse_transform
+    with torch.autocast("cuda", enabled=False):
+        cm = ops.spec_mix(spec, conv.weight, B, filt.l_off, filt.m_off)
+        if group is None and type(it) is InverseRealSHT and ops.irfft_affine_add_supported(it.nlon, it.mmax):
+            km = ops.SPECTRAL_GEMM == "bf16x3"
+            xf = ops.legendre_inv(cm, it.pct, it.nlat, 0, km)
+            return _NormSkipAddFFT.apply(xf, it.twiddles, it.nlon, km, z, sums, nw, nb, norm.eps)
+        r = filt.synthesise(cm, B, z.dtype)
+        return _NormSkipAdd.apply(r.view(B, C, H, W), z, sums, nw, nb, norm.eps, group, count)
+
+
+class _PceConvGelu(torch.autograd.Function):
+
+    @staticmethod
+    def forward(ctx, x3, w, bias, keep_pre):
+        from . import ops
+        if keep_pre:
+            h, pre = ops.pce_gemm(x3, ops.pce_pack(w), w.shape[0], bias=bias, want_pre=True, gelu=True)
+        else:
+            h, pre = ops.pce_gemm(x3, ops.pce_pack(w), w.shape[0], bias=bias, gelu=True), x3.new_empty(0)
+        ctx.save_for_backward(x3, w, pre)
+        ctx.bias_dtype = None if bias is None else bias.dtype
+        ctx.step = _step_items(w)
+        return h
+
+    @staticmethod
+    def backward(ctx, gh):
+        from . import ops
+        x3, w, pre = ctx.saved_tensors
+        (wimg_t, gbuf), ctx.step = (ctx.step or (None, None)), None
+        need_gb = ctx.bias_dtype is not None and ctx.needs_input_grad[2]
+        gpre, gsum = ops.gelu_backward(pre, gh.contiguous(), need_gb)
+        gx = gw = gb = None
+        if ctx.needs_input_grad[0]:
+            gx = ops.pce_gemm(gpre, wimg_t if wimg_t is not None else ops.pce_pack(w, transpose=True), w.shape[1])
+        if ctx.needs_input_grad[1]:
+            gw = ops.conv1x1_wgrad_raw(gpre, x3, out=gbuf).to(w.dtype)
+        if need_gb:
+            gb = gsum.to(ctx.bias_dtype)
+        return gx, gw, gb, None
+
+
+def encoder_head(encoder, x):
+    from . import ops
+    mods = list(encoder.fwd)
+    pat = _mlp_pattern(mods)
+    if pat is None or x.dim() != 4:
+        return None
+    fc1, fc2 = pat
+    if fc2.bias is not None or not ops.spec_mix_supported(fc2.in_channels, fc2.out_channels):
+        return None
+    x3 = _engine_field(x)
+    if x3 is None or not ops.pce_supported_train(fc1.out_channels, fc1.in_channels):
+        return None
+    with torch.autocast("cuda", enabled=False):
+        h = _PceConvGelu.apply(x3, fc1.weight2d(), fc1.bias, torch.is_grad_enabled())
+    return h.view(x.shape[0], fc1.out_channels, x.shape[2], x.shape[3]), fc2
 
 
 class _PceMLP(torch.autograd.Function):
diff --git a/makani_amd/ops.py b/makani_amd/ops.py
--- a/makani_amd/ops.py
+++ b/makani_amd/ops.py
@@ -94,6 +94,27 @@
                                          bc, k, nlon, m, 1.0, 1.0, 1.0, int(bool(kmajor)), int(chans), int(cpp), sums.data_ptr(),
                                          _stream()), "mk_irfft_sums")
     return x, sums
+
+
+def irfft_affine_add_supported(nlon, mmax):
+    return nlon in (480, 1440) and mmax <= 241 and os.environ.get("MK_FFT_LEGACY", "0") != "1" \
+        and os.environ.get("MK_IRFFT_AFFINE_ADD", "1") != "0"
+
+
+def irfft_affine_add_raw(xf, twiddles, nlon, z, affine, kmajor=False):
+    _need_cuda(xf, twiddles, z, affine)
+    assert xf.dim() == 3 and xf.is_contiguous() and xf.dtype == torch.complex64
+    if kmajor:
+        k, m, bc = xf.shape
+    else:
+        m, k, bc = xf.shape
+    assert z.is_contiguous() and z.numel() == bc * k * nlon and z.dtype in (torch.float32, torch.bfloat16)
+    assert affine.dtype == torch.float32 and affine.is_contiguous() and affine.numel() == 2 * bc
+    x = torch.empty_like(z)
+    _lib.check(_lib.load().mk_irfft_affine_add(xf.data_ptr(), x.data_ptr(), _pw_dtype(z), twiddles.data_ptr(), bc, k, nlon, m,
+                                               1.0, 1.0, 1.0, int(bool(kmajor)), z.data_ptr(), affine.data_ptr(), _stream()),
+               "mk_irfft_affine_add")
+    return x
 
 
 def irfft_raw(xf, twiddles, nlon, s0, sm, sh, out_dtype=torch.float32, kmajor=False):
@@ -723,6 +744,72 @@
         return gx, gw, None, None, None
 
 
+def spec_mix_supported(cin, cout):
+    return (os.environ.get("MK_SPEC_MIX", "1") != "0" and _gemm_mode(None) == "bf16x3" and cin % 2 == 0 and cout % 2 == 0)
+
+
+def _spec_mix_args(x, batch):
+    _need_cuda(x)
+    assert x.dim() == 3 and x.is_contiguous() and x.dtype == torch.complex64 and x.shape[2] % batch == 0
+    return x.shape[0], x.shape[1], x.shape[2] // batch
+
+
+def spec_mix_fwd_raw(x, w, batch, l_off=0, m_off=0):
+    lloc, mloc, cin = _spec_mix_args(x, batch)
+    assert w.dtype == torch.float32 and w.is_contiguous() and w.dim() == 2 and w.shape[1] == cin
+    cout = w.shape[0]
+    y = torch.empty(lloc, mloc, batch * cout, dtype=torch.complex64, device=x.device)
+    _lib.check(_lib.load().mk_spec_mix_fwd(x.data_ptr(), w.data_ptr(), y.data_ptr(), lloc, mloc, batch, cin, cout, l_off, m_off,
+                                           _stream()), "mk_spec_mix_fwd")
+    return y
+
+
+def spec_mix_dgrad_raw(gy, w, batch, l_off=0, m_off=0):
+    lloc, mloc, cout = _spec_mix_args(gy, batch)
+    assert w.dtype == torch.float32 and w.is_contiguous() and w.dim() == 2 and w.shape[0] == cout
+    cin = w.shape[1]
+    gx = torch.empty(lloc, mloc, batch * cin, dtype=torch.complex64, device=gy.device)
+    _lib.check(_lib.load().mk_spec_mix_dgrad(gy.data_ptr(), w.data_ptr(), gx.data_ptr(), lloc, mloc, batch, cin, cout, l_off,
+                                             m_off, _stream()), "mk_spec_mix_dgrad")
+    return gx
+
+
+def spec_mix_wgrad_raw(x, gy, batch, l_off=0, m_off=0):
+    lloc, mloc, cin = _spec_mix_args(x, batch)
+    l2, m2, cout = _spec_mix_args(gy, batch)
+    assert (l2, m2) == (lloc, mloc)
+    gw = torch.zeros(cout, cin, dtype=torch.float32, device=x.device)
+    _lib.check(_lib.load().mk_spec_mix_wgrad(x.data_ptr(), gy.data_ptr(), gw.data_ptr(), lloc, mloc, batch, cin, cout, l_off,
+                                             m_off, _stream()), "mk_spec_mix_wgrad")
+    return gw
+
+
+class _SpecMix(torch.autograd.Function):
+
+    @staticmethod
+    def forward(ctx, x, w, batch, l_off, m_off):
+        wf = w.detach().float().contiguous()
+        ctx.save_for_backward(x, wf)
+        ctx.args = (batch, l_off, m_off, w.dtype, tuple(w.shape))
+        return spec_mix_fwd_raw(x, wf.view(wf.shape[0], -1), batch, l_off, m_off)
+
+    @staticmethod
+    def backward(ctx, gy):
+        x, wf = ctx.saved_tensors
+        batch, l_off, m_off, wdt, wshape = ctx.args
+        gy = gy.contiguous()
+        gx = gw = None
+        if ctx.needs_input_grad[0]:
+            gx = spec_mix_dgrad_raw(gy, wf.view(wf.shape[0], -1), batch, l_off, m_off)
+        if ctx.needs_input_grad[1]:
+            gw = spec_mix_wgrad_raw(x, gy, batch, l_off, m_off).view(wshape).to(wdt)
+        return gx, gw, None, None, None
+
+
+def spec_mix(x, w, batch, l_off=0, m_off=0):
+    return _SpecMix.apply(x, w, batch, l_off, m_off)
+
+
 def rfft(x, twiddles, mmax, kmajor=False):
     return _RFFT.apply(x, twiddles, mmax, kmajor)
 
@@ -936,6 +1023,28 @@
 
 def bias_gelu(x, bias):
     return _BiasGelu.apply(x, bias)
+
+
+def gelu_backward(pre, gy, want_row_sums=False):
+    _need_cuda(pre, gy)
+    assert pre.dim() == 3 and pre.is_contiguous() and gy.is_contiguous() and gy.shape == pre.shape and gy.dtype == pre.dtype
+    b, c, p = pre.shape
+    gx = torch.empty_like(pre)
+    gsum = torch.zeros(c, dtype=torch.float32, device=pre.device) if want_row_sums else None
+    _lib.check(_lib.load().mk_bias_gelu_bwd(pre.data_ptr(), 0, gy.data_ptr(), gx.data_ptr(), 0 if gsum is None else gsum.data_ptr(),
+                                            _pw_dtype(pre), b * c, c, p, _stream()), "mk_bias_gelu_bwd")
+    return gx, gsum
+
+
+def affine_add(r, z, affine):
+    _need_cuda(r, z, affine)
+    assert r.is_contiguous() and z.is_contiguous() and r.shape == z.shape and r.dtype == z.dtype and z.dim() == 4
+    B, C, H, W = z.shape
+    assert affine.dtype == torch.float32 and affine.is_contiguous() and affine.numel() == 2 * B * C
+    y = torch.empty_like(z)
+    _lib.check(_lib.load().mk_affine_add(r.data_ptr(), z.data_ptr(), affine.data_ptr(), y.data_ptr(), _pw_dtype(z), B * C, H * W,
+                                         _stream()), "mk_affine_add")
+    return y
 
 
 def instance_norm(x, weight, bias, eps=1e-5, fuse_gelu=False, group=None, count=None, row_sums=None):
diff --git a/makani_amd/sfnonet.py b/makani_amd/sfnonet.py
--- a/makani_amd/sfnonet.py
+++ b/makani_amd/sfnonet.py
@@ -11,7 +11,8 @@
 from .distributed import DistributedInverseRealFFT2, DistributedInverseRealSHT, DistributedRealFFT2, DistributedRealSHT
 from .layer_norm import DistributedInstanceNorm2d, DistributedLayerNorm
 from .layers import (Conv1x1, DropPath, EncoderDecoder, InstanceNorm2d, InverseRealFFT2, MLP, RealFFT2, _engine_field,
-                     _is_exact_gelu, conv_plus_instance_norm)
+                     _is_exact_gelu, _is_noop, conv_plus_instance_norm, encoder_head, spectral_skip_plus_instance_norm,
+                     spectral_skip_supported)
 from .sht import InverseRealSHT, RealSHT
 from .spectral_convolution import FactorizedSpectralConv, SpectralAttention, SpectralConv
 
@@ -54,11 +55,18 @@
             self.filter = FactorizedSpectralConv(forward_transform, inverse_transform, embed_dim, embed_dim, rank=rank,
                                                  factorization=factorization, **common)
 
-    def forward(self, x, want_row_sums=False):
+    def forward(self, x, want_row_sums=False, **spectral):
+        spectral = {k: v for k, v in spectral.items() if v}
+        if spectral:
+            out = self.filter(x, want_row_sums=want_row_sums, **spectral)
+            return out
         if want_row_sums and isinstance(self.filter, SpectralConv) and type(self.filter).forward is SpectralConv.forward:
             return self.filter(x, want_row_sums=True)
         out = self.filter(x)
         return (out[0], out[1], None) if want_row_sums else out
+
+    def takes_spectral_mix(self):
+        return isinstance(self.filter, SpectralConv) and self.filter.takes_spectral_mix()
 
 
 class FourierNeuralOperatorBlock(nn.Module):
@@ -101,13 +109,27 @@
         return (isinstance(norm, (nn.InstanceNorm2d, DistributedInstanceNorm2d))
                 and not getattr(norm, "track_running_stats", False))
 
-    def forward(self, x):
+    def _spectral_outer_skip(self, x):
+        outer = getattr(self, "outer_skip", None)
+        return (outer is not None and hasattr(self, "mlp") and not hasattr(self, "inner_skip")
+                and isinstance(self.filter, SpectralFilterLayer) and self.filter.takes_spectral_mix()
+                and self.filter.filter.scale_residual
+                and self.output_shape_loc[0] * self.output_shape_loc[1] > self.input_shape_loc[0] * self.input_shape_loc[1]
+                and isinstance(self.norm1, (InstanceNorm2d, DistributedInstanceNorm2d))
+                and isinstance(self.drop_path, nn.Identity) and not hasattr(self, "act_layer1")
+                and getattr(self.mlp, "checkpointing", 0) < 2 and spectral_skip_supported(outer, x))
+
+    def forward(self, x, premix=None):
         inner = getattr(self, "inner_skip", None)
         hip_norm0 = isinstance(self.norm0, (InstanceNorm2d, DistributedInstanceNorm2d)) \
             and not getattr(self.norm0, "track_running_stats", False)
         sums0 = None
+        batch, in_dtype = x.shape[0], x.dtype
+        spec_skip = self._spectral_outer_skip(x)
         if hip_norm0 and isinstance(self.filter, SpectralFilterLayer):
-            x, residual, sums0 = self.filter(x, want_row_sums=True)
+            x, residual, sums0 = self.filter(x, want_row_sums=True, premix=premix, spectrum_residual=spec_skip)
+        elif premix is not None or spec_skip:
+            x, residual = self.filter(x, premix=premix, spectrum_residual=spec_skip)
         else:
             x, residual = self.filter(x)
         if inner is None and hip_norm0 and _is_exact_gelu(self.act_layer0):
@@ -129,6 +151,11 @@
             else:
                 x = self.mlp(x, skip_last_bias=self._removes_channel_constants(self.norm1))
         outer = getattr(self, "outer_skip", None)
+        if spec_skip:
+            y = spectral_skip_plus_instance_norm(outer, self.filter.filter, residual, x, sums, self.norm1)
+            if y is not None:
+                return y
+            residual = self.filter.filter.residual_from_spectrum(residual, batch, in_dtype)
         if sums is not None and isinstance(self.drop_path, nn.Identity) and not hasattr(self, "act_layer1"):
             y = conv_plus_instance_norm(outer, residual, x, sums, self.norm1)
             if y is not None:
@@ -270,11 +297,22 @@
         with torch.autocast(device_type=x.device.type, enabled=False):
             return self.itrans_up(self.trans_down(x.float()).contiguous()).to(x.dtype)
 
-    def _forward_features(self, x):
+    def _forward_features(self, x, premix=None):
         for _ in range(self.repeat_layers):
-            for blk in self.blocks:
-                x = checkpoint(blk, x, use_reentrant=False) if self.checkpointing >= 3 else blk(x)
+            for i, blk in enumerate(self.blocks):
+                if i == 0 and premix is not None:
+                    x = blk(x, premix=premix)
+                else:
+                    x = checkpoint(blk, x, use_reentrant=False) if self.checkpointing >= 3 else blk(x)
         return x
+
+    def _spectral_encoder(self, x):
+        blk = self.blocks[0] if len(self.blocks) else None
+        if (blk is None or hasattr(self, "pos_embed") or not _is_noop(self.pos_drop) or self.checkpointing != 0
+                or self.repeat_layers != 1 or not blk.filter.takes_spectral_mix() or not blk.filter.filter.scale_residual
+                or hasattr(blk, "inner_skip")):
+            return None
+        return encoder_head(self.encoder, x)
 
     def _engine_arena(self, x):
         from . import ops
@@ -307,10 +345,14 @@
             if x3 is not None and x3.dtype != x.dtype:
                 x = x3.view(x.shape)
         skip_in = self._big_skip_input(x) if self.big_skip else None
-        x = checkpoint(self.encoder, x, use_reentrant=False) if self.checkpointing >= 1 else self.encoder(x)
-        if hasattr(self, "pos_embed"):
-            x = x + self._position_field(x)
-        x = self._forward_features(self.pos_drop(x))
+        head = self._spectral_encoder(x)
+        if head is not None:
+            x = self._forward_features(head[0], premix=head[1])
+        else:
+            x = checkpoint(self.encoder, x, use_reentrant=False) if self.checkpointing >= 1 else self.encoder(x)
+            if hasattr(self, "pos_embed"):
+                x = x + self._position_field(x)
+            x = self._forward_features(self.pos_drop(x))
         x = checkpoint(self.decoder, x, use_reentrant=False) if self.checkpointing >= 1 else self.decoder(x)
         if skip_in is not None:
             x = self.residual_transform(skip_in, addend=x)
diff --git a/makani_amd/spectral_convolution.py b/makani_amd/spectral_convolution.py
--- a/makani_amd/spectral_convolution.py
+++ b/makani_amd/spectral_convolution.py
@@ -92,7 +92,19 @@
     def _weight_tensor(self):
         return self.weight
 
-    def _forward_fused(self, x, dtype, want_row_sums=False):
+    def synthesise(self, c, B, odt):
+        it = self.inverse_transform
+        return it.inverse_packed(c, B, odt) if self._distributed else it.inverse_packed(c, odt)
+
+    def residual_from_spectrum(self, c, B, dtype):
+        with torch.autocast(device_type="cuda", enabled=False):
+            r = self.synthesise(c, B, dtype if dtype in (torch.float32, torch.bfloat16) else torch.float32)
+        return r.view(B, -1, r.shape[-2], r.shape[-1]).to(dtype)
+
+    def takes_spectral_mix(self):
+        return type(self) is SpectralConv and self._fused
+
+    def _forward_fused(self, x, dtype, want_row_sums=False, premix=None, spectrum_residual=False):
         B, C = x.shape[0], x.shape[1]
         ft, it = self.forward_transform, self.inverse_transform
         xin = x if x.dtype in (torch.float32, torch.bfloat16) else x.float()
@@ -101,10 +113,15 @@
             c = ft.forward_packed(xin)
         else:
             c = ft.forward_packed(xin.view(B * C, xin.shape[2], xin.shape[3]))
+        if premix is not None:
+            c = ops.spec_mix(c, premix.weight, B, self.l_off, self.m_off)
+            C = premix.out_channels
         odt = dtype if dtype in (torch.float32, torch.bfloat16) else torch.float32
         residual = x
-        if self.scale_residual:
-            r = it.inverse_packed(c, B, odt) if self._distributed else it.inverse_packed(c, odt)
+        if self.scale_residual and spectrum_residual:
+            residual = c
+        elif self.scale_residual:
+            r = self.synthesise(c, B, odt)
             residual = r.view(B, C, r.shape[-2], r.shape[-1]).to(dtype)
         y = ops.dhconv(c, self._weight_tensor(), B, self.l_off, self.m_off)
         sums = None
@@ -115,13 +132,16 @@
         out = out.view(B, self.out_channels, out.shape[-2], out.shape[-1])
         return out, residual, sums
 
-    def forward(self, x, want_row_sums=False):
+    def forward(self, x, want_row_sums=False, premix=None, spectrum_residual=False):
         dtype = x.dtype
         residual = x
         sums = None
+        if premix is not None or spectrum_residual:
+            assert self.takes_spectral_mix() and x.is_cuda and x.dim() == 4 and (premix is None or self.scale_residual)
         if self._fused and x.is_cuda and x.dim() == 4:
             with torch.autocast(device_type="cuda", enabled=False):
-                x, residual, sums = self._forward_fused(x, dtype, want_row_sums and not hasattr(self, "bias"))
+                x, residual, sums = self._forward_fused(x, dtype, want_row_sums and not hasattr(self, "bias"), premix,
+                                                        spectrum_residual)
             if sums is not None and x.dtype != dtype:
                 sums = None
         else:
```

After: 24.83 samples/s (median of 6 runs). 5.1% higher.
